# troyvvgroup/quemb

Measured on AMD Instinct MI355X. Metric: fragment CCSD iters/sec (full BE sweep over synthetic n_occ=20 n_virt=200 fragments); corr-E error vs oracle in parity_max_abs_err_Eh / parity_n220_abs_err_Eh, higher is better.
Workload: dtype f64

## Files before the change

### include/qemb_hip_ops.h

```cpp
#ifndef QEMB_HIP_OPS_H
#define QEMB_HIP_OPS_H
#include "qemb_hip.h"
#ifdef __cplusplus
extern "C" {
#endif

#define QEMB_TIMER_LADDER 0
#define QEMB_TIMER_RINGS 1
#define QEMB_TIMER_ITER 2
#define QEMB_TIMER_AO2MO 3
#define QEMB_TIMER_SCF 4
#define QEMB_TIMER_GEMM_ANY 5
#define QEMB_TIMER_SCHMIDT 6
#define QEMB_TIMER_DF 7
int qemb_timer_begin(int slot);
int qemb_timer_end(int slot);
int qemb_timer_read(int slot, double* total_ms, int64_t* count);
int qemb_timer_reset(int slot);
int qemb_alloc_stats(long long* n_driver_allocs, long long* n_driver_frees, double* ms_in_driver_calls, double* gb_allocated, int reset);
int qemb_gemm_flop_count(double* flops, int reset);
int qemb_tape_cache_counters(int64_t* reused, int64_t* recorded, int reset);
int qemb_ctx_timer_read(int ctx, int slot, double* total_ms, int64_t* count, int reset);
int qemb_timer_live_events(int slot);


int qemb_op_gemm(int64_t M, int64_t N, int64_t K, double alpha, const double* A, int64_t lda, int a_kcontig,
                 int64_t strideA, const double* B, int64_t ldb, int b_kcontig, int64_t strideB, double beta,
                 double* C, int64_t ldc, int64_t strideC, int64_t batch);
int qemb_op_gemm_slab_rows(int64_t M, int64_t N, int64_t K, const double* A, int64_t lda, int64_t a_slab, int64_t a_slab_skip, const double* B, int64_t ldb,
                           int b_kcontig, double* C, int64_t ldc, int cfg);
int qemb_set_gemm_config(int cfg);
int qemb_mfma_f64_peak(int iters, int blocks_per_cu, double* tflops);
int qemb_set_gemm_splitk(int enabled);
int qemb_op_gemm_probe(int64_t M, int64_t N, int64_t K, const double* A, int64_t lda, int a_kcontig, const double* B, int64_t ldb, int b_kcontig,
                       double* C, int64_t ldc, int cfg, int ksplit, double* ms, double* clock_ghz, int64_t* workgroups);
int qemb_op_gemm_stamps(int64_t M, int64_t N, int64_t K, const double* A, int64_t lda, const double* B, int64_t ldb, double* C, int64_t ldc, int cfg,
                        int ksplit, double* out7);
int qemb_pair_gemm_choice(int64_t rows, int64_t cols, int* cfg, int* ksplit);
int qemb_ccsd_gemm_plans(int o, int v, int64_t* out);
int qemb_set_gemm_ksplit(int ksplit);
int qemb_gemm_tile_table(int index, int* id, int* rows, int* cols, int* bk, int* mode1, int* has_classic, int* ladder_twin);
int qemb_gemm_last_launch(int* cfg, int* vec2, int* mode, int* ksplit, int* sb_m, int* sb_n, int* wide_c);
int qemb_op_copy4(const int64_t dim[4], const double* in, const int64_t si[4], double* out,
                  const int64_t so[4], double alpha, double beta);
int qemb_op_outer4(const int64_t dim[4], const double* u, int64_t su0, int64_t su2, const double* v,
                   int64_t sv1, int64_t sv3, double* out, const int64_t so[4], double alpha, double beta);
int qemb_op_div_denom(double* x, int64_t d0, int64_t d1, int64_t d2, int64_t d3, const double* ea,
                      const double* eb, const double* ec, const double* ed);
int qemb_op_ladder_pack_vvvv(int64_t n, int64_t o, const double* M, double* Vp, int64_t ldp, double* Vm, int64_t ldm);
int qemb_op_ladder_pack_tau(int64_t o, int64_t v, const double* tau, double* Tp, int64_t ldp, double* Tm, int64_t ldm);
int qemb_op_ladder_scatter_pm(int64_t o, int64_t v, const double* Rp, int64_t ldp, const double* Rm, int64_t ldm, double* t2);
int qemb_op_dot(int64_t n, const double* x, const double* y, double* out_dev);
int qemb_op_absmax(int64_t n, const double* x, double* out_dev);
int qemb_op_gemv_rows(int64_t rows, int64_t cols, const double* T, int64_t ldt, const double* x, double* y,
                      double alpha, double beta);
int qemb_op_gemv_rows_batched(int64_t rows, int64_t cols, int64_t nbatch, const double* T, int64_t ldt, int64_t strideT,
                              const double* x, int64_t stridex, double* y, double alpha, double beta);
int qemb_op_contract_mid(int64_t outer, int64_t mid, int64_t inner, const double* T, const double* x,
                         double* Y, int64_t ldy, double alpha, double beta);
int qemb_op_unpack_s4(int64_t n, const double* s4, double* s1);
int qemb_op_pack_s4(int64_t n, const double* s1, double* s4);
int qemb_op_unpack_s8_to_s4(int64_t n, const double* s8, double* s4);
int qemb_op_mirror_lower(int64_t n, double* A, int64_t lda);
int qemb_op_k_from_pairs(int64_t n, const double* H, const double* D, double* K);
int qemb_op_jk_from_packed(int64_t n, const double* S4, const double* D, const double* Dp, double* Jp, double* K);
int qemb_op_pack_pm_cols(int64_t rows, int64_t v, const double* in, double* Op, int64_t ldp, double* Om, int64_t ldm);
int qemb_op_scatter_pm_rows(int64_t o, int64_t ncols, const double* Xp, const double* Xm, double* out);
int qemb_op_pack_w_pm(int64_t o, const double* W, double* Ap, int64_t lda_p, double* Am, int64_t lda_m);
int qemb_op_ladder_scatter_pm2(int64_t o, int64_t v, const double* Rp, int64_t ldp, const double* Rm, int64_t ldm, const double* Hp, const double* Hm,
                               int assign, double* t2);
int qemb_op_lincomb2(int64_t n, double a, const double* x, double b, const double* y, double beta, double* out);
int qemb_op_small_k_update(int64_t batch, int64_t M, int64_t N, int64_t K, double alpha, const double* A, int64_t sA, const double* B, int64_t sB, double* C, int64_t sC);
int qemb_op_ccsd_ph_layouts(int64_t o, int64_t v, const double* t2, const double* t1, double* T, double* Tp, double* S, double* Ut, double* Tpt, double* Th);
int qemb_op_ccsd_y_traces(int64_t o, int64_t v, const double* ZC, const double* ZB, double* Y);
int qemb_op_copy4_two(const int64_t dim[4], const double* in, const int64_t si[4], double* out, const int64_t so[4], double alpha, double beta, const double* base,
                      double* out2, const double* in2, double c2a, double c2b);
int qemb_op_scatter_pm_rows_add(int64_t o, int64_t ncols, const double* Xp, const double* Xm, double* out, const double* add);
int qemb_op_ccsd_y_traces_add(int64_t o, int64_t v, const double* ZC, const double* ZB, double* Y, const double* add);
int qemb_op_pack_w_pm_sum(int64_t o, const double* Wt, const double* X, const double* At, double* Ap, int64_t lda_p, double* Am, int64_t lda_m);
int qemb_op_ccsd_t1_small(int64_t o, int64_t v, const double* t1, const double* Lvv, const double* Loo, const double* Fov, double* t1n);
int qemb_op_ccsd_t1_assemble(int64_t o, int64_t v, const double* t1, const double* Lvv, const double* Loo, const double* Fov, const double* S, const double* Lph1,
                             const double* PA, int SA, int64_t strideA, const double* PB, int SB, int64_t strideB, double* t1n);
int qemb_op_gemv_rows_two(int64_t rows1, int64_t cols1, const double* T1, int64_t ld1, const double* x1, double* y1, double a1, double b1,
                          int64_t rows2, int64_t cols2, const double* T2, int64_t ld2, const double* x2, double* y2, double a2, double b2);
int qemb_op_ccsd_y_traces_slabs(int64_t o, int64_t v, const double* ZC, const double* ZB, double* Y, const double* add, int S, int64_t stride, double scale);
int qemb_op_gemv_rows2(int64_t rows, int64_t cols, const double* T1, int64_t ld1, const double* x1, const double* T2, int64_t ld2, const double* x2, double* y, double alpha, double beta);
int qemb_op_ccsd_finish_t2_rings(int64_t o, int64_t v, double* t2n, const double* U, const double* OV, const double* RS, const double* M, const double* eo, const double* ev, double* t1n);
int qemb_op_diis_push(int64_t n, const double* trial, const double* prev, double* e, double* xcopy, int m, const double* const* ys, int self, double* row_dev, double* row_host);
int qemb_op_ccsd_extrapolate_energy(int64_t o, int64_t v, int nterms, const double* coef, const double* const* xs, double* amp, const double* L, double* tau, double* e_host);
int qemb_op_gather_rows(int64_t nrows, int64_t len, const int64_t* idx_dev, const double* src, int64_t ld, double* dst);
int qemb_op_scale_rows(int64_t nrows, int64_t len, double* x, const double* s);
int qemb_op_pack_pair_rows(int64_t n, int64_t ncols, const double* in, double* out);
int qemb_op_unpack_tril_pair_rows(int64_t nr, int64_t n, const double* in, double* full);
int qemb_op_extract_pf(int64_t n, const double* Mp, int64_t p0, int64_t q0, int64_t r0, int64_t s0, int64_t sp, int64_t sq,
                       int64_t sr, int64_t ss, double* out);
int qemb_op_extract_pf_t(int64_t n, const double* T, int64_t x0, int64_t r0, int64_t s0, int64_t c0, int64_t sx, int64_t sr,
                         int64_t ss, int64_t sc, double* out);
int qemb_op_ladder_pack_vvvv_pf(int64_t n, int64_t o, const double* Mp, double* Vp, int64_t ldp, double* Vm, int64_t ldm);
int qemb_op_extract_pf_t_compact(int64_t n, const double* T, int64_t x0, int64_t c0, int64_t sx, int64_t sr, int64_t ss, int64_t sc,
                                 double* out, int64_t slab);
int qemb_op_gather_pair_cols(int64_t rows, int64_t n, const double* in, int64_t r0, int64_t s0, int64_t sr, int64_t ss, double* out);
int qemb_op_extract_ps(int64_t n, const double* S, int64_t p0, int64_t q0, int64_t r0, int64_t s0, int64_t sp, int64_t sq,
                       int64_t sr, int64_t ss, double* out);
int qemb_op_extract_ps_packed(int64_t n, const double* S, int64_t p0, int64_t q0, int64_t r0, int64_t sp, int64_t sq, int64_t sr, double* out);
int qemb_op_unpack_pair_block(int64_t n, int64_t o, const double* S, double* Mv, int64_t ld);
int qemb_op_ladder_pack_vvvv_pf_ld(int64_t n, int64_t o, const double* Mp, int64_t ld, double* Vp, int64_t ldp, double* Vm, int64_t ldm);
int qemb_op_pack_pm_ovvv(int64_t o, int64_t v, const double* ovvv, double* Op, int64_t ldp, double* Om, int64_t ldm);
int qemb_op_df_pair_product(int64_t np, int64_t naux, const double* bb, double* out);
int qemb_op_unpack_tril_rows(int64_t rows, int64_t n, const double* packed, double* full);
int qemb_op_pack_tril_rows(int64_t rows, int64_t n, const double* full, double* packed);
int qemb_op_jacobi_eigh(int64_t n, double* A, double* w, double* V, int* sweeps);
int qemb_op_scf_fused_max(void);
int qemb_op_jacobi_eigh_in_basis(int64_t n, const double* F, const double* Cp, double* w, double* C_out, double* C2_out, int nocc, double* dm_out, double stop_below, int* sweeps);
int qemb_op_scf_fock_small(int64_t n, const double* h, const double* J, const double* K, const double* D, double* F, double* err, double* scal2);
int qemb_op_pack_density_sym(int64_t n, const double* D, double* Dp);
int qemb_op_jacobi_svd(int64_t m, int64_t n, double* G, double* s, double* U, double* V, int* sweeps);
int qemb_op_cholesky_lower(int64_t n, double* A);
int qemb_op_tri_inverse_lower(int64_t n, const double* L, double* Linv);


int qemb_op_mp2_amplitudes(int64_t o, int64_t v, const double* ovov, const double* eo, const double* ev, double* t2, double* G, double* e_host);

int qemb_op_rdm2_assemble(int kind, int64_t o, int64_t v, const double* t1, const double* t2, const double* dm1c, double* out);
int qemb_op_rdm2_add_nc(int64_t m, const double* g, double alpha, double* X);
int qemb_op_rdm2_symmetrize(int64_t m, const double* g, double* X);
int qemb_op_rdm2_eri_dot(int64_t m, int sym, const double* eri, const double* K, double* e_host);

int qemb_op_kdf_split(int64_t rows, int64_t nao, const double* z, double* planes);
int qemb_op_kdf_stack(int64_t nk, int64_t nao, int64_t n, const double* ta, double* Cs, double* Dk);
int qemb_op_kdf_pack(int64_t naux, int64_t n, const double* M, int paired, double w, double* F, int64_t ldf, double* out2_host);

int qemb_frag_prepare_ccsd(qemb_frag_t f, int nsocc, const double* h, const double* dm0, const qemb_solver_opts* opts);
int qemb_frag_ccsd_iterate(qemb_frag_t f, int niter, double* e_corr, double* normt);
int qemb_frag_ccsd_reset(qemb_frag_t f);
int qemb_frag_ccsd_export(qemb_frag_t f, const char* name, double* host, int64_t nelem);


int qemb_op_boys(int m_max, int64_t n, const double* x, double* out);
int qemb_op_int3c_class(int la, int lb, int lP, const void* bf_a, const void* bf_b, const void* bf_P, const double* c2s, double* out_host);
int qemb_op_int4c_class(int la, int lb, int lc, int ld, const void* bf_a, const void* bf_b, const void* bf_c, const void* bf_d, const double* c2s, double* out_host);
int qemb_op_int4c_tile(void* basis, const int32_t* pairs_r, int64_t n_r, const int32_t* pairs_s, int64_t n_s, double thresh, double* out_host);
int qemb_op_cd_panel_factor(int n, const double* A_host, double thr, double* T_host, int32_t* piv_host, int32_t* rank, int* in_lds);
int qemb_op_cd_diag_update(int64_t np, int r, const double* Lnew_host, const int32_t* pivrow_host, double* d_host, int64_t nsp, const int32_t* row0_host, const int32_t* cnt_host,
                           double* spmax_host, double* dmax_host);
int qemb_op_cd_permute(int64_t M, int64_t N, const double* L_host, const int32_t* pos_host, int full, double* out_host);
int qemb_op_df_get_ints(void* df, double* out_host, int* identity_metric);

int qemb_op_fci_sigma(int n, int nsocc, const double* h_host, const double* V_dev, const double* c_dev, double* sigma_dev);
int qemb_op_fci_rdm12(int n, int nsocc, const double* c_dev, int cumulant, double* dm1_host, double* dm2_dev);
int qemb_op_fci_sigma_timed(int n, int nsocc, const double* h_host, const double* V_dev, const double* c_dev, double* sigma_dev, double* ms3);
int qemb_op_fci_links(int n, int nsocc, int64_t* ns, int* nlink, int32_t* strings_host, int32_t* links_host);

int qemb_op_joint_diag(int64_t K, int64_t m, double* Q_dev, double* U_dev, double stop_angle, int max_sweeps, int* sweeps, double* f, int* converged);
int qemb_op_joint_diag_bytes(int64_t K, int64_t m, int64_t* bytes, int* in_lds);
int qemb_op_joint_diag_mem_limit(int64_t bytes);

#ifdef __cplusplus
}
#endif
#endif
```

### quemb_amd/_lib.py

```python

from __future__ import annotations

import ctypes as C
import os
from pathlib import Path

import numpy as np

_HERE = Path(__file__).resolve().parent
LIB_PATH = _HERE / "libqemb_hip.so"

c_dp = C.POINTER(C.c_double)
c_i64 = C.c_int64
c_vp = C.c_void_p


QEMB_ERR_ARG, QEMB_ERR_ALLOC, QEMB_ERR_DEVICE, QEMB_ERR_NOCONV, QEMB_ERR_NUMERIC, QEMB_ERR_UNSUPPORTED = -1, -2, -3, -4, -5, -6


class QembError(RuntimeError):

    def __init__(self, msg="", status=None):
        super().__init__(msg)
        self.status = status


class SolverOpts(C.Structure):
    _fields_ = [("struct_size", C.c_uint32), ("cc_conv_tol", C.c_double), ("cc_conv_tol_normt", C.c_double), ("cc_max_cycle", C.c_int),
                ("cc_diis_space", C.c_int), ("scf_conv_tol", C.c_double), ("scf_conv_tol_grad", C.c_double),
                ("scf_max_cycle", C.c_int), ("scf_diis_space", C.c_int), ("warm_start", C.c_int), ("verbose", C.c_int),
                ("relax_density", C.c_int), ("lambda_conv_tol", C.c_double), ("lambda_max_cycle", C.c_int),
                ("strict_convergence", C.c_int)]


class FciOpts(C.Structure):
    _fields_ = [("struct_size", C.c_uint32), ("conv_tol", C.c_double), ("max_cycle", C.c_int), ("max_space", C.c_int), ("lindep", C.c_double)]


_lib = None
_initialised_device = None


def _declare(lib):
    def f(name, restype, *argtypes):
        fn = getattr(lib, name)
        fn.restype = restype
        fn.argtypes = list(argtypes)

    I, D, P, V, L = C.c_int, C.c_double, c_vp, c_vp, c_i64
    f("qemb_init", I, I)
    f("qemb_last_error", C.c_char_p)
    f("qemb_backend", C.c_char_p)
    f("qemb_sync", I)
    f("qemb_device_sync", I)
    f("qemb_mem_info", I, C.POINTER(C.c_size_t), C.POINTER(C.c_size_t))
    f("qemb_malloc", I, C.POINTER(c_vp), C.c_size_t)
    f("qemb_free", I, V)
    f("qemb_trim", I)
    f("qemb_trim_all", I)
    f("qemb_h2d", I, V, V, C.c_size_t)
    f("qemb_d2h", I, V, V, C.c_size_t)
    f("qemb_h2d_async", I, V, V, C.c_size_t)
    f("qemb_d2d", I, V, V, C.c_size_t)
    f("qemb_timer_begin", I, I)
    f("qemb_timer_end", I, I)
    f("qemb_timer_read", I, I, C.POINTER(D), C.POINTER(L))
    f("qemb_timer_reset", I, I)
    f("qemb_timer_live_events", I, I)
    f("qemb_op_gemm", I, L, L, L, D, P, L, I, L, P, L, I, L, D, P, L, L, L)
    f("qemb_op_gemm_slab_rows", I, L, L, L, P, L, L, L, P, L, I, P, L, I)
    f("qemb_op_gemm_probe", I, L, L, L, P, L, I, P, L, I, P, L, I, I, C.POINTER(D), C.POINTER(D), C.POINTER(L))
    f("qemb_op_gemm_stamps", I, L, L, L, P, L, P, L, P, L, I, I, C.POINTER(D))
    f("qemb_set_gemm_config", I, I)
    f("qemb_set_gemm_splitk", I, I)
    f("qemb_set_gemm_ksplit", I, I)
    f("qemb_pair_gemm_choice", I, L, L, C.POINTER(I), C.POINTER(I))
    f("qemb_ccsd_gemm_plans", I, I, I, C.POINTER(L))
    f("qemb_gemm_tile_table", I, I, *([C.POINTER(I)] * 7))
    f("qemb_gemm_last_launch", I, *([C.POINTER(I)] * 7))
    f("qemb_op_ladder_pack_vvvv", I, L, L, P, P, L, P, L)
    f("qemb_op_ladder_pack_tau", I, L, L, P, P, L, P, L)
    f("qemb_op_ladder_scatter_pm", I, L, L, P, L, P, L, P)
    f("qemb_mfma_f64_peak", I, I, I, C.POINTER(D))
    f("qemb_op_copy4", I, C.POINTER(L), P, C.POINTER(L), P, C.POINTER(L), D, D)
    f("qemb_op_outer4", I, C.POINTER(L), P, L, L, P, L, L, P, C.POINTER(L), D, D)
    f("qemb_op_div_denom", I, P, L, L, L, L, P, P, P, P)
    f("qemb_op_dot", I, L, P, P, P)
    f("qemb_op_mp2_amplitudes", I, L, L, P, P, P, P, P, C.POINTER(D))
    f("qemb_op_rdm2_assemble", I, I, L, L, P, P, P, P)
    f("qemb_op_rdm2_add_nc", I, L, P, D, P)
    f("qemb_op_rdm2_symmetrize", I, L, P, P)
    f("qemb_op_rdm2_eri_dot", I, L, I, P, P, C.POINTER(D))
    f("qemb_op_absmax", I, L, P, P)
    f("qemb_op_gemv_rows", I, L, L, P, L, P, P, D, D)
    f("qemb_op_gemv_rows_batched", I, L, L, L, P, L, L, P, L, P, D, D)
    f("qemb_op_contract_mid", I, L, L, L, P, P, P, L, D, D)
    f("qemb_op_unpack_s4", I, L, P, P)
    f("qemb_op_pack_s4", I, L, P, P)
    f("qemb_op_unpack_s8_to_s4", I, L, P, P)
    f("qemb_op_unpack_tril_rows", I, L, L, P, P)
    f("qemb_op_pack_pair_rows", I, L, L, P, P)
    f("qemb_op_mirror_lower", I, L, P, L)
    f("qemb_op_k_from_pairs", I, L, P, P, P)
    f("qemb_op_jk_from_packed", I, L, P, P, P, P, P)
    f("qemb_op_pack_pm_cols", I, L, L, P, P, L, P, L)
    f("qemb_op_scatter_pm_rows", I, L, L, P, P, P)
    f("qemb_op_pack_w_pm", I, L, P, P, L, P, L)
    f("qemb_op_ladder_scatter_pm2", I, L, L, P, L, P, L, P, P, I, P)
    f("qemb_op_lincomb2", I, L, D, P, D, P, D, P)
    f("qemb_op_small_k_update", I, L, L, L, L, D, P, L, P, L, P, L)
    f("qemb_op_ccsd_ph_layouts", I, L, L, P, P, P, P, P, P, P, P)
    f("qemb_op_ccsd_y_traces", I, L, L, P, P, P)
    f("qemb_op_copy4_two", I, C.POINTER(L), P, C.POINTER(L), P, C.POINTER(L), D, D, P, P, P, D, D)
    f("qemb_op_scatter_pm_rows_add", I, L, L, P, P, P, P)
    f("qemb_op_ccsd_y_traces_add", I, L, L, P, P, P, P)
    f("qemb_op_pack_w_pm_sum", I, L, P, P, P, P, L, P, L)
    f("qemb_op_ccsd_t1_small", I, L, L, P, P, P, P, P)
    f("qemb_op_gemv_rows2", I, L, L, P, L, P, P, L, P, P, D, D)
    f("qemb_op_ccsd_t1_assemble", I, L, L, P, P, P, P, P, P, P, I, L, P, I, L, P)
    f("qemb_op_gemv_rows_two", I, L, L, P, L, P, P, D, D, L, L, P, L, P, P, D, D)
    f("qemb_op_ccsd_y_traces_slabs", I, L, L, P, P, P, P, I, L, D)
    f("qemb_op_ccsd_finish_t2_rings", I, L, L, P, P, P, P, P, P, P, P)
    f("qemb_op_diis_push", I, L, P, P, P, P, I, P, I, P, P)
    f("qemb_op_ccsd_extrapolate_energy", I, L, L, I, P, P, P, P, P, P)
    f("qemb_op_gather_rows", I, L, L, P, P, L, P)
    f("qemb_op_scale_rows", I, L, L, P, P)
    f("qemb_ctx_count", I, I)
    f("qemb_ctx_bind", I, I)
    f("qemb_ctx_partition", I, I)
    f("qemb_ctx_timer_read", I, I, I, C.POINTER(C.c_double), C.POINTER(c_i64), I)
    f("qemb_gemm_flop_count", I, C.POINTER(C.c_double), I)
    f("qemb_tape_cache_counters", I, C.POINTER(L), C.POINTER(L), I)
    f("qemb_alloc_stats", I, C.POINTER(C.c_longlong), C.POINTER(C.c_longlong), C.POINTER(C.c_double), C.POINTER(C.c_double), I)
    f("qemb_op_unpack_tril_pair_rows", I, L, L, P, P)
    f("qemb_op_extract_pf", I, L, P, L, L, L, L, L, L, L, L, P)
    f("qemb_op_extract_pf_t", I, L, P, L, L, L, L, L, L, L, L, P)
    f("qemb_op_ladder_pack_vvvv_pf", I, L, L, P, P, L, P, L)
    f("qemb_op_extract_pf_t_compact", I, L, P, L, L, L, L, L, L, P, L)
    f("qemb_op_gather_pair_cols", I, L, L, P, L, L, L, L, P)
    f("qemb_op_extract_ps", I, L, P, L, L, L, L, L, L, L, L, P)
    f("qemb_op_extract_ps_packed", I, L, P, L, L, L, L, L, L, P)
    f("qemb_op_unpack_pair_block", I, L, L, P, P, L)
    f("qemb_op_ladder_pack_vvvv_pf_ld", I, L, L, P, L, P, L, P, L)
    f("qemb_op_pack_pm_ovvv", I, L, L, P, P, L, P, L)
    f("qemb_op_df_pair_product", I, L, L, P, P)
    f("qemb_op_pack_tril_rows", I, L, L, P, P)
    f("qemb_op_jacobi_eigh", I, L, P, P, P, C.POINTER(I))
    f("qemb_op_scf_fused_max", I)
    f("qemb_op_jacobi_eigh_in_basis", I, L, P, P, P, P, P, I, P, D, C.POINTER(I))
    f("qemb_op_scf_fock_small", I, L, P, P, P, P, P, P, P)
    f("qemb_op_pack_density_sym", I, L, P, P)
    f("qemb_op_jacobi_svd", I, L, L, P, P, P, P, C.POINTER(I))
    f("qemb_op_cholesky_lower", I, L, P)
    f("qemb_op_joint_diag", I, L, L, P, P, D, I, C.POINTER(I), C.POINTER(D), C.POINTER(I))
    f("qemb_df_localize_er", I, V, P, I, D, I, P, C.POINTER(I), C.POINTER(D), C.POINTER(D), C.POINTER(I))
    f("qemb_op_joint_diag_bytes", I, L, L, C.POINTER(L), C.POINTER(I))
    f("qemb_op_joint_diag_mem_limit", I, L)
    f("qemb_op_tri_inverse_lower", I, L, P, P)
    f("qemb_comm_unique_id", I, P)
    f("qemb_comm_init", I, I, I, P)
    f("qemb_comm_info", I, C.POINTER(I), C.POINTER(I))
    f("qemb_comm_allreduce", I, P, L, I)
    f("qemb_comm_destroy", I)
    OP = C.POINTER(SolverOpts)
    IP = C.POINTER(I)
    DP = C.POINTER(D)
    f("qemb_default_opts", None, OP)
    f("qemb_frag_create", I, I, I, C.POINTER(c_vp))
    f("qemb_frag_free", I, V)
    f("qemb_frag_set_eri_s4", I, V, P)
    f("qemb_frag_set_eri_s4_dev", I, V, P)
    f("qemb_frag_set_df_factor", I, V, I, P)
    f("qemb_frag_set_df_factor_dev", I, V, I, P)
    f("qemb_frag_mo_route", I, V, I)
    f("qemb_frag_set_df_only", I, V, I, P)
    f("qemb_frag_set_df_only_dev", I, V, I, V)
    f("qemb_frag_resident_bytes", I, V, C.POINTER(L))
    f("qemb_frag_mo_route_used", I, V, IP, IP)
    f("qemb_frag_get_eri_s4", I, V, P)
    f("qemb_frag_set_energy_data", I, V, P, P, P, D, IP, I)
    f("qemb_frag_jk", I, V, P, P, P)
    f("qemb_frag_solve", I, V, I, P, P, OP, I, P, P, P, P, P, P, P, DP, DP, DP, IP, IP)
    f("qemb_frag_solve_mp2", I, V, I, P, P, OP, I, P, P, P, P, P, P, DP, DP, DP, IP)
    f("qemb_frag_solve_mp2_batch", I, I, P, IP, P, P, OP, I, P, P, P, P, P, P, P, P, P, IP)
    f("qemb_default_fci_opts", None, C.POINTER(FciOpts))
    f("qemb_frag_solve_fci", I, V, I, P, P, OP, C.POINTER(FciOpts), I, P, P, P, P, P, P, DP, DP, DP, IP, IP)
    f("qemb_frag_fci_bytes", I, I, I, I, C.POINTER(L))
    f("qemb_frag_fci_mem_limit", I, V, L)
    f("qemb_frag_fci_residual", I, V, DP)
    f("qemb_op_fci_sigma", I, I, I, P, P, P, P)
    f("qemb_op_fci_rdm12", I, I, I, P, I, P, P)
    f("qemb_op_fci_sigma_timed", I, I, I, P, P, P, P, P)
    f("qemb_op_fci_links", I, I, I, C.POINTER(L), IP, P, P)
    f("qemb_frag_rdm2", I, V, I, I, P)
    f("qemb_frag_rdm2_mem_limit", I, V, L)
    f("qemb_frag_rdm2_dev", I, V, I, I, P)
    f("qemb_rdm2_full_guard", I, L, L, L)
    f("qemb_frag_lambda_iters", I, P, C.POINTER(C.c_int))
    f("qemb_frag_solve_batch", I, I, P, IP, P, P, OP, I, P, P, P, P, P, P, P, P, P, P, IP, IP, C.POINTER(L))
    f("qemb_frag_scf", I, V, I, P, P, OP, P, P, P, P, DP, IP, IP)
    f("qemb_frag_cphf", I, V, I, P, P, OP, P, I, P)
    f("qemb_ccsd_solve", I, I, I, I, P, P, P, OP, P, P, D, IP, I, P, P, P, P, P, P, DP, IP)
    f("qemb_frag_prepare_ccsd", I, V, I, P, P, OP)
    f("qemb_frag_ccsd_iterate", I, V, I, DP, DP)
    f("qemb_frag_ccsd_reset", I, V)
    f("qemb_frag_ccsd_export", I, V, C.c_char_p, P, L)
    LP = C.POINTER(L)
    f("qemb_aoeri_upload", I, I, P, I, C.POINTER(c_vp))
    f("qemb_aoeri_free", I, V)
    f("qemb_ao2mo_dense", I, V, P, I, P, V)
    f("qemb_df_create", I, I, P, C.POINTER(c_vp))
    f("qemb_lpq_upload", I, P, I, C.POINTER(c_vp))
    f("qemb_df_create_pbc", I, I, P, C.POINTER(c_vp), IP)
    f("qemb_df_alloc_ints", I, V, I)
    f("qemb_df_add_pw_block", I, V, I, P, P, P, P)
    f("qemb_df_add_rs_block", I, V, I, I, P)
    f("qemb_df_pw_imag_absmax", I, V, C.POINTER(C.c_double))
    f("qemb_df_pw_select", I, V, I)
    f("qemb_df_free", I, V)
    f("qemb_df_set_ints", I, V, I, P, I)
    f("qemb_df_set_ints_semisparse", I, V, I, L, P, P, P, P)
    f("qemb_df_transform", I, V, P, I, P, V)
    f("qemb_df_transform_screened", I, V, P, I, P, D, P, V)
    f("qemb_df_transform_factor", I, V, P, I, V)
    f("qemb_df_transform_screened_factor", I, V, P, I, P, D, V)
    f("qemb_kdf_create", I, I, I, I, IP, IP, C.POINTER(c_vp))
    f("qemb_kdf_set_pair", I, V, I, I, P)
    f("qemb_kdf_transform", I, V, P, I, P, V, I)
    f("qemb_kdf_free", I, V)
    f("qemb_kdf_guard", I, I, I, I, I, I, I, L)
    f("qemb_frag_get_df_factor", I, V, P)
    f("qemb_int_basis_create", I, I, P, C.c_size_t, P, C.POINTER(c_vp))
    f("qemb_int_basis_free", I, V)
    f("qemb_int3c2e", I, V, V, P, L, I, P, I)
    f("qemb_int2c2e", I, V, P, I)
    f("qemb_df_create_empty", I, C.POINTER(c_vp))
    f("qemb_df_set_ints_from_basis", I, V, V, V)
    f("qemb_df_set_ints_semisparse_from_basis", I, V, V, V, L, P, P, P, P)
    f("qemb_int4c2e", I, V, I, D, P, I)
    f("qemb_int4c_mem_limit", I, V, L)
    f("qemb_int4c_stats", I, V, C.POINTER(L), C.POINTER(L))
    f("qemb_aoeri_from_basis", I, V, D, C.POINTER(c_vp))
    f("qemb_int_jk_direct", I, V, P, D, P, P, I)
    f("qemb_int_jk_direct_bytes", I, V, C.POINTER(L))
    f("qemb_ao2mo_direct", I, V, I, P, P, P, P, L, D)
    f("qemb_ao2mo_direct_bytes", I, V, I, P, L, C.POINTER(L))
    f("qemb_int4c_tile_stats", I, V, C.POINTER(L), C.POINTER(L))
    f("qemb_op_int4c_tile", I, V, P, L, P, L, D, P)
    f("qemb_int_cholesky", I, V, D, D, L, L, P, C.POINTER(L))
    f("qemb_int_cholesky_bytes", I, V, L, L, C.POINTER(L))
    f("qemb_int_cholesky_stats", I, V, P)
    f("qemb_df_set_ints_from_cholesky", I, V, V, D, D, L, L)
    f("qemb_op_cd_panel_factor", I, I, P, D, P, P, C.POINTER(C.c_int32), C.POINTER(I))
    f("qemb_op_cd_diag_update", I, L, I, P, P, P, L, P, P, P, P)
    f("qemb_op_cd_permute", I, L, L, P, P, I, P)
    f("qemb_op_df_get_ints", I, V, P, C.POINTER(I))
    f("qemb_int1e", I, V, I, P, P, P, P, P)
    f("qemb_int1e_dipole", I, V, P, P)
    f("qemb_df_jk", I, V, I, P, P, I, I, I, P, P)
    f("qemb_df_jk_bytes", I, V, I, I, C.POINTER(L))
    f("qemb_df_jk_mem_limit", I, V, L)
    f("qemb_op_int4c_class", I, I, I, I, I, P, P, P, P, P, P)
    f("qemb_op_boys", I, I, L, P, P)
    f("qemb_op_int3c_class", I, I, I, I, P, P, P, P, P)
    f("qemb_op_kdf_split", I, L, L, P, P)
    f("qemb_op_kdf_stack", I, L, L, L, P, P, P)
    f("qemb_op_kdf_pack", I, L, L, P, I, D, P, L, DP)
    f("qemb_schmidt", I, P, I, I, I, LP, I, D, P, I, IP, IP)
    f("qemb_schmidt_subspace", I, P, I, I, I, LP, I, D, P, I, IP, IP)
    f("qemb_schmidt_svd", I, P, I, LP, I, D, P, I, IP, IP)
    f("qemb_nsocc_guess", I, P, I, I, P, IP, P)
    f("qemb_matmul", I, L, L, L, P, I, P, I, P)
    f("qemb_abs_overlap_prim", I, I, P, P, P, P, L, I, P, P, P)
    return lib


def load(path: os.PathLike | None = None):
    global _lib
    if _lib is None:
        p = Path(path) if path else LIB_PATH
        if not p.exists():
            raise QembError(
                f"{p} not found: build it with `python -c 'import __graft_entry__ as g; g.build()'` "
                "(make -C quemb_amd/csrc). quemb_amd has no CPU fallback."
            )
        _lib = _declare(C.CDLL(str(p)))
    return _lib


def declare(cdll):
    return _declare(cdll)


class ConvergenceWarning(RuntimeWarning):
    """A fragment solve did not converge and `strict_convergence = 0` asked for PySCF's behaviour (warn, carry on)."""


def check(rc: int, what: str = "", lib=None):
    if rc > 0:
        import warnings
        msg = (lib or load()).qemb_last_error().decode(errors="replace")
        warnings.warn(ConvergenceWarning(f"{what or 'libqemb_hip call'}: {msg}"), stacklevel=3)
    elif rc != 0:
        msg = (lib or load()).qemb_last_error().decode(errors="replace")
        raise QembError(f"{what or 'libqemb_hip call'} failed (status {rc}): {msg}", status=int(rc))


def init(device: int | None = None):
    global _initialised_device
    lib = load()
    if device is None:
        if _initialised_device is not None:
            return lib
        device = int(os.environ.get("LOCAL_RANK", "0"))
    if _initialised_device != device:
        check(lib.qemb_init(int(device)), "qemb_init")
        _initialised_device = device
    return lib


class DeviceBuffer:

    def __init__(self, nelem: int, lib=None):
        self.lib = lib or init()
        self.n = int(nelem)
        p = c_vp()
        check(self.lib.qemb_malloc(C.byref(p), max(self.n, 1) * 8), "qemb_malloc")
        self.ptr = p.value

    @classmethod
    def from_numpy(cls, a: np.ndarray, lib=None):
        a = np.ascontiguousarray(a, dtype=np.float64)
        b = cls(a.size, lib=lib)
        b.upload(a)
        return b

    def upload(self, a: np.ndarray):
        a = np.ascontiguousarray(a, dtype=np.float64)
        assert a.size <= self.n
        check(self.lib.qemb_h2d(self.ptr, a.ctypes.data, a.size * 8), "qemb_h2d")

    def numpy(self, shape=None) -> np.ndarray:
        out = np.empty(self.n, dtype=np.float64)
        check(self.lib.qemb_d2h(out.ctypes.data, self.ptr, self.n * 8), "qemb_d2h")
        return out if shape is None else out[: int(np.prod(shape))].reshape(shape)

    def at(self, offset_elems: int) -> int:
        return self.ptr + 8 * int(offset_elems)

    def free(self):
        if getattr(self, "ptr", None):
            self.lib.qemb_free(self.ptr)
            self.ptr = None

    def __del__(self):
        try:
            self.free()
        except Exception:
            pass


def i64x4(v):
    return (c_i64 * 4)(*[int(x) for x in v])
```

### quemb_amd/csrc/ao2mo.cpp

```cpp
#include "ao2mo.h"
#include "int4c_core.h"
#include <algorithm>
#include <cmath>
#include <cstdlib>
#include <vector>

namespace qemb {

static inline int64_t npair(int64_t n) { return n * (n + 1) / 2; }

int AoEri::upload(int N_, const double* host, int sym) {
  N = N_;
  const int64_t np = npair(N), n2 = (int64_t)N * N;
  QTRY(s4.alloc(np * np));
  if (sym == 4) return dev_h2d(s4, host, sizeof(double) * np * np);
  if (sym == 8) {
    DBuf s8;
    const int64_t n8 = np * (np + 1) / 2;
    QTRY(s8.alloc(n8));
    QTRY(dev_h2d(s8, host, sizeof(double) * n8));
    return dev_unpack_s8_to_s4(N, s8, s4);
  }
  if (sym == 1) {
    DBuf s1;
    QTRY(s1.alloc(n2 * n2));
    QTRY(dev_h2d(s1, host, sizeof(double) * n2 * n2));
    return dev_pack_s4(N, s1, s4);
  }
  set_error("AoEri::upload: sym must be 1, 4 or 8");
  return QEMB_ERR_ARG;
}

int ao2mo_dense(const AoEri& ao, const double* TA, int n, double* out_s4) {
  const int64_t N = ao.N;
  if (N <= 0 || n <= 0 || n > N) { set_error("ao2mo_dense: need 0 < n <= N"); return QEMB_ERR_ARG; }
  const int64_t npN = npair(N), npn = npair(n);
  DBuf W1, W2;
  QTRY(W1.alloc(std::max<int64_t>(npN * N * N, (int64_t)n * n * npN)));
  QTRY(W2.alloc(std::max<int64_t>((int64_t)n * npN * N, npn * N * N)));
  TimerScope lap_AO2MO(TIMER_AO2MO);
  const int tcfg = fits_one_224_tile(n) ? GEMM_224x128 : -1;
  QTRY(dev_unpack_tril_rows(npN, N, ao.s4, W1));
  QTRY(gemm(n, npN * N, N, 1.0, TA, n, false, W1, N, true, 0.0, W2, npN * N, 1, 0, 0, 0, tcfg));
  QTRY(gemm_quarter_lower_rows(n, npN, N, TA, W2, W1));
  QTRY(dev_unpack_tril_pair_rows(n, N, W1, W2));
  QTRY(gemm(n, npn * N, N, 1.0, TA, n, false, W2, N, true, 0.0, W1, npn * N, 1, 0, 0, 0, tcfg));
  QTRY(gemm_quarter_lower_rows(n, npn, N, TA, W1, W2));
  QTRY(dev_pack_pair_rows(n, npn, W2, out_s4));
  QTRY(lap_AO2MO.close());
  return 0;
}

int ao2mo_tile_accumulate(const double* E, int64_t ld, const TileRows& R, const TileRows& S, bool diagonal, const double* TA, int n, double* PR, double* PS,
                          double* T, double* A) {
  const int64_t npq = npair(n);
  int4c::PairProdArgs g{};
  g.TA = TA; g.n = n; g.npq = npq;
  g.mu = S.mu; g.nu = S.nu; g.rows = S.rows; g.P = PS;
  QTRY(dev_int4c_pairprod(g));
  if (!diagonal) {
    g.mu = R.mu; g.nu = R.nu; g.rows = R.rows; g.P = PR;
    QTRY(dev_int4c_pairprod(g));
  }
  QTRY(gemm(R.rows, npq, S.rows, 1.0, E, ld, true, PS, npq, false, 0.0, T, npq));
  return gemm(npq, npq, R.rows, diagonal ? 0.5 : 1.0, diagonal ? PS : PR, npq, false, T, npq, false, 1.0, A, npq);
}

int DfContext::set_metric(int naux_, const double* j2c) {
  naux = naux_; identity_metric = false;
  DBuf L;
  QTRY(L.alloc((int64_t)naux * naux));
  QTRY(dev_h2d(L, j2c, sizeof(double) * naux * naux));
  QTRY(dev_cholesky_lower(naux, L));
  QTRY(Linv.alloc((int64_t)naux * naux));
  return dev_tri_inverse_lower(naux, L, Linv);
}
int DfContext::set_cholesky_factor(int naux_, const double* Lh) {
  naux = naux_; identity_metric = false;
  DBuf L;
  QTRY(L.alloc((int64_t)naux * naux));
  QTRY(dev_h2d(L, Lh, sizeof(double) * naux * naux));
  QTRY(Linv.alloc((int64_t)naux * naux));
  return dev_tri_inverse_lower(naux, L, Linv);
}
int DfContext::set_metric_pbc(int naux_, const double* j2c, int* ischol) {
  naux = naux_; identity_metric = false;
  DBuf A, w, V;
  const int64_t n2 = (int64_t)naux * naux;
  QTRY(A.alloc(n2));
  QTRY(dev_h2d(A, j2c, sizeof(double) * n2));
  QTRY(Linv.alloc(n2));
  int rc = dev_cholesky_lower(naux, A);
  if (rc == QEMB_OK) { if (ischol) *ischol = 1; return dev_tri_inverse_lower(naux, A, Linv); }
  if (rc != QEMB_ERR_NUMERIC) return rc;
  if (ischol) *ischol = 0;
  QTRY(dev_h2d(A, j2c, sizeof(double) * n2));
  QTRY(w.alloc(naux)); QTRY(V.alloc(n2));
  QTRY(dev_jacobi_eigh(naux, A, w, V, nullptr));
  {
    DBuf AV, D;
    QTRY(AV.alloc(n2)); QTRY(D.alloc(n2));
    QTRY(dev_h2d(A, j2c, sizeof(double) * n2));
    QTRY(gemm(naux, naux, naux, 1.0, A, naux, true, V, naux, false, 0.0, AV, naux));
    QTRY(gemm(naux, naux, naux, 1.0, V, naux, false, AV, naux, false, 0.0, D, naux));
    Copy4Desc c{};
    c.dim[0] = 1; c.dim[1] = 1; c.dim[2] = 1; c.dim[3] = naux;
    c.in = D; c.si[0] = 0; c.si[1] = 0; c.si[2] = 0; c.si[3] = naux + 1;
    c.out = w; c.so[0] = 0; c.so[1] = 0; c.so[2] = 0; c.so[3] = 1; c.alpha = 1.0; c.beta = 0.0;
    QTRY(dev_copy4(c));
  }
  std::vector<double> d(naux);
  QTRY(dev_d2h(d.data(), w, sizeof(double) * naux));
  for (double& x : d) x = (x > 1e-14) ? 1.0 / std::sqrt(std::sqrt(x)) : 0.0;
  QTRY(dev_h2d(w, d.data(), sizeof(double) * naux));
  QTRY(dev_mul_bcast_rows(naux, naux, V, w));
  return gemm(naux, naux, naux, 1.0, V, naux, true, V, naux, true, 0.0, Linv, naux);
}
int DfContext::alloc_ints(int N_) {
  if (naux <= 0) { set_error("DfContext: set the metric first"); return QEMB_ERR_ARG; }
  if (N_ <= 0) { set_error("DfContext::alloc_ints: N must be positive"); return QEMB_ERR_ARG; }
  N = N_;
  Usp.release(); n_unique = 0;
  const int64_t sz = (int64_t)naux * N * N;
  QTRY(Lpq.alloc(sz)); QTRY(Lpq_im.alloc(sz));
  Lpq_sum.release(); Lact = nullptr;
  QTRY(dev_fill(Lpq, sz, 0.0));
  return dev_fill(Lpq_im, sz, 0.0);
}
int DfContext::add_rs_block(int p0, int p1, const double* h) {
  if (!Lpq.p || !Lpq_im.p) { set_error("DfContext::add_rs_block: alloc_ints first"); return QEMB_ERR_ARG; }
  if (p0 < 0 || p1 > naux || p0 >= p1 || !h) { set_error("DfContext::add_rs_block: need 0 <= p0 < p1 <= naux"); return QEMB_ERR_ARG; }
  const int64_t n2 = (int64_t)N * N, sz = (int64_t)(p1 - p0) * n2;
  DBuf tmp;
  QTRY(tmp.alloc(sz));
  QTRY(dev_h2d(tmp, h, sizeof(double) * sz));
  return axpby(sz, 1.0, tmp, 1.0, Lpq.p + (int64_t)p0 * n2);
}
int DfContext::add_pw_block(int nG, const double* F_re, const double* F_im, const double* pw_re, const double* pw_im) {
  if (!Lpq.p || !Lpq_im.p) { set_error("DfContext::add_pw_block: alloc_ints first"); return QEMB_ERR_ARG; }
  if (nG <= 0 || !F_re || !F_im || !pw_re || !pw_im) { set_error("DfContext::add_pw_block: bad arguments"); return QEMB_ERR_ARG; }
  const int64_t n2 = (int64_t)N * N;
  DBuf fr, fi, pr, pi;
  QTRY(fr.alloc((int64_t)naux * nG)); QTRY(fi.alloc((int64_t)naux * nG));
  QTRY(pr.alloc((int64_t)nG * n2)); QTRY(pi.alloc((int64_t)nG * n2));
  QTRY(dev_h2d(fr, F_re, sizeof(double) * naux * nG)); QTRY(dev_h2d(fi, F_im, sizeof(double) * naux * nG));
  QTRY(dev_h2d(pr, pw_re, sizeof(double) * nG * n2)); QTRY(dev_h2d(pi, pw_im, sizeof(double) * nG * n2));
  QTRY(gemm(naux, n2, nG, 1.0, fr, nG, true, pr, n2, false, 1.0, Lpq, n2));
  QTRY(gemm(naux, n2, nG, -1.0, fi, nG, true, pi, n2, false, 1.0, Lpq, n2));
  QTRY(gemm(naux, n2, nG, 1.0, fr, nG, true, pi, n2, false, 1.0, Lpq_im, n2));
  return gemm(naux, n2, nG, 1.0, fi, nG, true, pr, n2, false, 1.0, Lpq_im, n2);
}
int DfContext::imag_absmax(double* out) const {
  if (!Lpq_im.p || !out) { set_error("DfContext::imag_absmax: no plane-wave accumulation on this context"); return QEMB_ERR_ARG; }
  DBuf r;
  QTRY(r.alloc(1));
  QTRY(dev_absmax((int64_t)naux * N * N, Lpq_im, r));
  return dev_d2h(out, r, sizeof(double));
}
int DfContext::select_part(int part) {
  if (part == 0) { Lact = nullptr; return QEMB_OK; }
  if (!Lpq.p || !Lpq_im.p) { set_error("DfContext::select_part: no plane-wave accumulation on this context"); return QEMB_ERR_ARG; }
  if (part == 1) { Lact = Lpq_im.p; return QEMB_OK; }
  if (part == 2) {
    const int64_t sz = (int64_t)naux * N * N;
    QTRY(Lpq_sum.alloc(sz));
    QTRY(dcopy(sz, Lpq, Lpq_sum));
    QTRY(axpby(sz, 1.0, Lpq_im, 1.0, Lpq_sum));
    Lact = Lpq_sum.p;
    return QEMB_OK;
  }
  set_error("DfContext::select_part: part must be 0, 1 or 2");
  return QEMB_ERR_ARG;
}
int DfContext::set_ints_Lpq(int N_, const double* h) {
  N = N_;
  Usp.release(); n_unique = 0; Lact = nullptr; Lpq_im.release(); Lpq_sum.release();
  if (naux <= 0) { set_error("DfContext: set the metric first"); return QEMB_ERR_ARG; }
  QTRY(Lpq.alloc((int64_t)naux * N * N));
  return dev_h2d(Lpq, h, sizeof(double) * naux * N * N);
}
int DfContext::set_ints_pqL(int N_, const double* h) {
  N = N_;
  Usp.release(); n_unique = 0; Lact = nullptr; Lpq_im.release(); Lpq_sum.release();
  if (naux <= 0) { set_error("DfContext: set the metric first"); return QEMB_ERR_ARG; }
  DBuf tmp;
  const int64_t n2 = (int64_t)N * N;
  QTRY(tmp.alloc(n2 * naux));
  QTRY(dev_h2d(tmp, h, sizeof(double) * n2 * naux));
  QTRY(Lpq.alloc(n2 * naux));
  return perm4(Lpq, tmp, 1, 1, n2, naux, 0, 1, 3, 2);
}
int DfContext::set_ints_packed(int N_, const double* h) {
  N = N_;
  Usp.release(); n_unique = 0; Lact = nullptr; Lpq_im.release(); Lpq_sum.release();
  if (naux <= 0) { set_error("DfContext: set the metric first"); return QEMB_ERR_ARG; }
  DBuf tmp;
  QTRY(tmp.alloc((int64_t)naux * npair(N)));
  QTRY(dev_h2d(tmp, h, sizeof(double) * naux * npair(N)));
  QTRY(Lpq.alloc((int64_t)naux * N * N));
  return dev_unpack_tril_rows(naux, N, tmp, Lpq);
}

int DfContext::set_ints_semisparse(int N_, int64_t n_unique_, const double* unique_host, const int64_t* ptr, const int32_t* nu,
                                   const int64_t* off) {
  if (n_unique_ > 0 && !unique_host) { set_error("set_ints_semisparse: bad arguments"); return QEMB_ERR_ARG; }
  QTRY(begin_ints_semisparse(N_, n_unique_, ptr, nu, off));
  return n_unique > 0 ? dev_h2d(Usp, unique_host, sizeof(double) * n_unique * naux) : QEMB_OK;
}

int DfContext::set_metric_from_device(int naux_, DBuf&& J) {
  if (naux_ <= 0 || !J.p) { set_error("DfContext::set_metric_from_device: bad arguments"); return QEMB_ERR_ARG; }
  naux = naux_; identity_metric = false;
  DBuf L = std::move(J);
  QTRY(dev_cholesky_lower(naux, L));
  QTRY(Linv.alloc((int64_t)naux * naux));
  return dev_tri_inverse_lower(naux, L, Linv);
}
int DfContext::begin_ints_Lpq(int N_) {
  if (naux <= 0) { set_error("DfContext: set the metric first"); return QEMB_ERR_ARG; }
  if (N_ <= 0) { set_error("DfContext::begin_ints_Lpq: N must be positive"); return QEMB_ERR_ARG; }
  N = N_;
  Usp.release(); n_unique = 0; Lact = nullptr; Lpq_im.release(); Lpq_sum.release();
  return Lpq.alloc((int64_t)naux * N * N);
}
int DfContext::begin_ints_identity(int N_, int naux_) {
  if (N_ <= 0 || naux_ <= 0) { set_error("DfContext::begin_ints_identity: N and the number of vectors must be positive"); return QEMB_ERR_ARG; }
  N = N_; naux = naux_;
  Linv.release(); identity_metric = true;
  Usp.release(); n_unique = 0; Lact = nullptr; Lpq_im.release(); Lpq_sum.release();
  return Lpq.alloc((int64_t)naux * N * N);
}
int DfContext::begin_ints_semisparse(int N_, int64_t n_unique_, const int64_t* ptr, const int32_t* nu, const int64_t* off) {
  if (naux <= 0) { set_error("DfContext: set the metric first"); return QEMB_ERR_ARG; }
  if (N_ <= 0 || n_unique_ < 0 || !ptr || (n_unique_ > 0 && (!nu || !off))) { set_error("set_ints_semisparse: bad arguments"); return QEMB_ERR_ARG; }
  if (ptr[0] != 0) { set_error("set_ints_semisparse: reach_ptr[0] must be 0"); return QEMB_ERR_ARG; }
  for (int mu = 0; mu < N_; ++mu) {
    if (ptr[mu + 1] < ptr[mu]) { set_error("set_ints_semisparse: reach_ptr must be non-decreasing"); return QEMB_ERR_ARG; }
    for (int64_t e = ptr[mu]; e < ptr[mu + 1]; ++e)
      if (nu[e] < 0 || nu[e] >= N_ || off[e] < 0 || off[e] >= n_unique_) { set_error("set_ints_semisparse: partner or offset out of range"); return QEMB_ERR_ARG; }
  }
  N = N_; n_unique = n_unique_;
  reach_ptr.assign(ptr, ptr + N + 1);
  reach_nu.assign(nu, nu + ptr[N]);
  reach_off.assign(off, off + ptr[N]);
  Lpq.release(); Lact = nullptr; Lpq_im.release(); Lpq_sum.release();
  return Usp.alloc(std::max<int64_t>(1, n_unique * naux));
}

int DfContext::finish_from_pair_rows(int n, const double* bpT, double* out_s4, DBuf* keep_bb) const {
  const int64_t np = npair(n);
  DBuf bbT;
  QTRY(bbT.alloc(np * naux));
  QTRY(gemm(np, naux, naux, 1.0, bpT, naux, true, Linv, naux, true, 0.0, bbT, naux));
  if (keep_bb) {
    QTRY(keep_bb->alloc(naux * np));
    QTRY(perm4(*keep_bb, bbT, 1, 1, np, naux, 0, 1, 3, 2));
  }
  if (!out_s4) return 0;
  const int64_t nblk = np >= 2048 ? 8 : 1;
  const int64_t w = ((np + nblk - 1) / nblk + 127) / 128 * 128;
  for (int64_t c0 = 0; c0 < np; c0 += w) {
    const int64_t cw = std::min(w, np - c0);
    QTRY(gemm(np - c0, cw, naux, 1.0, bbT.p + c0 * naux, naux, true, bbT.p + c0 * naux, naux, true, 0.0, out_s4 + c0 * np + c0, np));
  }
  if (nblk > 1) QTRY(dev_mirror_lower(np, out_s4, np));
  return 0;
}

int DfContext::transform_semisparse(const double* TA, int n, double* out_s4, const double* S_abs, double eps, DBuf* keep_bb) const {
  const int64_t np = npair(n);
  DBuf T1, T2, bpT, maskb, Xb, TAact, idx_dev;
  TimerScope lap_DF(TIMER_DF);
  std::vector<int64_t> act;
  if (S_abs) {
    QTRY(Xb.alloc((int64_t)N * n)); QTRY(maskb.alloc((int64_t)N * n));
    QTRY(gemm(N, n, N, 1.0, S_abs, N, true, TA, n, false, 0.0, Xb, n));
    QTRY(dev_threshold_mask((int64_t)N * n, Xb, eps, maskb));
    std::vector<double> mh((size_t)N * n);
    QTRY(dev_d2h(mh.data(), maskb, sizeof(double) * N * n));
    for (int64_t mu = 0; mu < N; ++mu) {
      bool any = false;
      for (int i = 0; i < n && !any; ++i) any = mh[(size_t)mu * n + i] != 0.0;
      if (any) act.push_back(mu);
    }
  } else {
    act.resize(N);
    for (int64_t mu = 0; mu < N; ++mu) act[mu] = mu;
  }
  const int64_t Na = (int64_t)act.size();
  if (Na == 0) {
    QTRY(dev_fill(out_s4, np * np, 0.0));
    return lap_DF.close();
  }
  QTRY(T1.alloc(Na * n * naux));
  {
    int64_t budget = (int64_t)1 << 27;
    budget = std::max<int64_t>(1, env_int("QEMB_DF_GATHER_BUDGET", budget));
    int64_t a0 = 0;
    std::vector<int64_t> idxD, idxT;
    DBuf Dg, TAg;
    while (a0 < Na) {
      int64_t Kc = 0, a1 = a0;
      while (a1 < Na) {
        const int64_t k = reach_ptr[act[a1] + 1] - reach_ptr[act[a1]];
        const int64_t Kn = std::max(Kc, std::max<int64_t>(k, 1));
        if (a1 > a0 && (a1 + 1 - a0) * Kn * (naux + n) > budget) break;
        Kc = Kn; ++a1;
      }
      const int64_t B = a1 - a0;
      idxD.assign(B * Kc, -1); idxT.assign(B * Kc, -1);
      for (int64_t b = 0; b < B; ++b) {
        const int64_t e0 = reach_ptr[act[a0 + b]], cnt = reach_ptr[act[a0 + b] + 1] - e0;
        for (int64_t k = 0; k < cnt; ++k) { idxD[b * Kc + k] = reach_off[e0 + k]; idxT[b * Kc + k] = reach_nu[e0 + k]; }
      }
      QTRY(idx_dev.alloc(2 * B * Kc));
      QTRY(dev_h2d(idx_dev, idxD.data(), sizeof(int64_t) * B * Kc));
      QTRY(dev_h2d(idx_dev.p + B * Kc, idxT.data(), sizeof(int64_t) * B * Kc));
      QTRY(Dg.alloc(B * Kc * naux)); QTRY(TAg.alloc(B * Kc * n));
      QTRY(dev_gather_rows(B * Kc, naux, reinterpret_cast<const int64_t*>(idx_dev.p), Usp, naux, Dg));
      QTRY(dev_gather_rows(B * Kc, n, reinterpret_cast<const int64_t*>(idx_dev.p + B * Kc), TA, n, TAg));
      QTRY(gemm(n, naux, Kc, 1.0, TAg, n, false, Dg, naux, false, 0.0, T1.p + a0 * n * naux, naux, B, Kc * n, Kc * naux, (int64_t)n * naux));
      QTRY(dev_sync());
      a0 = a1;
    }
  }
  QTRY(idx_dev.alloc(Na));
  QTRY(dev_h2d(idx_dev, act.data(), sizeof(int64_t) * Na));
  QTRY(TAact.alloc(Na * n));
  QTRY(dev_gather_rows(Na, n, reinterpret_cast<const int64_t*>(idx_dev.p), TA, n, TAact));
  if (S_abs) {
    QTRY(dev_gather_rows(Na, n, reinterpret_cast<const int64_t*>(idx_dev.p), maskb, n, Xb));
    QTRY(dev_scale_rows(Na * n, naux, T1, Xb));
  }
  QTRY(T2.alloc((int64_t)n * n * naux));
  QTRY(gemm(n, naux, Na, 1.0, TAact, n, false, T1, (int64_t)n * naux, false, 0.0, T2, (int64_t)n * naux, n, 0, naux, naux));
  T1.release();
  QTRY(bpT.alloc(np * naux));
  QTRY(dev_pack_pair_rows(n, naux, T2, bpT));
  T2.release();
  QTRY(finish_from_pair_rows(n, bpT, out_s4, keep_bb));
  QTRY(lap_DF.close());
  return 0;
}

int DfContext::transform(const double* TA, int n, double* out_s4, const double* S_abs, double eps, DBuf* keep_bb) const {
  if (n <= 0 || n > N) { set_error("df transform: need 0 < n <= N"); return QEMB_ERR_ARG; }
  if (Linv.p && Usp.p) return transform_semisparse(TA, n, out_s4, S_abs, eps, keep_bb);
  if ((!Linv.p && !identity_metric) || !Lpq.p) { set_error("DfContext: metric and 3-index integrals must be set"); return QEMB_ERR_ARG; }
  const int64_t np = npair(n);
  DBuf T1, T2, bp, bb;
  QTRY(T1.alloc((int64_t)naux * n * N)); QTRY(T2.alloc((int64_t)naux * n * n));
  QTRY(bp.alloc((int64_t)naux * np));
  if (!identity_metric) QTRY(bb.alloc((int64_t)naux * np));
  TimerScope lap_DF(TIMER_DF);
  QTRY(gemm(n, N, N, 1.0, TA, n, false, Lact ? Lact : Lpq.p, N, false, 0.0, T1, N, naux, 0, (int64_t)N * N, (int64_t)n * N));
  if (S_abs) {
    DBuf X, mask;
    QTRY(X.alloc((int64_t)n * N)); QTRY(mask.alloc((int64_t)n * N));
    QTRY(gemm(n, N, N, 1.0, TA, n, false, S_abs, N, false, 0.0, X, N));
    QTRY(dev_threshold_mask((int64_t)n * N, X, eps, mask));
    QTRY(dev_mul_bcast_rows(naux, (int64_t)n * N, T1, mask));
  }
  if (S_abs) {
    QTRY(gemm(n, n, N, 1.0, TA, n, false, T1, N, true, 0.0, T2, n, naux, 0, (int64_t)n * N, (int64_t)n * n));
  } else {
    QTRY(gemm((int64_t)naux * n, n, N, 1.0, T1, N, true, TA, n, false, 0.0, T2, n));
  }
  QTRY(dev_pack_tril_rows(naux, n, T2, bp));
  if (identity_metric) bb = std::move(bp);
  else QTRY(gemm(naux, np, naux, 1.0, Linv, naux, true, bp, np, false, 0.0, bb, np));
  if (out_s4) QTRY(df_pair_product(np, naux, bb, out_s4));
  if (keep_bb) *keep_bb = std::move(bb);
  QTRY(lap_DF.close());
  return 0;
}

int DfContext::jk_check(const char* who) const {
  if (Usp.p) { set_error(std::string(who) + ": a semi-sparse context holds no dense tensor; J / K from it are not supported"); return QEMB_ERR_UNSUPPORTED; }
  if (Lpq_im.p) { set_error(std::string(who) + ": a periodic context (planar re / im tensor) is not supported"); return QEMB_ERR_UNSUPPORTED; }
  if ((!Linv.p && !identity_metric) || !Lpq.p || N <= 0 || naux <= 0) { set_error(std::string(who) + ": metric and 3-index integrals must be set"); return QEMB_ERR_ARG; }
  return 0;
}
static int64_t jk_splitk_slices(int64_t N, int64_t K) {
  const int64_t t = ((N + 255) / 256) * ((N + 255) / 256);
  if (K < 1024 || t >= 256) return 0;
  const int64_t S = std::min<int64_t>((768 + t - 1) / t, K / 256);
  return S > 1 ? S : 0;
}
static int64_t jk_words(int64_t naux, int64_t N, bool identity, int64_t ncol, int64_t kb) {
  return (identity ? 1 : 2) * naux * N * kb + N * ncol + (3 + jk_splitk_slices(N, naux * kb)) * N * N + 3 * naux;
}
int DfContext::jk_bytes(int ncol, int occ_block, int64_t* bytes) const {
  QTRY(jk_check("qemb_df_jk_bytes"));
  if (ncol < 0 || occ_block < 0 || !bytes) { set_error("qemb_df_jk_bytes: bad arguments"); return QEMB_ERR_ARG; }
  const int64_t kb = occ_block > 0 ? std::min(occ_block, ncol) : ncol;
  *bytes = 8 * jk_words(naux, N, identity_metric, ncol, kb);
  return QEMB_OK;
}
int DfContext::jk(const double* dm_host, const double* Cw_host, int npos, int nneg, int occ_block, double* J_host, double* K_host) const {
  QTRY(jk_check("qemb_df_jk"));
  if (npos < 0 || nneg < 0 || occ_block < 0 || (!J_host && !K_host)) { set_error("qemb_df_jk: bad arguments"); return QEMB_ERR_ARG; }
  const int64_t ncol = (int64_t)npos + nneg, n2 = (int64_t)N * N;
  if (ncol > 0 && !Cw_host) { set_error("qemb_df_jk: the density factor is null"); return QEMB_ERR_ARG; }
  const bool need_cw = K_host || !dm_host;
  size_t free_b = 0, total_b = 0;
  QTRY(dev_mem_info(&free_b, &total_b));
  double room = (double)free_b;
  if (jk_mem_limit >= 0 && (double)jk_mem_limit < room) room = (double)jk_mem_limit;
  int64_t kb = K_host ? (occ_block > 0 ? std::min<int64_t>(occ_block, ncol) : ncol) : 0;
  if (occ_block <= 0)
    while (kb > 1 && 8.0 * (double)jk_words(naux, N, identity_metric, ncol, kb) > room) kb = (kb + 1) / 2;
  const double need = 8.0 * (double)jk_words(naux, N, identity_metric, ncol, kb);
  if (need > room) {
    auto bytes = [](double b) { const std::string t = std::to_string(b); return t.substr(0, t.find('.')) + " bytes"; };
    set_error("qemb_df_jk: with N = " + std::to_string(N) + ", naux = " + std::to_string(naux) + " and slabs of " + std::to_string(kb) + " columns the J / K work space takes " +
              bytes(need) + ", more than the " + bytes(room) + " of device memory it may take");
    return QEMB_ERR_ALLOC;
  }
  constexpr int64_t kBatchMax = 32768;
  DBuf D, Cw, J, K, vec, Y, Z;
  if (need_cw && ncol > 0) { QTRY(Cw.alloc((int64_t)N * ncol)); QTRY(dev_h2d(Cw, Cw_host, sizeof(double) * N * ncol)); }
  TimerScope lap_DF(TIMER_DF);
  if (J_host) {
    QTRY(D.alloc(n2)); QTRY(J.alloc(n2)); QTRY(vec.alloc(3 * (int64_t)naux));
    if (dm_host) QTRY(dev_h2d(D, dm_host, sizeof(double) * n2));
    else {
      QTRY(dev_fill(D, n2, 0.0));
      if (npos > 0) QTRY(gemm(N, N, npos, 1.0, Cw, ncol, true, Cw, ncol, true, 0.0, D, N, 1, 0, 0, 0, -1, -1));
      if (nneg > 0) QTRY(gemm(N, N, nneg, -1.0, Cw.p + npos, ncol, true, Cw.p + npos, ncol, true, 1.0, D, N, 1, 0, 0, 0, -1, -1));
    }
    double *rho = vec.p, *t = vec.p + naux, *c = vec.p + 2 * (int64_t)naux;
    QTRY(dev_gemv_rows(naux, n2, Lpq, n2, D, rho, 1.0, 0.0));
    if (identity_metric) c = rho;
    else {
      QTRY(dev_gemv_rows(naux, naux, Linv, naux, rho, t, 1.0, 0.0));
      QTRY(dev_contract_mid(1, naux, naux, Linv, t, c, naux, 1.0, 0.0));
    }
    QTRY(dev_contract_mid(1, naux, n2, Lpq, c, J, n2, 1.0, 0.0));
  }
  if (K_host) {
    QTRY(K.alloc(n2));
    QTRY(dev_fill(K, n2, 0.0));
    if (kb > 0) {
      QTRY(Y.alloc((int64_t)naux * N * kb));
      if (!identity_metric) QTRY(Z.alloc((int64_t)naux * N * kb));
    }
    bool first = true;
    for (int sign = 0; sign < 2; ++sign) {
      const int64_t c0 = sign ? npos : 0, c1 = sign ? ncol : npos;
      for (int64_t k0 = c0; k0 < c1; k0 += kb) {
        const int64_t w = std::min(kb, c1 - k0), ld = (int64_t)naux * w;
        for (int64_t P0 = 0; P0 < naux; P0 += kBatchMax)
          QTRY(gemm(N, w, N, 1.0, Lpq.p + P0 * n2, N, true, Cw.p + k0, ncol, false, 0.0, Y.p + P0 * w, ld, std::min<int64_t>(kBatchMax, naux - P0), n2, 0, w, -1, -1));
        const double* F = Y;
        if (!identity_metric) {
          for (int64_t m0 = 0; m0 < N; m0 += kBatchMax)
            QTRY(gemm(naux, w, naux, 1.0, Linv, naux, true, Y.p + m0 * ld, w, false, 0.0, Z.p + m0 * ld, w, std::min<int64_t>(kBatchMax, N - m0), 0, ld, ld, -1, -1));
          F = Z;
        }
        QTRY(gemm(N, N, ld, sign ? -1.0 : 1.0, F, ld, true, F, ld, true, first ? 0.0 : 1.0, K, N));
        first = false;
      }
    }
    QTRY(dev_mirror_lower(N, K, N));
  }
  QTRY(lap_DF.close());
  if (J_host) QTRY(dev_d2h(J_host, J, sizeof(double) * n2));
  if (K_host) QTRY(dev_d2h(K_host, K, sizeof(double) * n2));
  return dev_sync();
}

int df_pair_product(int64_t np, int64_t naux, const double* bb, double* out) {
  const int64_t nblk = np >= 2048 ? 8 : 1;
  const int64_t w = ((np + nblk - 1) / nblk + 127) / 128 * 128;
  for (int64_t c0 = 0; c0 < np; c0 += w) {
    const int64_t cw = std::min(w, np - c0);
    QTRY(gemm(np - c0, cw, naux, 1.0, bb + c0, np, false, bb + c0, np, false, 0.0, out + c0 * np + c0, np));
  }
  if (nblk > 1) QTRY(dev_mirror_lower(np, out, np));
  return 0;
}

}
```

### quemb_amd/csrc/ao2mo.h

```cpp
#pragma once
#include <cstdint>
#include <vector>
#include "dev_ops.h"
#include "tensor_utils.h"

namespace qemb {

class AoEri {
 public:
  int N = 0;
  DBuf s4;
  int upload(int N_, const double* eri_host, int sym);
};

int ao2mo_dense(const AoEri& ao, const double* TA_dev, int n, double* out_s4_dev);

struct TileRows { const int32_t* mu; const int32_t* nu; int64_t rows; };
int ao2mo_tile_accumulate(const double* E, int64_t ld, const TileRows& R, const TileRows& S, bool diagonal, const double* TA_dev, int n, double* PR, double* PS,
                          double* T, double* A);

class DfContext {
 public:
  int N = 0, naux = 0;
  DBuf Linv;
  DBuf Lpq;
  int set_metric(int naux_, const double* j2c_host);
  int set_cholesky_factor(int naux_, const double* L_host);
  int set_metric_pbc(int naux_, const double* j2c_host, int* ischol);
  int alloc_ints(int N_);
  int add_rs_block(int p0, int p1, const double* block_host);
  int add_pw_block(int nG, const double* F_re, const double* F_im, const double* pw_re, const double* pw_im);
  int imag_absmax(double* out_host) const;
  int select_part(int part);
  DBuf Lpq_im, Lpq_sum;
  const double* Lact = nullptr;
  int set_ints_pqL(int N_, const double* pqL_host);
  int set_ints_Lpq(int N_, const double* Lpq_host);
  int set_ints_packed(int N_, const double* P_munu_packed_host);
  int set_ints_semisparse(int N_, int64_t n_unique_, const double* unique_host, const int64_t* reach_ptr, const int32_t* reach_nu,
                          const int64_t* reach_off);
  int set_metric_from_device(int naux_, DBuf&& j2c_dev);
  int begin_ints_Lpq(int N_);
  int begin_ints_identity(int N_, int naux_);
  bool identity_metric = false;
  int begin_ints_semisparse(int N_, int64_t n_unique_, const int64_t* reach_ptr, const int32_t* reach_nu, const int64_t* reach_off);
  int transform(const double* TA_dev, int n, double* out_s4_dev, const double* S_abs_dev = nullptr, double eps = 0.0, DBuf* keep_bb = nullptr) const;

  int jk(const double* dm_host, const double* Cw_host, int npos, int nneg, int occ_block, double* J_host, double* K_host) const;
  int jk_bytes(int ncol, int occ_block, int64_t* bytes) const;
  int64_t jk_mem_limit = -1;

  DBuf Usp;
  int64_t n_unique = 0;
  std::vector<int64_t> reach_ptr, reach_off;
  std::vector<int32_t> reach_nu;
 private:
  int transform_semisparse(const double* TA_dev, int n, double* out_s4_dev, const double* S_abs_dev, double eps, DBuf* keep_bb) const;
  int finish_from_pair_rows(int n, const double* bpT, double* out_s4, DBuf* keep_bb) const;
  int jk_check(const char* who) const;
};

int df_pair_product(int64_t np, int64_t naux, const double* bb, double* out);

}
```

### quemb_amd/csrc/api.cpp

```cpp
#include <cstring>
#include <cstdlib>
#include <vector>
#include <execinfo.h>
#include <signal.h>
#include <unistd.h>
#include "../../include/qemb_hip_ops.h"
#include "dev_ops.h"
#include "ccsd.h"
#include "fragment.h"
#include "ao2mo.h"
#include "kdf.h"
#include "int3c.h"
#include "int4c.h"
#include "cd_core.h"
#include "loc_core.h"
#include <mutex>
#include <set>

using namespace qemb;
namespace qemb {
int dev_mfma_f64_peak(int iters, int blocks_per_cu, double* tflops);
int schmidt_eigh(const double* lmo, int N, int nmo, int nocc, const int64_t* frag, int n_f, double thr, double* TA_out,
                 int ld_out, int* n_b_out, int* sweeps_out);
int schmidt_subspace(const double* lmo, int N, int nmo, int nocc, const int64_t* frag, int n_f, double thr, double* TA_out,
                     int ld_out, int* n_b_out, int* sweeps_out);
int schmidt_svd(const double* rdm, int N, const int64_t* frag_in, int n_f, double thr, double* TA_out, int ld_out, int* n_b_out,
                int* sweeps_out);
int nsocc_guess(const double* Cproj, int n, int nocc, double* P_out, int* nsocc, double* mo_out);
}

static thread_local int g_test_ksplit = 0;
#ifdef QEMB_HOSTCHECK
static thread_local GemmLaunchRecord g_hostcheck_last{};
#endif

extern "C" {

static void qemb_fault_handler(int sig) {
  void* frames[64];
  const int nfr = backtrace(frames, 64);
  const char msg[] = "[qemb] fatal signal; native backtrace:\n";
  (void)!write(2, msg, sizeof(msg) - 1);
  backtrace_symbols_fd(frames, nfr, 2);
  signal(sig, SIG_DFL);
  raise(sig);
}
int qemb_init(int device) {
  static const bool bt = [] { if (env_flag("QEMB_BACKTRACE", false)) { signal(SIGSEGV, qemb_fault_handler); signal(SIGABRT, qemb_fault_handler); } return true; }();
  (void)bt;
  return dev_init(device);
}
const char* qemb_last_error(void) { return last_error(); }
const char* qemb_backend(void) { return dev_backend_name(); }
int qemb_sync(void) { return dev_sync(); }
int qemb_device_sync(void) { return dev_sync_device(); }
int qemb_mem_info(size_t* f, size_t* t) { return dev_mem_info(f, t); }
int qemb_malloc(void** p, size_t bytes) { return dev_alloc(p, bytes); }
int qemb_free(void* p) { return dev_free(p); }
int qemb_trim(void) { return dev_trim(); }
int qemb_trim_all(void) { return dev_trim_all(); }
int qemb_h2d(void* d, const void* h, size_t b) { return dev_h2d(d, h, b); }
int qemb_d2h(void* h, const void* d, size_t b) { return dev_d2h(h, d, b); }
int qemb_h2d_async(void* d, const void* h, size_t b) { return dev_h2d_async(d, h, b); }
int qemb_d2d(void* d, const void* s, size_t b) { return dev_d2d(d, s, b); }
int qemb_timer_begin(int s) { return dev_timer_begin(s); }
int qemb_timer_end(int s) { return dev_timer_end(s); }
int qemb_timer_read(int s, double* ms, int64_t* c) { return dev_timer_read(s, ms, c); }
int qemb_timer_reset(int s) { return dev_timer_reset(s); }
int qemb_timer_live_events(int s) { return dev_timer_live_events(s); }

int qemb_op_gemm(int64_t M, int64_t N, int64_t K, double alpha, const double* A, int64_t lda, int a_kcontig,
                 int64_t strideA, const double* B, int64_t ldb, int b_kcontig, int64_t strideB, double beta,
                 double* C, int64_t ldc, int64_t strideC, int64_t batch) {
  GemmDesc g{M, N, K, alpha, beta, A, lda, a_kcontig, strideA, B, ldb, b_kcontig, strideB, C, ldc, strideC, batch, -1, g_test_ksplit};
#ifdef QEMB_HOSTCHECK
  g_hostcheck_last = GemmLaunchRecord{};
  g_hostcheck_last.vec2 = gemm_desc_vec2(g) ? 1 : 0;
  g_hostcheck_last.wide_c = gemm_wide_c(C, ldc, N, strideC, batch) ? 1 : 0;
#endif
  return dev_gemm(g);
}
int qemb_op_gemm_probe(int64_t M, int64_t N, int64_t K, const double* A, int64_t lda, int a_kcontig, const double* B, int64_t ldb, int b_kcontig,
                       double* C, int64_t ldc, int cfg, int ksplit, double* ms, double* clock_ghz, int64_t* workgroups) {
  GemmDesc g{M, N, K, 1.0, 0.0, A, lda, a_kcontig, 0, B, ldb, b_kcontig, 0, C, ldc, 0, 1, cfg, ksplit};
  long long wg = 0;
  const int rc = dev_gemm_probe(g, ms, clock_ghz, &wg);
  if (workgroups) *workgroups = wg;
  return rc;
}
int qemb_op_gemm_stamps(int64_t M, int64_t N, int64_t K, const double* A, int64_t lda, const double* B, int64_t ldb, double* C, int64_t ldc, int cfg, int ksplit,
                        double* out7) {
  GemmDesc g{M, N, K, 1.0, 0.0, A, lda, 1, 0, B, ldb, 1, 0, C, ldc, 0, 1, cfg, ksplit};
  return dev_gemm_stamps(g, 8, out7);
}
int qemb_gemm_tile_table(int index, int* id, int* rows, int* cols, int* bk, int* mode1, int* has_classic, int* ladder_twin) {
  GemmTileEntry e;
  if (!gemm_tile_entry(index, &e)) { set_error("qemb_gemm_tile_table: index past the end of the table"); return QEMB_ERR_ARG; }
  if (id) *id = e.id;
  if (rows) *rows = e.rows;
  if (cols) *cols = e.cols;
  if (bk) *bk = e.bk;
  if (mode1) *mode1 = e.mode1;
  if (has_classic) *has_classic = e.has_classic;
  if (ladder_twin) *ladder_twin = e.ladder_twin;
  return QEMB_OK;
}
int qemb_gemm_last_launch(int* cfg, int* vec2, int* mode, int* ksplit, int* sb_m, int* sb_n, int* wide_c) {
#ifdef QEMB_HOSTCHECK
  const GemmLaunchRecord r = g_hostcheck_last;
#else
  GemmLaunchRecord r;
  dev_gemm_last_launch(&r);
#endif
  if (cfg) *cfg = r.cfg;
  if (vec2) *vec2 = r.vec2;
  if (mode) *mode = r.mode;
  if (ksplit) *ksplit = r.ksplit;
  if (sb_m) *sb_m = r.sb_m;
  if (sb_n) *sb_n = r.sb_n;
  if (wide_c) *wide_c = r.wide_c;
  return QEMB_OK;
}
int qemb_set_gemm_ksplit(int ks) { g_test_ksplit = ks; return QEMB_OK; }
int qemb_set_gemm_config(int cfg) { dev_gemm_set_force_cfg(cfg); return QEMB_OK; }
#ifndef QEMB_HOSTCHECK
int qemb_mfma_f64_peak(int iters, int blocks_per_cu, double* tflops) { return dev_mfma_f64_peak(iters, blocks_per_cu, tflops); }
#else
int qemb_mfma_f64_peak(int, int, double*) { set_error("not available in the hostcheck build"); return QEMB_ERR_DEVICE; }
#endif
int qemb_pair_gemm_choice(int64_t rows, int64_t cols, int* cfg, int* ksplit) {
  const GemmPlan p = pick_pair_gemm(rows, cols);
  if (cfg) *cfg = p.cfg;
  if (ksplit) *ksplit = p.ks;
  return QEMB_OK;
}
int qemb_ccsd_gemm_plans(int o, int v, int64_t* out) {
  if (o < 1 || v < 0 || !out) { set_error("qemb_ccsd_gemm_plans: bad arguments"); return QEMB_ERR_ARG; }
  const CcsdGemmPlans p = ccsd_gemm_plans(o, v);
  for (const GemmPlan* g : {&p.fvv, &p.pa, &p.pb, &p.ladder_p, &p.ladder_m, &p.xw_p, &p.xw_m, &p.x_p, &p.x_m})
    for (const int64_t x : {g->M, g->N, g->K, (int64_t)g->cfg, (int64_t)g->ks, (int64_t)g->S}) *out++ = x;
  return QEMB_OK;
}
int qemb_set_gemm_splitk(int enabled) { dev_gemm_set_auto_splitk(enabled); return QEMB_OK; }
int qemb_op_copy4(const int64_t dim[4], const double* in, const int64_t si[4], double* out, const int64_t so[4],
                  double alpha, double beta) {
  Copy4Desc c{};
  for (int k = 0; k < 4; ++k) { c.dim[k] = dim[k]; c.si[k] = si[k]; c.so[k] = so[k]; }
  c.in = in; c.out = out; c.alpha = alpha; c.beta = beta;
  return dev_copy4(c);
}
int qemb_op_outer4(const int64_t dim[4], const double* u, int64_t su0, int64_t su2, const double* v, int64_t sv1,
                   int64_t sv3, double* out, const int64_t so[4], double alpha, double beta) {
  Outer4Desc o{};
  for (int k = 0; k < 4; ++k) { o.dim[k] = dim[k]; o.so[k] = so[k]; }
  o.u = u; o.su0 = su0; o.su2 = su2; o.v = v; o.sv1 = sv1; o.sv3 = sv3; o.out = out; o.alpha = alpha; o.beta = beta;
  return dev_outer4(o);
}
int qemb_op_div_denom(double* x, int64_t d0, int64_t d1, int64_t d2, int64_t d3, const double* ea, const double* eb,
                      const double* ec, const double* ed) { return dev_div_denom(x, d0, d1, d2, d3, ea, eb, ec, ed); }
int qemb_op_ladder_pack_vvvv(int64_t n, int64_t o, const double* M, double* Vp, int64_t ldp, double* Vm, int64_t ldm) { return dev_ladder_pack_vvvv(n, o, M, Vp, ldp, Vm, ldm); }
int qemb_op_ladder_pack_tau(int64_t o, int64_t v, const double* tau, double* Tp, int64_t ldp, double* Tm, int64_t ldm) { return dev_ladder_pack_tau(o, v, tau, Tp, ldp, Tm, ldm); }
int qemb_op_ladder_scatter_pm(int64_t o, int64_t v, const double* Rp, int64_t ldp, const double* Rm, int64_t ldm, double* t2) { return dev_ladder_scatter_pm(o, v, Rp, ldp, Rm, ldm, t2); }
int qemb_op_dot(int64_t n, const double* x, const double* y, double* o) { return dev_dot(n, x, y, o); }
int qemb_op_absmax(int64_t n, const double* x, double* o) { return dev_absmax(n, x, o); }
int qemb_op_gemv_rows(int64_t rows, int64_t cols, const double* T, int64_t ldt, const double* x, double* y, double alpha,
                      double beta) { return dev_gemv_rows(rows, cols, T, ldt, x, y, alpha, beta); }
int qemb_op_gemv_rows_batched(int64_t rows, int64_t cols, int64_t nbatch, const double* T, int64_t ldt, int64_t strideT, const double* x,
                              int64_t stridex, double* y, double alpha, double beta) { return dev_gemv_rows_batched(rows, cols, nbatch, T, ldt, strideT, x, stridex, y, alpha, beta); }
int qemb_op_contract_mid(int64_t outer, int64_t mid, int64_t inner, const double* T, const double* x, double* Y,
                         int64_t ldy, double alpha, double beta) { return dev_contract_mid(outer, mid, inner, T, x, Y, ldy, alpha, beta); }
int qemb_op_unpack_s4(int64_t n, const double* s4, double* s1) { return dev_unpack_s4(n, s4, s1); }
int qemb_op_pack_s4(int64_t n, const double* s1, double* s4) { return dev_pack_s4(n, s1, s4); }
int qemb_op_unpack_s8_to_s4(int64_t n, const double* s8, double* s4) { return dev_unpack_s8_to_s4(n, s8, s4); }
int qemb_comm_unique_id(void* id) { return dev_comm_unique_id(id); }
int qemb_comm_init(int rank, int world, const void* id) { return dev_comm_init(rank, world, id); }
int qemb_comm_info(int* rank, int* world) { return dev_comm_info(rank, world); }
int qemb_comm_allreduce(double* buf, int64_t n, int op) { return dev_comm_allreduce(buf, n, op); }
int qemb_comm_destroy(void) { return dev_comm_destroy(); }
int qemb_ctx_count(int n) { return dev_ctx_count(n); }
int qemb_ctx_bind(int k) { return dev_ctx_bind(k); }
int qemb_ctx_partition(int parts) { return dev_ctx_partition(parts); }
int qemb_op_gemm_slab_rows(int64_t M, int64_t N, int64_t K, const double* A, int64_t lda, int64_t a_slab, int64_t a_slab_skip, const double* B, int64_t ldb,
                           int b_kcontig, double* C, int64_t ldc, int cfg) {
  GemmDesc g{};
  g.M = M; g.N = N; g.K = K; g.alpha = 1.0; g.beta = 0.0;
  g.A = A; g.lda = lda; g.a_kcontig = 0; g.strideA = 0; g.a_slab = a_slab; g.a_slab_skip = a_slab_skip;
  g.B = B; g.ldb = ldb; g.b_kcontig = b_kcontig; g.strideB = 0;
  g.C = C; g.ldc = ldc; g.strideC = 0; g.batch = 1; g.cfg = cfg; g.ksplit = 0;
  return dev_gemm(g);
}
int qemb_gemm_flop_count(double* flops, int reset) { return dev_gemm_flop_count(flops, reset); }
int qemb_tape_cache_counters(int64_t* reused, int64_t* recorded, int reset) {
  long long a = 0, b = 0;
  tape_cache_counters(&a, &b, reset);
  if (reused) *reused = a;
  if (recorded) *recorded = b;
  return QEMB_OK;
}
int qemb_alloc_stats(long long* n, long long* nfree, double* ms, double* gb, int reset) { return dev_alloc_stats(n, nfree, ms, gb, reset); }
int qemb_ctx_timer_read(int ctx, int slot, double* total_ms, int64_t* count, int reset) { return dev_ctx_timer_read(ctx, slot, total_ms, count, reset); }
int qemb_op_k_from_pairs(int64_t n, const double* H, const double* D, double* K) { return dev_k_from_pairs(n, H, D, K); }
int qemb_op_jk_from_packed(int64_t n, const double* S4, const double* D, const double* Dp, double* Jp, double* K) { return dev_jk_from_packed(n, S4, D, Dp, Jp, K); }
int qemb_op_pack_pm_cols(int64_t rows, int64_t v, const double* in, double* Op, int64_t ldp, double* Om, int64_t ldm) { return dev_pack_pm_cols(rows, v, in, Op, ldp, Om, ldm); }
int qemb_op_scatter_pm_rows(int64_t o, int64_t ncols, const double* Xp, const double* Xm, double* out) { return dev_scatter_pm_rows(o, ncols, Xp, Xm, out); }
int qemb_op_pack_w_pm(int64_t o, const double* W, double* Ap, int64_t lda_p, double* Am, int64_t lda_m) { return dev_pack_w_pm(o, W, Ap, lda_p, Am, lda_m); }
int qemb_op_ladder_scatter_pm2(int64_t o, int64_t v, const double* Rp, int64_t ldp, const double* Rm, int64_t ldm, const double* Hp, const double* Hm,
                               int assign, double* t2) { return dev_ladder_scatter_pm2(o, v, Rp, ldp, Rm, ldm, Hp, Hm, assign, t2); }
int qemb_op_lincomb2(int64_t n, double a, const double* x, double b, const double* y, double beta, double* out) {
  const double c[2] = {a, b};
  const double* xs[2] = {x, y};
  return dev_lincomb(n, 2, c, xs, beta, out);
}
int qemb_op_mirror_lower(int64_t n, double* A, int64_t lda) { return dev_mirror_lower(n, A, lda); }
int qemb_op_small_k_update(int64_t batch, int64_t M, int64_t N, int64_t K, double alpha, const double* A, int64_t sA, const double* B, int64_t sB, double* C, int64_t sC) {
  return dev_small_k_update(batch, M, N, K, alpha, A, sA, B, sB, C, sC);
}
int qemb_op_ccsd_ph_layouts(int64_t o, int64_t v, const double* t2, const double* t1, double* T, double* Tp, double* S, double* Ut, double* Tpt, double* Th) {
  return dev_ccsd_ph_layouts(o, v, t2, t1, T, Tp, S, Ut, Tpt, Th);
}
int qemb_op_copy4_two(const int64_t dim[4], const double* in, const int64_t si[4], double* out, const int64_t so[4], double alpha, double beta, const double* base,
                      double* out2, const double* in2, double c2a, double c2b) {
  Copy4Desc c{};
  for (int k = 0; k < 4; ++k) { c.dim[k] = dim[k]; c.si[k] = si[k]; c.so[k] = so[k]; }
  c.in = in; c.out = out; c.alpha = alpha; c.beta = beta; c.base = base;
  c.out2 = out2; c.in2 = in2; c.c2a = c2a; c.c2b = c2b;
  return dev_copy4(c);
}
int qemb_op_scatter_pm_rows_add(int64_t o, int64_t ncols, const double* Xp, const double* Xm, double* out, const double* add) { return dev_scatter_pm_rows(o, ncols, Xp, Xm, out, add); }
int qemb_op_ccsd_y_traces_add(int64_t o, int64_t v, const double* ZC, const double* ZB, double* Y, const double* add) { return dev_ccsd_y_traces(o, v, ZC, ZB, Y, add); }
int qemb_op_pack_w_pm_sum(int64_t o, const double* Wt, const double* X, const double* At, double* Ap, int64_t lda_p, double* Am, int64_t lda_m) {
  return dev_pack_w_pm_sum(o, Wt, X, At, Ap, lda_p, Am, lda_m);
}
int qemb_op_ccsd_t1_small(int64_t o, int64_t v, const double* t1, const double* Lvv, const double* Loo, const double* Fov, double* t1n) { return dev_ccsd_t1_small(o, v, t1, Lvv, Loo, Fov, t1n); }
int qemb_op_ccsd_t1_assemble(int64_t o, int64_t v, const double* t1, const double* Lvv, const double* Loo, const double* Fov, const double* S, const double* Lph1,
                             const double* PA, int SA, int64_t strideA, const double* PB, int SB, int64_t strideB, double* t1n) {
  return dev_ccsd_t1_assemble(o, v, t1, Lvv, Loo, Fov, S, Lph1, PA, SA, strideA, PB, SB, strideB, t1n);
}
int qemb_op_gemv_rows_two(int64_t rows1, int64_t cols1, const double* T1, int64_t ld1, const double* x1, double* y1, double a1, double b1,
                          int64_t rows2, int64_t cols2, const double* T2, int64_t ld2, const double* x2, double* y2, double a2, double b2) {
  return dev_gemv_rows_two(rows1, cols1, T1, ld1, x1, y1, a1, b1, rows2, cols2, T2, ld2, x2, y2, a2, b2);
}
int qemb_op_ccsd_y_traces_slabs(int64_t o, int64_t v, const double* ZC, const double* ZB, double* Y, const double* add, int S, int64_t stride, double scale) {
  return dev_ccsd_y_traces(o, v, ZC, ZB, Y, add, S, stride, scale);
}
int qemb_op_gemv_rows2(int64_t rows, int64_t cols, const double* T1, int64_t ld1, const double* x1, const double* T2, int64_t ld2, const double* x2, double* y, double alpha, double beta) {
  return dev_gemv_rows2(rows, cols, T1, ld1, x1, T2, ld2, x2, y, alpha, beta);
}
int qemb_op_ccsd_finish_t2_rings(int64_t o, int64_t v, double* t2n, const double* U, const double* OV, const double* RS, const double* M, const double* eo, const double* ev, double* t1n) {
  return dev_ccsd_finish_t2_rings(o, v, t2n, U, OV, RS, M, eo, ev, t1n);
}
int qemb_op_diis_push(int64_t n, const double* trial, const double* prev, double* e, double* xcopy, int m, const double* const* ys, int self, double* row_dev, double* row_host) {
  void* pin = nullptr;
  QTRY(dev_pinned_alloc(&pin, sizeof(double) * 8));
  int rc = dev_diis_push(n, trial, prev, e, xcopy, m, ys, self, row_dev, (double*)pin);
  if (!rc) rc = dev_sync();
  if (!rc) for (int j = 0; j < m; ++j) row_host[j] = ((double*)pin)[j];
  dev_pinned_free(pin);
  return rc;
}
int qemb_op_ccsd_extrapolate_energy(int64_t o, int64_t v, int nterms, const double* coef, const double* const* xs, double* amp, const double* L, double* tau, double* e_host) {
  void* pin = nullptr;
  DBuf e_dev;
  QTRY(e_dev.alloc(1));
  QTRY(dev_pinned_alloc(&pin, sizeof(double) * 8));
  int rc = dev_ccsd_extrapolate_energy(o, v, nterms, coef, xs, amp, L, tau, e_dev, (double*)pin);
  if (!rc) rc = dev_sync();
  if (!rc) *e_host = *(double*)pin;
  dev_pinned_free(pin);
  return rc;
}
int qemb_op_ccsd_y_traces(int64_t o, int64_t v, const double* ZC, const double* ZB, double* Y) { return dev_ccsd_y_traces(o, v, ZC, ZB, Y); }
int qemb_op_gather_rows(int64_t nrows, int64_t len, const int64_t* idx_dev, const double* src, int64_t ld, double* dst) { return dev_gather_rows(nrows, len, idx_dev, src, ld, dst); }
int qemb_op_scale_rows(int64_t nrows, int64_t len, double* x, const double* s) { return dev_scale_rows(nrows, len, x, s); }
int qemb_op_pack_pair_rows(int64_t n, int64_t ncols, const double* in, double* out) { return dev_pack_pair_rows(n, ncols, in, out); }
int qemb_op_extract_pf(int64_t n, const double* Mp, int64_t p0, int64_t q0, int64_t r0, int64_t s0, int64_t sp, int64_t sq, int64_t sr, int64_t ss, double* out) {
  return dev_extract_pf(n, Mp, p0, q0, r0, s0, sp, sq, sr, ss, out);
}
int qemb_op_extract_pf_t(int64_t n, const double* T, int64_t x0, int64_t r0, int64_t s0, int64_t c0, int64_t sx, int64_t sr, int64_t ss, int64_t sc, double* out) {
  return dev_extract_pf_t(n, T, x0, r0, s0, c0, sx, sr, ss, sc, out);
}
int qemb_op_ladder_pack_vvvv_pf(int64_t n, int64_t o, const double* Mp, double* Vp, int64_t ldp, double* Vm, int64_t ldm) { return dev_ladder_pack_vvvv_pf(n, o, Mp, Vp, ldp, Vm, ldm); }
int qemb_op_extract_pf_t_compact(int64_t n, const double* T, int64_t x0, int64_t c0, int64_t sx, int64_t sr, int64_t ss, int64_t sc, double* out, int64_t slab) {
  return dev_extract_pf_t_compact(n, T, x0, c0, sx, sr, ss, sc, out, slab);
}
int qemb_op_gather_pair_cols(int64_t rows, int64_t n, const double* in, int64_t r0, int64_t s0, int64_t sr, int64_t ss, double* out) {
  return dev_gather_pair_cols(rows, n, in, r0, s0, sr, ss, out);
}
int qemb_op_extract_ps(int64_t n, const double* S, int64_t p0, int64_t q0, int64_t r0, int64_t s0, int64_t sp, int64_t sq, int64_t sr, int64_t ss, double* out) {
  return dev_extract_ps(n, S, p0, q0, r0, s0, sp, sq, sr, ss, out);
}
int qemb_op_extract_ps_packed(int64_t n, const double* S, int64_t p0, int64_t q0, int64_t r0, int64_t sp, int64_t sq, int64_t sr, double* out) {
  return dev_extract_ps_packed(n, S, p0, q0, r0, sp, sq, sr, out);
}
int qemb_op_unpack_pair_block(int64_t n, int64_t o, const double* S, double* Mv, int64_t ld) { return dev_unpack_pair_block(n, o, S, Mv, ld); }
int qemb_op_ladder_pack_vvvv_pf_ld(int64_t n, int64_t o, const double* Mp, int64_t ld, double* Vp, int64_t ldp, double* Vm, int64_t ldm) {
  return dev_ladder_pack_vvvv_pf_ld(n, o, Mp, ld, Vp, ldp, Vm, ldm);
}
int qemb_op_pack_pm_ovvv(int64_t o, int64_t v, const double* ovvv, double* Op, int64_t ldp, double* Om, int64_t ldm) { return dev_pack_pm_ovvv(o, v, ovvv, Op, ldp, Om, ldm); }
int qemb_op_df_pair_product(int64_t np, int64_t naux, const double* bb, double* out) { return df_pair_product(np, naux, bb, out); }
int qemb_op_unpack_tril_pair_rows(int64_t nr, int64_t n, const double* in, double* full) { return dev_unpack_tril_pair_rows(nr, n, in, full); }
int qemb_op_unpack_tril_rows(int64_t rows, int64_t n, const double* p, double* f) { return dev_unpack_tril_rows(rows, n, p, f); }
int qemb_op_pack_tril_rows(int64_t rows, int64_t n, const double* f, double* p) { return dev_pack_tril_rows(rows, n, f, p); }
int qemb_op_jacobi_eigh(int64_t n, double* A, double* w, double* V, int* sweeps) { return dev_jacobi_eigh(n, A, w, V, sweeps); }
int qemb_op_scf_fused_max(void) { return dev_scf_fused_max(); }
int qemb_op_jacobi_eigh_in_basis(int64_t n, const double* F, const double* Cp, double* w, double* C_out, double* C2_out, int nocc, double* dm_out, double stop_below, int* sweeps) {
  DBuf st;
  QTRY(st.alloc(1));
  QTRY(dev_jacobi_eigh_in_basis(n, F, Cp, w, C_out, C2_out, nocc, dm_out, stop_below, reinterpret_cast<int*>(st.p)));
  double word = 0.0;
  QTRY(dev_d2h(&word, st.p, sizeof(double)));
  int sw; std::memcpy(&sw, &word, sizeof(int));
  if (sweeps) *sweeps = sw;
  return jacobi_status_code(sw, "dev_jacobi_eigh_in_basis");
}
int qemb_op_scf_fock_small(int64_t n, const double* h, const double* J, const double* K, const double* D, double* F, double* err, double* scal2) { return dev_scf_fock_small(n, h, J, K, D, F, err, scal2); }
int qemb_op_pack_density_sym(int64_t n, const double* D, double* Dp) { return dev_pack_density_sym(n, D, Dp); }
int qemb_op_jacobi_svd(int64_t m, int64_t n, double* G, double* s, double* U, double* V, int* sweeps) { return dev_jacobi_svd(m, n, G, s, U, V, sweeps); }
int qemb_op_cholesky_lower(int64_t n, double* A) { return dev_cholesky_lower(n, A); }
static thread_local int64_t g_joint_diag_limit = -1;
int qemb_op_joint_diag_mem_limit(int64_t bytes) { g_joint_diag_limit = bytes; return QEMB_OK; }
int qemb_op_joint_diag_bytes(int64_t K, int64_t m, int64_t* bytes, int* in_lds) {
  if (K < 0 || m < 0 || !bytes) { set_error("qemb_op_joint_diag_bytes: bad arguments"); return QEMB_ERR_ARG; }
  *bytes = (int64_t)loc::footprint_bytes(K, m);
  if (in_lds) *in_lds = loc::in_lds(K, m) ? 1 : 0;
  return QEMB_OK;
}
static int joint_diag_guard(const char* who, int64_t K, int64_t m, double extra_bytes, double to_allocate) {
  size_t free_b = 0, total_b = 0;
  QTRY(dev_mem_info(&free_b, &total_b));
  const double need = loc::footprint_bytes(K, m) + extra_bytes;
  if ((g_joint_diag_limit >= 0 && need > (double)g_joint_diag_limit) || to_allocate > (double)free_b) {
    set_error(std::string(who) + ": with K = " + std::to_string(K) + " and m = " + std::to_string(m) + " the stack, U and the workspace take " + std::to_string(need * 1e-9) +
              " GB (" + std::to_string(to_allocate * 1e-9) + " GB still to allocate), more than the " +
              std::to_string((g_joint_diag_limit >= 0 && (double)g_joint_diag_limit < (double)free_b ? (double)g_joint_diag_limit : (double)free_b) * 1e-9) + " GB they may take");
    return QEMB_ERR_ALLOC;
  }
  return QEMB_OK;
}
int qemb_op_joint_diag(int64_t K, int64_t m, double* Q_dev, double* U_dev, double stop_angle, int max_sweeps, int* sweeps, double* f, int* converged) {
  QTRY(loc::check_joint_diag("qemb_op_joint_diag", K, m, Q_dev != nullptr, U_dev != nullptr, stop_angle, max_sweeps));
  QTRY(joint_diag_guard("qemb_op_joint_diag", K, m, 0.0, 8.0 * (double)loc::work_doubles(K, m)));
  return dev_joint_diag(K, m, Q_dev, U_dev, stop_angle, max_sweeps, sweeps, f, converged);
}
int qemb_df_localize_er(qemb_df_t df, const double* C_host, int m, double stop_angle, int max_sweeps, double* U_host, int* sweeps, double* f_before, double* f_after, int* converged) {
  if (!df || !C_host || !U_host) { set_error("qemb_df_localize_er: null argument"); return QEMB_ERR_ARG; }
  const DfContext* d = reinterpret_cast<const DfContext*>(df);
  if (d->Usp.p || d->Lpq_im.p) { set_error("qemb_df_localize_er: a semi-sparse or periodic context holds no dense real 3-index tensor"); return QEMB_ERR_UNSUPPORTED; }
  if ((!d->Linv.p && !d->identity_metric) || !d->Lpq.p || d->N <= 0 || d->naux <= 0) { set_error("qemb_df_localize_er: metric and 3-index integrals must be set"); return QEMB_ERR_ARG; }
  if (m <= 0 || m > d->N) { set_error("qemb_df_localize_er: need 0 < m <= N"); return QEMB_ERR_ARG; }
  const int64_t K = d->naux, N = d->N, np = (int64_t)m * (m + 1) / 2;
  QTRY(loc::check_joint_diag("qemb_df_localize_er", K, m, true, true, stop_angle, max_sweeps));
  const double transform_b = 8.0 * ((double)K * m * N + (double)K * m * m + (d->identity_metric ? 1.0 : 2.0) * (double)K * np + (double)N * m);
  QTRY(joint_diag_guard("qemb_df_localize_er", K, m, transform_b, transform_b + loc::footprint_bytes(K, m)));
  DBuf dC, bb, Q, U;
  QTRY(dC.alloc(N * m));
  QTRY(dev_h2d(dC, C_host, sizeof(double) * N * m));
  QTRY(d->transform(dC, m, nullptr, nullptr, 0.0, &bb));
  QTRY(Q.alloc(K * m * m));
  QTRY(dev_unpack_tril_rows(K, m, bb, Q));
  bb.release();
  QTRY(U.alloc((int64_t)m * m));
  int cv0 = 0;
  QTRY(dev_joint_diag(K, m, Q, U, stop_angle, 0, nullptr, f_before, &cv0));
  QTRY(dev_joint_diag(K, m, Q, U, stop_angle, max_sweeps, sweeps, f_after, converged));
  return dev_d2h(U_host, U, sizeof(double) * m * m);
}

int qemb_op_tri_inverse_lower(int64_t n, const double* L, double* Linv) { return dev_tri_inverse_lower(n, L, Linv); }
int qemb_op_boys(int m_max, int64_t n, const double* x, double* out) { QTRY(dev_boys(m_max, n, x, out)); return dev_sync(); }
int qemb_op_int4c_class(int la, int lb, int lc, int ld, const void* bf_a, const void* bf_b, const void* bf_c, const void* bf_d, const double* c2s, double* out_host) {
  const int l[4] = {la, lb, lc, ld};
  const BfRecord* const rec[4] = {reinterpret_cast<const BfRecord*>(bf_a), reinterpret_cast<const BfRecord*>(bf_b), reinterpret_cast<const BfRecord*>(bf_c), reinterpret_cast<const BfRecord*>(bf_d)};
  return int4c_block(l, rec, c2s, out_host);
}
int qemb_op_int3c_class(int la, int lb, int lP, const void* bf_a, const void* bf_b, const void* bf_P, const double* c2s, double* out_host) {
  return int3c_block(la, lb, lP, reinterpret_cast<const BfRecord*>(bf_a), reinterpret_cast<const BfRecord*>(bf_b), reinterpret_cast<const BfRecord*>(bf_P), c2s, out_host);
}
int qemb_op_mp2_amplitudes(int64_t o, int64_t v, const double* ovov, const double* eo, const double* ev, double* t2, double* G, double* e_host) {
  DBuf part, e;
  QTRY(part.alloc(dev_mp2_partial_count(o, v))); QTRY(e.alloc(1));
  QTRY(dev_mp2_amplitudes(o, v, ovov, eo, ev, t2, G, part, e));
  return e_host ? dev_d2h(e_host, e, sizeof(double)) : dev_sync();
}

int qemb_op_rdm2_assemble(int kind, int64_t o, int64_t v, const double* t1, const double* t2, const double* dm1c, double* out) {
  QTRY(dev_rdm2_assemble(kind, o, v, t1, t2, dm1c, out));
  return dev_sync();
}

int qemb_op_rdm2_add_nc(int64_t m, const double* g, double alpha, double* X) { return dev_rdm2_add_nc(m, g, alpha, X); }
int qemb_op_rdm2_symmetrize(int64_t m, const double* g, double* X) { return dev_rdm2_symmetrize(m, g, X); }
int qemb_op_rdm2_eri_dot(int64_t m, int sym, const double* eri, const double* K, double* e_host) {
  if (!e_host) { set_error("qemb_op_rdm2_eri_dot: e_host is NULL"); return QEMB_ERR_ARG; }
  DBuf w;
  QTRY(w.alloc(rdm2_full_grid(m > 0 ? m : 1) + 1));
  QTRY(dev_rdm2_eri_dot(m, sym, eri, K, w.p + 1, w.p));
  return dev_d2h(e_host, w.p, sizeof(double));
}

int qemb_op_kdf_split(int64_t rows, int64_t nao, const double* z, double* planes) { QTRY(dev_kdf_split(rows, nao, z, planes)); return dev_sync(); }
int qemb_op_kdf_stack(int64_t nk, int64_t nao, int64_t n, const double* ta, double* Cs, double* Dk) { QTRY(dev_kdf_stack(nk, nao, n, ta, Cs, Dk)); return dev_sync(); }
int qemb_op_kdf_pack(int64_t naux, int64_t n, const double* M, int paired, double w, double* F, int64_t ldf, double* out2_host) {
  if (!out2_host) { set_error("qemb_op_kdf_pack: out2_host is NULL"); return QEMB_ERR_ARG; }
  DBuf wk;
  QTRY(wk.alloc(dev_kdf_partial_count(naux > 0 ? naux : 1, n > 0 ? n : 1) + 2));
  QTRY(dev_kdf_pack(naux, n, M, paired, w, F, ldf, wk.p + 2, wk.p));
  return dev_d2h(out2_host, wk.p, 2 * sizeof(double));
}

void qemb_default_opts(qemb_solver_opts* o) {
  CcsdOptions c; ScfOptions s;
  memset(o, 0, sizeof *o);
  o->struct_size = (uint32_t)sizeof(qemb_solver_opts);
  o->cc_conv_tol = c.conv_tol; o->cc_conv_tol_normt = c.conv_tol_normt; o->cc_max_cycle = c.max_cycle; o->cc_diis_space = c.diis_space;
  o->scf_conv_tol = s.conv_tol; o->scf_conv_tol_grad = s.conv_tol_grad; o->scf_max_cycle = s.max_cycle; o->scf_diis_space = s.diis_space;
  o->warm_start = 0; o->verbose = 0;
  LambdaOptions l;
  o->relax_density = 0; o->lambda_conv_tol = l.conv_tol; o->lambda_max_cycle = l.max_cycle;
  o->strict_convergence = 1;
}
static FragmentOptions to_opts(const qemb_solver_opts* o) {
  FragmentOptions f;
  if (o) {
    f.cc.conv_tol = o->cc_conv_tol; f.cc.conv_tol_normt = o->cc_conv_tol_normt; f.cc.max_cycle = o->cc_max_cycle;
    f.cc.diis_space = o->cc_diis_space; f.cc.verbose = o->verbose;
    f.scf.conv_tol = o->scf_conv_tol; f.scf.conv_tol_grad = o->scf_conv_tol_grad; f.scf.max_cycle = o->scf_max_cycle;
    f.scf.diis_space = o->scf_diis_space; f.scf.verbose = o->verbose;
    f.warm_start = o->warm_start;
    f.relax_density = o->relax_density; f.lam.conv_tol = o->lambda_conv_tol; f.lam.max_cycle = o->lambda_max_cycle;
    f.lam.diis_space = o->cc_diis_space; f.lam.verbose = o->verbose;
    f.strict = o->strict_convergence;
  }
  return f;
}
#define CHECK_OPTS(o)                                                                                                     \
  do {                                                                                                                    \
    if ((o) && (o)->struct_size != (uint32_t)sizeof(qemb_solver_opts)) {                                                  \
      set_error("qemb_solver_opts.struct_size is " + std::to_string((o)->struct_size) + ", this library expects " +       \
                std::to_string(sizeof(qemb_solver_opts)) + ": initialise the struct with qemb_default_opts() (binding built " \
                "against another qemb_hip.h?)");                                                                          \
      return QEMB_ERR_ARG;                                                                                                \
    }                                                                                                                     \
  } while (0)
#define FRAG(f) (reinterpret_cast<Fragment*>(f))
#define CHECK_FRAG(f) do { if (!(f)) { set_error("null fragment handle"); return QEMB_ERR_ARG; } } while (0)

int qemb_frag_create(int n, int n_f, qemb_frag_t* out) {
  if (n <= 0 || n_f < 0 || n_f > n || !out) { set_error("qemb_frag_create: bad arguments"); return QEMB_ERR_ARG; }
  *out = new Fragment(n, n_f);
  return QEMB_OK;
}
int qemb_frag_free(qemb_frag_t f) { delete FRAG(f); return QEMB_OK; }
int qemb_frag_set_eri_s4(qemb_frag_t f, const double* s4) { CHECK_FRAG(f); return FRAG(f)->set_eri_s4_host(s4); }
int qemb_frag_set_eri_s4_dev(qemb_frag_t f, const double* s4) { CHECK_FRAG(f); return FRAG(f)->set_eri_s4_dev(s4); }
int qemb_frag_set_df_factor(qemb_frag_t f, int naux, const double* B) { CHECK_FRAG(f); return FRAG(f)->set_df_factor_host(naux, B); }
int qemb_frag_set_df_factor_dev(qemb_frag_t f, int naux, const double* B) { CHECK_FRAG(f); return FRAG(f)->set_df_factor_dev(naux, B); }
int qemb_frag_set_df_only(qemb_frag_t f, int naux, const double* B) { CHECK_FRAG(f); return FRAG(f)->set_df_only_host(naux, B); }
int qemb_frag_set_df_only_dev(qemb_frag_t f, int naux, const double* B) { CHECK_FRAG(f); return FRAG(f)->set_df_only_dev(naux, B); }
int qemb_frag_resident_bytes(qemb_frag_t f, int64_t* bytes) { CHECK_FRAG(f); if (!bytes) { set_error("qemb_frag_resident_bytes: null argument"); return QEMB_ERR_ARG; } *bytes = FRAG(f)->resident_bytes(); return QEMB_OK; }
int qemb_frag_mo_route(qemb_frag_t f, int route) { CHECK_FRAG(f); return FRAG(f)->set_mo_route(route); }
int qemb_frag_mo_route_used(qemb_frag_t f, int* used_factor, int* naux) {
  CHECK_FRAG(f);
  if (used_factor) *used_factor = FRAG(f)->last_route_was_factor() ? 1 : 0;
  if (naux) *naux = FRAG(f)->df_naux();
  return QEMB_OK;
}
int qemb_frag_get_eri_s4(qemb_frag_t f, double* s4) {
  CHECK_FRAG(f);
  if (!s4) { set_error("qemb_frag_get_eri_s4: null buffer"); return QEMB_ERR_ARG; }
  return FRAG(f)->export_eri_s4(s4);
}
int qemb_frag_get_df_factor(qemb_frag_t f, double* B) {
  CHECK_FRAG(f);
  if (!B) { set_error("qemb_frag_get_df_factor: null buffer"); return QEMB_ERR_ARG; }
  return FRAG(f)->export_df_factor(B);
}
int qemb_frag_set_energy_data(qemb_frag_t f, const double* h1, const double* veff0, const double* veff, double weight,
                              const int* centers, int ncenter) {
  CHECK_FRAG(f);
  for (int i = 0; i < ncenter; ++i) if (centers[i] < 0 || centers[i] >= FRAG(f)->nf()) { set_error("centre index outside the fragment sites"); return QEMB_ERR_ARG; }
  FRAG(f)->set_energy_data(h1, veff0, veff, weight, centers, ncenter);
  return QEMB_OK;
}
int qemb_frag_jk(qemb_frag_t f, const double* P, double* J, double* K) { CHECK_FRAG(f); return FRAG(f)->hf_veff_from_dm(P, J, K); }
static void store_result(Fragment* fr, const FragmentResult& r, int rc, int f, bool e_total, double* e_frag, double* e, double* e_scf, double* ebe_hf, int* n_iter, int* scf_cycles) {
  if (n_iter) n_iter[f] = r.n_iter;
  if (scf_cycles) scf_cycles[f] = r.scf_cycles;
  fr->last_lambda_iters = r.lambda_iters;
  if (rc < 0) return;
  if (e_frag) for (int k = 0; k < 3; ++k) e_frag[3 * f + k] = r.e_frag[k];
  if (e) e[f] = e_total ? r.e_scf + r.e_corr_mo : r.e_corr_mo;
  if (e_scf) e_scf[f] = r.e_scf;
  if (ebe_hf) ebe_hf[f] = r.ebe_hf;
}
static int gather_batch(const char* name, int nfrag, const qemb_frag_t* frags, const int* nsocc, const double* const* h, const double* const* dm0, const qemb_solver_opts* opts,
                        double* const* mo_coeff, double* const* mo_energy, double* const* rdm1_emb, double* const* rdm1_mo, double* const* t1, double* const* t2,
                        std::vector<Fragment*>& frs, std::vector<int>& o, std::vector<const double*>& hs, std::vector<const double*>& dms, std::vector<Fragment::BatchOutputs>& outs) {
  if (nfrag < 0 || (nfrag > 0 && (!frags || !nsocc || !h))) { set_error(std::string(name) + ": bad arguments"); return QEMB_ERR_ARG; }
  CHECK_OPTS(opts);
  outs.assign(nfrag > 0 ? nfrag : 0, Fragment::BatchOutputs());
  for (int f = 0; f < nfrag; ++f) {
    if (!frags[f] || !h[f]) { set_error(std::string(name) + ": null fragment handle or h"); return QEMB_ERR_ARG; }
    for (int g = 0; g < f; ++g) if (frags[g] == frags[f]) { set_error(std::string(name) + ": the same fragment twice"); return QEMB_ERR_ARG; }
    frs.push_back(FRAG(frags[f])); o.push_back(nsocc[f]); hs.push_back(h[f]); dms.push_back(dm0 ? dm0[f] : nullptr);
    auto pick = [&](double* const* arr) { return arr ? arr[f] : nullptr; };
    outs[f].mo_coeff = pick(mo_coeff); outs[f].mo_energy = pick(mo_energy); outs[f].rdm1_emb = pick(rdm1_emb);
    outs[f].rdm1_mo = pick(rdm1_mo); outs[f].t1 = pick(t1); outs[f].t2 = pick(t2);
  }
  return QEMB_OK;
}
int qemb_frag_solve(qemb_frag_t f, int nsocc, const double* h, const double* dm0, const qemb_solver_opts* opts, int eeval,
                    double* mo_coeff, double* mo_energy, double* rdm1_emb, double* rdm1_mo, double* t1, double* t2,
                    double* e_frag, double* e_corr_mo, double* e_scf, double* ebe_hf, int* n_iter, int* scf_cycles) {
  CHECK_FRAG(f); CHECK_OPTS(opts);
  if (!h) { set_error("qemb_frag_solve: h is NULL"); return QEMB_ERR_ARG; }
  FragmentResult r;
  const int rc = FRAG(f)->solve(nsocc, h, dm0, to_opts(opts), eeval, &r, mo_coeff, mo_energy, rdm1_emb, rdm1_mo, t1, t2);
  store_result(FRAG(f), r, rc, 0, false, e_frag, e_corr_mo, e_scf, ebe_hf, n_iter, scf_cycles);
  return rc;
}
int qemb_frag_solve_batch(int nfrag, const qemb_frag_t* frags, const int* nsocc, const double* const* h, const double* const* dm0,
                          const qemb_solver_opts* opts, int eeval, double* const* mo_coeff, double* const* mo_energy,
                          double* const* rdm1_emb, double* const* rdm1_mo, double* const* t1, double* const* t2, double* e_frag,
                          double* e_corr_mo, double* e_scf, double* ebe_hf, int* n_iter, int* scf_cycles, int64_t* stats) {
  std::vector<Fragment*> frs; std::vector<int> o; std::vector<const double*> hs, dms; std::vector<Fragment::BatchOutputs> outs;
  QTRY(gather_batch("qemb_frag_solve_batch", nfrag, frags, nsocc, h, dm0, opts, mo_coeff, mo_energy, rdm1_emb, rdm1_mo, t1, t2, frs, o, hs, dms, outs));
  std::vector<FragmentResult> res;
  LockstepStats st;
  const int rc = Fragment::solve_batch(frs, o, hs, dms, to_opts(opts), eeval, res, outs, &st);
  for (int f = 0; f < (int)res.size(); ++f) store_result(frs[f], res[f], rc, f, false, e_frag, e_corr_mo, e_scf, ebe_hf, n_iter, scf_cycles);
  if (stats) { stats[0] = st.merged_runs; stats[1] = st.launches; stats[2] = st.grouped; stats[3] = st.operations; stats[4] = st.max_group; }
  return rc;
}
int qemb_frag_solve_mp2(qemb_frag_t f, int nsocc, const double* h, const double* dm0, const qemb_solver_opts* opts, int eeval,
                        double* mo_coeff, double* mo_energy, double* rdm1_emb, double* rdm1_mo, double* t2, double* e_frag,
                        double* e_corr_mo, double* e_scf, double* ebe_hf, int* scf_cycles) {
  CHECK_FRAG(f); CHECK_OPTS(opts);
  if (!h) { set_error("qemb_frag_solve_mp2: h is NULL"); return QEMB_ERR_ARG; }
  FragmentResult r;
  const int rc = FRAG(f)->solve_mp2(nsocc, h, dm0, to_opts(opts), eeval, &r, mo_coeff, mo_energy, rdm1_emb, rdm1_mo, t2);
  store_result(FRAG(f), r, rc, 0, false, e_frag, e_corr_mo, e_scf, ebe_hf, nullptr, scf_cycles);
  return rc;
}
int qemb_frag_solve_mp2_batch(int nfrag, const qemb_frag_t* frags, const int* nsocc, const double* const* h, const double* const* dm0,
                              const qemb_solver_opts* opts, int eeval, double* const* mo_coeff, double* const* mo_energy,
                              double* const* rdm1_emb, double* const* rdm1_mo, double* const* t2, double* e_frag, double* e_corr_mo,
                              double* e_scf, double* ebe_hf, int* scf_cycles) {
  std::vector<Fragment*> frs; std::vector<int> o; std::vector<const double*> hs, dms; std::vector<Fragment::BatchOutputs> outs;
  QTRY(gather_batch("qemb_frag_solve_mp2_batch", nfrag, frags, nsocc, h, dm0, opts, mo_coeff, mo_energy, rdm1_emb, rdm1_mo, nullptr, t2, frs, o, hs, dms, outs));
  std::vector<FragmentResult> res;
  const int rc = Fragment::solve_mp2_batch(frs, o, hs, dms, to_opts(opts), eeval, res, outs);
  for (int f = 0; f < (int)res.size(); ++f) store_result(frs[f], res[f], rc, f, false, e_frag, e_corr_mo, e_scf, ebe_hf, nullptr, scf_cycles);
  return rc;
}
void qemb_default_fci_opts(qemb_fci_opts* o) {
  FciOptions d;
  memset(o, 0, sizeof *o);
  o->struct_size = (uint32_t)sizeof(qemb_fci_opts);
  o->conv_tol = d.conv_tol; o->max_cycle = d.max_cycle; o->max_space = d.max_space; o->lindep = d.lindep;
}
int qemb_frag_solve_fci(qemb_frag_t f, int nsocc, const double* h, const double* dm0, const qemb_solver_opts* opts, const qemb_fci_opts* fci_opts, int eeval,
                        double* mo_coeff, double* mo_energy, double* rdm1_emb, double* rdm1_mo, double* civec, double* e_frag, double* e_fci, double* e_scf,
                        double* ebe_hf, int* n_iter, int* scf_cycles) {
  CHECK_FRAG(f); CHECK_OPTS(opts);
  if (fci_opts && fci_opts->struct_size != (uint32_t)sizeof(qemb_fci_opts)) {
    set_error("qemb_fci_opts.struct_size is " + std::to_string(fci_opts->struct_size) + ", this library expects " + std::to_string(sizeof(qemb_fci_opts)) +
              ": initialise the struct with qemb_default_fci_opts()");
    return QEMB_ERR_ARG;
  }
  if (!h) { set_error("qemb_frag_solve_fci: h is NULL"); return QEMB_ERR_ARG; }
  FciOptions fo;
  if (fci_opts) { fo.conv_tol = fci_opts->conv_tol; fo.max_cycle = fci_opts->max_cycle; fo.max_space = fci_opts->max_space; fo.lindep = fci_opts->lindep; }
  FragmentResult r;
  const int rc = FRAG(f)->solve_fci(nsocc, h, dm0, to_opts(opts), fo, eeval, &r, mo_coeff, mo_energy, rdm1_emb, rdm1_mo, civec);
  store_result(FRAG(f), r, rc, 0, true, e_frag, e_fci, e_scf, ebe_hf, n_iter, scf_cycles);
  return rc;
}
int qemb_frag_fci_bytes(int n, int nsocc, int max_space, int64_t* bytes) {
  if (n <= 0 || nsocc <= 0 || nsocc > n || max_space < 2 || !bytes) { set_error("qemb_frag_fci_bytes: bad arguments"); return QEMB_ERR_ARG; }
  if (n > kFciMaxOrb) { set_error("qemb_frag_fci_bytes: n = " + std::to_string(n) + " embedding orbitals; the determinant-space solver takes at most " + std::to_string(kFciMaxOrb)); return QEMB_ERR_UNSUPPORTED; }
  *bytes = fci_bytes(n, nsocc, max_space);
  return QEMB_OK;
}
int qemb_frag_fci_mem_limit(qemb_frag_t f, int64_t bytes) { CHECK_FRAG(f); FRAG(f)->set_fci_mem_limit(bytes); return QEMB_OK; }
int qemb_frag_fci_residual(qemb_frag_t f, double* residual) { CHECK_FRAG(f); if (residual) *residual = FRAG(f)->fci_residual(); return QEMB_OK; }
int qemb_op_fci_links(int n, int nsocc, int64_t* ns, int* nlink, int32_t* strings_host, int32_t* links_host) {
  const FciTables* T = nullptr;
  QTRY(fci_tables(n, nsocc, &T));
  if (ns) *ns = T->ns;
  if (nlink) *nlink = T->nlink;
  if (strings_host) std::memcpy(strings_host, T->strings.data(), sizeof(int32_t) * T->strings.size());
  if (links_host) std::memcpy(links_host, T->links.data(), sizeof(int32_t) * T->links.size());
  return QEMB_OK;
}
int qemb_op_fci_sigma(int n, int nsocc, const double* h_host, const double* V_dev, const double* c_dev, double* sigma_dev) {
  if (!h_host || !V_dev || !c_dev || !sigma_dev) { set_error("qemb_op_fci_sigma: null argument"); return QEMB_ERR_ARG; }
  const FciTables* T = nullptr;
  QTRY(fci_tables(n, nsocc, &T));
  const int64_t n2 = (int64_t)n * n, N = T->ndet();
  std::vector<double> Vh((size_t)(n2 * n2)), kh((size_t)n2);
  QTRY(dev_d2h(Vh.data(), V_dev, sizeof(double) * n2 * n2));
  fci_one_body(n, h_host, Vh.data(), kh.data());
// ... 557 lines not shown
```

### quemb_amd/csrc/dev_ops.h

```cpp
#pragma once
#include <cstddef>
#include <cstdint>
#include <string>
#include "../../include/qemb_hip_ops.h"
#include "gemm_tiles.h"
#include "env.h"

namespace qemb {

void set_error(const std::string& msg);
const char* last_error();

#define QTRY(expr)              \
  do {                          \
    int _rc = (expr);           \
    if (_rc != 0) return _rc;   \
  } while (0)


int dev_init(int device);
int dev_sync();
int dev_sync_device();
int dev_ctx_count(int n);
int dev_ctx_bind(int k);
int dev_ctx_partition(int parts);
int dev_alloc(void** p, size_t bytes);
int dev_free(void* p);
int dev_trim();
int dev_trim_all();
int dev_h2d(void* dst, const void* src_host, size_t bytes);
int dev_h2d_async(void* dst, const void* src, size_t bytes);
int dev_d2h(void* dst_host, const void* src, size_t bytes);
int dev_d2h_async(void* dst_pinned, const void* src, size_t bytes);
int dev_pinned_alloc(void** p, size_t bytes);
int dev_pinned_free(void* p);
int dev_d2d(void* dst, const void* src, size_t bytes);
int dev_fill(double* x, int64_t n, double value);
int dev_mem_info(size_t* free_b, size_t* total_b);
int dev_alloc_stats(long long* n_driver_allocs, long long* n_driver_frees, double* ms_in_driver_calls, double* gb_allocated, int reset);
const char* dev_backend_name();

typedef void* dev_graph_t;
int dev_graph_begin(int for_tape = 0);
int dev_region_begin();
int dev_region_chain();
int dev_region_end();
int dev_graph_end(dev_graph_t* out);
int dev_graph_launch(dev_graph_t g);
int dev_graph_destroy(dev_graph_t g);
bool dev_capturing();
typedef void* dev_tape_t;
int dev_tape_end(dev_tape_t* out);
int dev_tape_run(const dev_tape_t* tapes, int n);
int dev_tape_destroy(dev_tape_t t);
int dev_tape_equal(dev_tape_t a, dev_tape_t b);
void dev_alloc_trace_begin();
unsigned long long dev_alloc_trace_end();
int dev_tape_last_stats(long long* launches, long long* grouped, long long* operations);

int dev_timer_begin(int slot);
int dev_timer_end(int slot);
int dev_timer_read(int slot, double* total_ms, int64_t* count);
int dev_timer_reset(int slot);
int dev_ctx_timer_read(int ctx, int slot, double* total_ms, int64_t* count, int reset);
int dev_timer_live_events(int slot);
enum { TIMER_LADDER = 0, TIMER_RINGS = 1, TIMER_ITER = 2, TIMER_AO2MO = 3, TIMER_SCF = 4,
       TIMER_GEMM_ANY = 5, TIMER_SCHMIDT = 6, TIMER_DF = 7, TIMER_NSLOTS = 16 };
struct TimerScope {
  int slot; bool open;
  explicit TimerScope(int s) : slot(s), open(dev_timer_begin(s) == 0) {}
  int close() { if (!open) return 0; open = false; return dev_timer_end(slot); }
  ~TimerScope() { if (open) (void)dev_timer_end(slot); }
  TimerScope(const TimerScope&) = delete;
  TimerScope& operator=(const TimerScope&) = delete;
};

struct GemmDesc {
  int64_t M, N, K;
  double alpha, beta;
  const double* A; int64_t lda; int a_kcontig; int64_t strideA;
  const double* B; int64_t ldb; int b_kcontig; int64_t strideB;
  double* C; int64_t ldc; int64_t strideC;
  int64_t batch;
  int cfg = -1;
  int ksplit = 0;
  int keep_slabs = 0;
  int64_t a_slab = 0, a_slab_skip = 0;
};
inline int gemm_slab_count(int64_t K, int ksplit) {
  if (ksplit <= 1 || K <= 0) return 1;
  int64_t chunk = (K + ksplit - 1) / ksplit;
  chunk = (chunk + 31) / 32 * 32;
  const int64_t S = (K + chunk - 1) / chunk;
  return S > 1 ? (int)S : 1;
}
inline int gemm_auto_ksplit(int64_t tiles, int64_t K) {
  if (tiles >= 256 || K < 1024) return 0;
  int64_t S = (768 + tiles - 1) / tiles;
  if (S > K / 256) S = K / 256;
  return S > 1 ? (int)S : 0;
}
struct GemmPlan {
  int64_t M = 0, N = 0, K = 0;
  int cfg = -1, ks = 0, S = 1;
  GemmPlan() = default;
  GemmPlan(int64_t m, int64_t n, int64_t k, int cfg_, int ks_) : M(m), N(n), K(k), cfg(cfg_), ks(ks_), S(gemm_slab_count(k, ks_)) {}
  int64_t elems() const { return (int64_t)S * M * N; }
};
int dev_gemm(const GemmDesc& g);
inline const char* gemm_desc_error(const GemmDesc& d) {
  if (d.a_slab <= 0 && d.lda < (d.a_kcontig ? d.K : d.M)) return "dev_gemm: lda is smaller than the contiguous extent of A";
  if (d.ldb < (d.b_kcontig ? d.K : d.N)) return "dev_gemm: ldb is smaller than the contiguous extent of B";
  if (!d.keep_slabs && d.ldc < d.N) return "dev_gemm: ldc is smaller than N";
  if (d.strideA < 0 || d.strideB < 0 || d.strideC < 0) return "dev_gemm: negative batch stride";
  return nullptr;
}
inline bool gemm_operand_vec2_ok(const double* p, int64_t ld, int64_t stride, int64_t contig_extent, bool kcontig, bool relaxed = true) {
  if (kcontig && relaxed) return (reinterpret_cast<uintptr_t>(p) & 7) == 0;
  return ((reinterpret_cast<uintptr_t>(p) & 15) == 0) && (ld % 2 == 0) && (stride % 2 == 0) && (contig_extent % 2 == 0);
}
inline bool gemm_desc_vec2(const GemmDesc& d, bool relaxed = true) {
  return gemm_operand_vec2_ok(d.A, d.lda, d.strideA, d.a_kcontig ? d.K : d.M, d.a_kcontig != 0, relaxed) &&
         gemm_operand_vec2_ok(d.B, d.ldb, d.strideB, d.b_kcontig ? d.K : d.N, d.b_kcontig != 0, relaxed);
}
inline bool gemm_wide_c(const double* C, int64_t ldc, int64_t N, int64_t strideC, int64_t nz) {
  return (ldc % 2 == 0) && (N % 2 == 0) && ((reinterpret_cast<uintptr_t>(C) & 15) == 0) && (nz <= 1 || strideC % 2 == 0);
}
struct GemmLaunchRecord { int cfg, vec2, mode, ksplit, sb_m, sb_n, wide_c; };
void dev_gemm_last_launch(GemmLaunchRecord* out);
int dev_gemm_flop_count(double* flops, int reset);
void dev_gemm_set_force_cfg(int cfg);
void dev_gemm_set_auto_splitk(int enabled);
int dev_gemm_probe(const GemmDesc& g, double* ms, double* ghz, long long* workgroups);
int dev_gemm_stamps(const GemmDesc& g, int waves_per_wg, double* out7);

struct Copy4Desc {
  int64_t dim[4];
  const double* in; int64_t si[4];
  double* out; int64_t so[4];
  double alpha, beta;
  const double* base = nullptr;
  double* out2 = nullptr; const double* in2 = nullptr; double c2a = 0.0, c2b = 0.0;
};
int dev_copy4(const Copy4Desc& c);

struct Outer4Desc {
  int64_t dim[4];
  const double* u; int64_t su0, su2;
  const double* v; int64_t sv1, sv3;
  double* out; int64_t so[4];
  double alpha, beta;
  const double* base = nullptr;
};
int dev_outer4(const Outer4Desc& c);
int dev_lincomb(int64_t n, int nterms, const double* coef, const double* const* xs, double beta, double* out);

int dev_div_denom(double* x, int64_t d0, int64_t d1, int64_t d2, int64_t d3,
                  const double* ea, const double* eb, const double* ec, const double* ed);

int dev_mirror_lower(int64_t n, double* A, int64_t lda);

int dev_k_from_pairs(int64_t n, const double* H, const double* D, double* K);
int dev_jk_from_packed(int64_t n, const double* S4, const double* D, const double* Dp, double* Jp, double* K);

int dev_pack_pair_rows(int64_t n, int64_t ncols, const double* in, double* out);
int dev_extract_pf(int64_t n, const double* Mp, int64_t p0, int64_t q0, int64_t r0, int64_t s0, int64_t sp, int64_t sq,
                   int64_t sr, int64_t ss, double* out);
int dev_extract_pf_t(int64_t n, const double* T, int64_t x0, int64_t r0, int64_t s0, int64_t c0, int64_t sx, int64_t sr,
                     int64_t ss, int64_t sc, double* out, int64_t slab = 0);
int dev_ladder_pack_vvvv_pf(int64_t n, int64_t o, const double* Mp, double* Vp, int64_t ldp, double* Vm, int64_t ldm);
int dev_extract_pf_t_compact(int64_t n, const double* T, int64_t x0, int64_t c0, int64_t sx, int64_t sr, int64_t ss, int64_t sc, double* out, int64_t slab = 0);
int dev_gather_pair_cols(int64_t rows, int64_t n, const double* in, int64_t r0, int64_t s0, int64_t sr, int64_t ss, double* out);
int dev_extract_ps(int64_t n, const double* S, int64_t p0, int64_t q0, int64_t r0, int64_t s0, int64_t sp, int64_t sq, int64_t sr, int64_t ss, double* out);
int dev_extract_ps_packed(int64_t n, const double* S, int64_t p0, int64_t q0, int64_t r0, int64_t sp, int64_t sq, int64_t sr, double* out);
int dev_unpack_pair_block(int64_t n, int64_t o, const double* S, double* Mv, int64_t ld);
int dev_ladder_pack_vvvv_pf_ld(int64_t n, int64_t o, const double* Mp, int64_t ld, double* Vp, int64_t ldp, double* Vm, int64_t ldm);

int dev_ladder_pack_vvvv(int64_t n, int64_t o, const double* M, double* Vp, int64_t ldp, double* Vm, int64_t ldm);
int dev_ladder_pack_tau(int64_t o, int64_t v, const double* tau, double* Tp, int64_t ldp, double* Tm, int64_t ldm);
int dev_pack_pm_cols(int64_t rows, int64_t v, const double* in, double* Op, int64_t ldp, double* Om, int64_t ldm);
int dev_pack_pm_ovvv(int64_t o, int64_t v, const double* ovvv, double* Op, int64_t ldp, double* Om, int64_t ldm);
int dev_scatter_pm_rows(int64_t o, int64_t ncols, const double* Xp, const double* Xm, double* out, const double* add = nullptr, int Sp = 1, int64_t strideP = 0,
                        int Sm = 1, int64_t strideM = 0);
int dev_ccsd_finish_t2(int64_t o, int64_t v, double* t2n, const double* U, const double* OV, const double* eo, const double* ev);
int dev_ccsd_finish_t2_rings(int64_t o, int64_t v, double* t2n, const double* U, const double* OV, const double* RS, const double* M, const double* eo, const double* ev, double* t1n);
int dev_ladder_scatter_pm(int64_t o, int64_t v, const double* Rp, int64_t ldp, const double* Rm, int64_t ldm, double* t2);
int dev_ladder_scatter_pm2(int64_t o, int64_t v, const double* Rp, int64_t ldp, const double* Rm, int64_t ldm, const double* Hp, const double* Hm,
                           int assign, double* t2, int Sp = 1, int64_t strideP = 0, int Sm = 1, int64_t strideM = 0, int64_t ldhp = 0, int64_t ldhm = 0);
int dev_pack_w_pm(int64_t o, const double* W, double* Ap, int64_t lda_p, double* Am, int64_t lda_m);
int dev_pack_w_pm_sum(int64_t o, const double* Wt, const double* X, const double* At, double* Ap, int64_t lda_p, double* Am, int64_t lda_m);
int dev_ccsd_t1_small(int64_t o, int64_t v, const double* t1, const double* Lvv, const double* Loo, const double* Fov, double* t1n);
int dev_ccsd_t1_assemble(int64_t o, int64_t v, const double* t1, const double* Lvv, const double* Loo, const double* Fov, const double* S, const double* Lph1,
                         const double* PA, int SA, int64_t strideA, const double* PB, int SB, int64_t strideB, double* t1n);
int dev_gemv_rows_two(int64_t rows1, int64_t cols1, const double* T1, int64_t ld1, const double* x1, double* y1, double a1, double b1,
                      int64_t rows2, int64_t cols2, const double* T2, int64_t ld2, const double* x2, double* y2, double a2, double b2);
int dev_gemv_rows2(int64_t rows, int64_t cols, const double* T1, int64_t ld1, const double* x1, const double* T2, int64_t ld2, const double* x2, double* y, double alpha, double beta);
int dev_foo_from_x(int64_t o, const double* X, double* F);
int dev_ccsd_ph_layouts(int64_t o, int64_t v, const double* t2, const double* t1, double* T, double* Tp, double* S, double* Ut, double* Tpt, double* Th);
int dev_small_k_update(int64_t batch, int64_t M, int64_t N, int64_t K, double alpha, const double* A, int64_t sA, const double* B, int64_t sB,
                       double* C, int64_t sC);
int dev_ccsd_y_traces(int64_t o, int64_t v, const double* ZC, const double* ZB, double* Y, const double* add = nullptr, int S = 1, int64_t stride = 0, double scale = 1.0);

inline int64_t dev_mp2_partial_count(int64_t o, int64_t v) {
  const int64_t nt = (v + 31) / 32, oo = o * o;
  return nt * (nt + 1) / 2 * (oo < 4096 ? oo : 4096);
}
int dev_mp2_amplitudes(int64_t o, int64_t v, const double* ovov, const double* eo, const double* ev, double* t2, double* G, double* partials, double* e_dev);

inline int rdm2_check_args(int kind, int64_t o, int64_t v, const double* t1, const double* t2, const double* out) {
  if (kind != QEMB_RDM2_CCSD && kind != QEMB_RDM2_MP2) { set_error("dev_rdm2_assemble: kind must be QEMB_RDM2_CCSD or QEMB_RDM2_MP2"); return QEMB_ERR_ARG; }
  if (o <= 0 || v < 0 || !out || (v > 0 && (!t2 || (kind == QEMB_RDM2_CCSD && !t1)))) { set_error("dev_rdm2_assemble: bad arguments"); return QEMB_ERR_ARG; }
  if (o + v > 32767) { set_error("dev_rdm2_assemble: n = " + std::to_string(o + v) + " is beyond any n^4 tensor"); return QEMB_ERR_ARG; }
  return 0;
}
int dev_rdm2_assemble(int kind, int64_t o, int64_t v, const double* t1, const double* t2, const double* dm1c, double* out);
inline int64_t rdm2_full_grid(int64_t m) { return m * m < 4096 ? m * m : 4096; }
inline int rdm2_check_full(int64_t m, const void* a, const void* b) {
  if (m <= 0 || m > 32767 || !a || !b) { set_error("rdm2 full-basis pass: bad arguments (N = " + std::to_string(m) + ")"); return QEMB_ERR_ARG; }
  return 0;
}
int dev_rdm2_add_nc(int64_t m, const double* g, double alpha, double* X);
int dev_rdm2_symmetrize(int64_t m, const double* g, double* X);
int dev_rdm2_eri_dot(int64_t m, int sym, const double* eri, const double* K, double* partials, double* out_dev);

constexpr int kFciMaxOrb = 16;
constexpr int64_t kFciMaxDet = (int64_t)12870 * 12870;
inline int fci_check_args(const char* who, int n, int64_t ns, int nlink, const void* a, const void* b, const void* c) {
  if (n <= 0 || n > kFciMaxOrb || ns <= 0 || ns > 12870 || nlink <= 0 || nlink > kFciMaxOrb * kFciMaxOrb || !a || !b || !c) {
    set_error(std::string(who) + ": bad arguments (n = " + std::to_string(n) + ", strings = " + std::to_string(ns) + ")");
    return QEMB_ERR_ARG;
  }
  return 0;
}
int dev_fci_gather(int n, int64_t ns, int nlink, const int32_t* links, const double* c, double* D);
int dev_fci_sigma(int n, int64_t ns, int nlink, const int32_t* links, const double* k, const double* D, const double* G, double* sigma);
int dev_fci_diag(int n, int64_t ns, const int32_t* strings, const double* h, const double* V, double* hdiag);
int dev_fci_precond(int64_t N, const double* r, const double* hdiag, double theta, double* out);
int dev_fci_dm2(int n, int o_cum, const double* A, const double* dm1, double* out);

inline int64_t kdf_ld(int64_t nao) { return (nao + 15) / 16 * 16; }
int dev_kdf_split(int64_t rows, int64_t nao, const double* z, double* planes);
int dev_kdf_stack(int64_t nk, int64_t nao, int64_t n, const double* ta, double* Cs, double* Dk);
inline int64_t dev_kdf_partial_count(int64_t naux, int64_t n) {
  const int64_t nt = (n + 31) / 32;
  return 2 * (nt * (nt + 1) / 2) * (naux < 1024 ? naux : 1024);
}
inline int kdf_check_pack(int64_t naux, int64_t n, const void* M, const void* F, int64_t ldf, const void* partials, const void* out2) {
  if (naux <= 0 || n <= 0 || n > 32767 || !M || !F || !partials || !out2 || ldf < n * (n + 1) / 2) { set_error("dev_kdf_pack: bad arguments"); return QEMB_ERR_ARG; }
  return 0;
}
int dev_kdf_pack(int64_t naux, int64_t n, const double* M, int paired, double w, double* F, int64_t ldf, double* partials, double* out2_dev);

int dev_boys(int m_max, int64_t n, const double* x, double* out);
namespace int3c { struct ClassArgs; }
int dev_int3c_class(int la, int lb, int lp, const int3c::ClassArgs& args);

namespace int1e { struct Args; }
int dev_int1e_class(int la, int lb, const int1e::Args& args);

namespace int4c { struct PairArgs; struct ClassArgs; }
int dev_int4c_pairs(int la, int lb, const int4c::PairArgs& args);
int dev_int4c_class(int la, int lb, int lc, int ld, const int4c::ClassArgs& args);
namespace int4c { struct JkArgs; }
namespace int3c { struct Shell; }
int dev_int4c_jk_class(int la, int lb, int lc, int ld, const int4c::JkArgs& args);
int dev_int4c_dmax(const int3c::Shell* sh, int nshell, int64_t N, const double* dm, double* out);
namespace int4c { struct PairProdArgs; }
int dev_int4c_pairprod(const int4c::PairProdArgs& args);
int dev_int4c_add_transpose(int64_t m, double* A);

int dev_cd_gather_cols(int64_t rows, int64_t ncols, const double* in, int64_t ldi, const int32_t* idx, double* out, int64_t ldo);
int dev_joint_diag(int64_t K, int64_t m, double* Q, double* U, double stop_angle, int max_sweeps, int* sweeps, double* f, int* converged);
int dev_cd_panel_factor(const double* E, int64_t ld, const int32_t* srow, int n, double thr, const double* d, double* T, int32_t* piv, int32_t* rank, double* work);
int dev_cd_new_rows(int64_t np, int n, int r, const double* E, int64_t ld, const double* T, const int32_t* piv, double* Lnew, int64_t ldl);
int dev_cd_diag_update(int64_t np, int r, const double* Lnew, int64_t ldl, const int32_t* piv, const int32_t* srow, double* d, int64_t nsp, const int32_t* row0, const int32_t* cnt,
                       double* spmax, double* partials, double* dmax);
int dev_cd_unpack(int64_t M, int64_t N, const double* L, int64_t ld, const int32_t* pos, double* out);

int dev_threshold_mask(int64_t n, const double* x, double eps, double* out);
int dev_mul_bcast_rows(int64_t rows, int64_t cols, double* x, const double* m);

int dev_abs_overlap_prim(int nsh, const int* l, const double* ex, const double* xyz, const int64_t* cart0, int64_t ncart, int nroots,
                         const double* roots, const double* weights, double* out);

int dev_gather_rows(int64_t nrows, int64_t len, const int64_t* idx_dev, const double* src, int64_t ld, double* dst);
int dev_scale_rows(int64_t nrows, int64_t len, double* x, const double* s);

int dev_dot(int64_t n, const double* x, const double* y, double* out_dev);
int dev_absmax(int64_t n, const double* x, double* out_dev);
int dev_dot_many(int64_t n, const double* x, int m, const double* const* ys, double* out_dev);
int dev_diis_push(int64_t n, const double* trial, const double* prev, double* e, double* xcopy, int m, const double* const* ys, int self,
                  double* row_dev, double* row_host, void* flag_host = nullptr, unsigned long long seq = 0);
int dev_batch_begin();
int dev_batch_flush();
int dev_wait_flag(const void* flag_host, unsigned long long seq);
int dev_ccsd_extrapolate_energy(int64_t o, int64_t v, int nterms, const double* coef, const double* const* xs, double* amp, const double* L,
                                double* tau, double* e_dev, double* e_host, void* flag_host = nullptr, unsigned long long seq = 0);

int dev_gemv_rows(int64_t rows, int64_t cols, const double* T, int64_t ldt, const double* x,
                  double* y, double alpha, double beta);
int dev_gemv_rows_batched(int64_t rows, int64_t cols, int64_t nbatch, const double* T, int64_t ldt, int64_t strideT,
                          const double* x, int64_t stridex, double* y, double alpha, double beta);
int dev_contract_mid(int64_t outer, int64_t mid, int64_t inner, const double* T, const double* x,
                     double* Y, int64_t ldy, double alpha, double beta);

int dev_unpack_s4(int64_t n, const double* s4, double* s1);
int dev_pack_s4(int64_t n, const double* s1, double* s4);
int dev_unpack_s8_to_s4(int64_t n, const double* s8, double* s4);
int dev_unpack_tril_rows(int64_t rows, int64_t n, const double* packed, double* full);
int dev_unpack_tril_rows_ld(int64_t rows, int64_t n, int64_t ld, const double* packed, double* full);
int dev_pack_tril_rows(int64_t rows, int64_t n, const double* full, double* packed);
int dev_unpack_tril_pair_rows(int64_t nr, int64_t n, const double* in, double* full);
int dev_unpack_tril_pair_rows_ld(int64_t nr, int64_t n, int64_t ld, const double* in, double* full);

int dev_jacobi_eigh(int64_t n, double* A, double* w, double* V, int* sweeps_out);
int dev_jacobi_eigh_until(int64_t n, double* A, double* w, double* V, int* sweeps_out, double stop_below);
enum { JACOBI_STATUS_NOCONV = -1, JACOBI_STATUS_NONFINITE = -2 };
inline int jacobi_status_code(int st, const char* who) {
  if (st == JACOBI_STATUS_NONFINITE) { set_error(std::string(who) + ": the matrix holds a NaN or an infinity"); return QEMB_ERR_NUMERIC; }
  if (st < 0) { set_error(std::string(who) + ": Jacobi sweeps did not converge in 40 sweeps"); return QEMB_ERR_NOCONV; }
  return QEMB_OK;
}
int dev_scf_fused_max();
int dev_jacobi_eigh_in_basis(int64_t n, const double* F, const double* Cp, double* w, double* C_out, double* C2_out, int nocc, double* dm_out, double stop_below,
                             int* status_dev);
int dev_scf_fock_small(int64_t n, const double* h, const double* J, const double* K, const double* D, double* F, double* err, double* scal2);
int dev_pack_density_sym(int64_t n, const double* D, double* Dp);
int dev_jacobi_svd(int64_t m, int64_t n, double* G, double* s, double* U, double* V, int* sweeps_out);

enum { COMM_ID_BYTES = 128, COMM_SUM = 0, COMM_MAX = 1 };
int dev_comm_unique_id(void* id128);
int dev_comm_init(int rank, int world, const void* id128);
int dev_comm_info(int* rank, int* world);
int dev_comm_allreduce(double* host_buf, int64_t n, int op);
int dev_comm_destroy();

int dev_cholesky_lower(int64_t n, double* A);
int dev_tri_inverse_lower(int64_t n, const double* L, double* Linv);

}
```

### quemb_amd/csrc/gemm_f64.hip

```cpp
#include <hip/hip_runtime.h>
#include <algorithm>
#include <atomic>
#include <mutex>
#include <cstdint>
#include <cstdio>
#include <cstdlib>
#include <type_traits>
#include <vector>
#include "dev_ops.h"
#include "hip_common.h"
#include "grouped_launch.h"

namespace qemb {

typedef double d4 __attribute__((ext_vector_type(4)));
typedef double d2 __attribute__((ext_vector_type(2)));
typedef double d2u __attribute__((ext_vector_type(2), aligned(8)));

static thread_local int t_gemm_force_cfg = -1;
static thread_local int t_gemm_splitk_enabled = 1;
static std::atomic<long long> g_gemm_flops{0};
static thread_local GemmLaunchRecord t_gemm_last{};
void dev_gemm_last_launch(GemmLaunchRecord* out) { *out = t_gemm_last; }
int dev_gemm_flop_count(double* flops, int reset) { if (flops) *flops = (double)g_gemm_flops.load(); if (reset) g_gemm_flops = 0; return QEMB_OK; }
void dev_gemm_set_force_cfg(int cfg) { t_gemm_force_cfg = cfg; }
void dev_gemm_set_auto_splitk(int enabled) { t_gemm_splitk_enabled = enabled; }

struct GemmKArgs {
  const double* A; const double* B; double* C;
  long long lda, ldb, ldc, strideA, strideB, strideC;
  int M, N, K;
  int tiles_m, tiles_n;
  int ksplit, kchunk;
  double alpha, beta;
  long long* cyc2;
  long long* cyc;
  int sb_m, sb_n;
  int a_slab; long long a_slab_skip;
};

__device__ __forceinline__ int xcd_remap(int bid, int nwg) {
  const int q = nwg >> 3, r = nwg & 7;
  const int xcd = bid & 7, k = bid >> 3;
  const int base = (xcd < r) ? xcd * (q + 1) : r * (q + 1) + (xcd - r) * q;
  return base + k;
}

template <int BMN, int BK, bool KCONTIG>
struct LdsImage {
  static constexpr int PADK = 2;
  static constexpr int PADMN = (16 - (BMN % 32) + 32) % 32;
  static constexpr int LDK = BK + PADK;
  static constexpr int LDMN = BMN + PADMN;
  static constexpr int SIZE = KCONTIG ? BMN * LDK : BK * LDMN;
  __host__ __device__ static constexpr int off(int mn, int k) {
    return KCONTIG ? mn * LDK + k : k * LDMN + mn;
  }
};

template <int BMN, int BK, bool KCONTIG, int VEC, int T, int NCH>
__device__ __forceinline__ void stage_load(double (&reg)[NCH][VEC], const double* __restrict__ P,
                                           long long ld, int mn0, int k0, int MN, int K, int tid, int slab = 0, long long slab_skip = 0) {
  constexpr int CPR = (KCONTIG ? BK : BMN) / VEC;
  constexpr int TOTAL = BMN * BK / VEC;
#pragma unroll
  for (int c = 0; c < NCH; ++c) {
    const int chunk = tid + c * T;
    if ((TOTAL % T != 0) && chunk >= TOTAL) { reg[c][0] = 0.0; reg[c][VEC - 1] = 0.0; continue; }
    const int r = chunk / CPR;
    const int cc = (chunk % CPR) * VEC;
    const int mn = KCONTIG ? r : cc;
    const int k = KCONTIG ? cc : r;
    const int gmn = mn0 + mn, gk = k0 + k;
    long long g = KCONTIG ? (long long)gmn * ld + gk : (long long)gk * ld + gmn;
    if (!KCONTIG && slab > 0) g += (long long)(gmn / slab) * slab_skip;
    if constexpr (VEC == 2) {
      const bool ok = (gmn < MN) && (gk < K);
      d2 v = {0.0, 0.0};
      if (KCONTIG) {
        if (ok && gk + 1 < K) { const d2u u = *reinterpret_cast<const d2u*>(P + g); v[0] = u[0]; v[1] = u[1]; }
        else if (ok) v[0] = P[g];
      } else if (ok) v = *reinterpret_cast<const d2*>(P + g);
      reg[c][0] = v[0];
      reg[c][VEC - 1] = v[1];
    } else {
      const bool ok = (gmn < MN) && (gk < K);
      reg[c][0] = ok ? P[g] : 0.0;
    }
  }
}

template <int BMN, int BK, bool KCONTIG, int VEC, int T, int NCH>
__device__ __forceinline__ void stage_ptrs(const double* (&ptr)[NCH], const double* __restrict__ P, long long ld, int mn0, int k0, int MN, int tid, int slab = 0,
                                           long long slab_skip = 0) {
  constexpr int CPR = (KCONTIG ? BK : BMN) / VEC;
  constexpr int TOTAL = BMN * BK / VEC;
#pragma unroll
  for (int c = 0; c < NCH; ++c) {
    const int chunk = tid + c * T;
    if ((TOTAL % T != 0) && chunk >= TOTAL) { ptr[c] = P; continue; }
    const int r = chunk / CPR, cc = (chunk % CPR) * VEC;
    const int mn = KCONTIG ? r : cc, k = KCONTIG ? cc : r;
    int gmn = mn0 + mn;
    const int last = KCONTIG ? MN - 1 : MN - VEC;
    gmn = gmn < last ? gmn : (last > 0 ? last : 0);
    ptr[c] = KCONTIG ? P + (long long)gmn * ld + (k0 + k) : P + (long long)(k0 + k) * ld + gmn;
    if (!KCONTIG && slab > 0) ptr[c] += (long long)(gmn / slab) * slab_skip;
  }
}
template <int BMN, int BK, bool KCONTIG, int VEC, int T, int NCH>
__device__ __forceinline__ void stage_load_fast(double (&reg)[NCH][VEC], const double* (&ptr)[NCH], long long step, int tid) {
#pragma unroll
  for (int c = 0; c < NCH; ++c) {
    if constexpr (VEC == 2) {
      if constexpr (KCONTIG) { const d2u v = *reinterpret_cast<const d2u*>(ptr[c]); reg[c][0] = v[0]; reg[c][VEC - 1] = v[1]; }
      else { const d2 v = *reinterpret_cast<const d2*>(ptr[c]); reg[c][0] = v[0]; reg[c][VEC - 1] = v[1]; }
    } else {
      reg[c][0] = *ptr[c];
    }
    ptr[c] += ((BMN * BK / VEC) % T != 0 && (tid + c * T) >= BMN * BK / VEC) ? 0 : step;
  }
}

template <int BMN, int BK, bool KCONTIG, int VEC, int T, int NCH>
__device__ __forceinline__ void stage_store(const double (&reg)[NCH][VEC], double* __restrict__ S,
                                            int tid) {
  using Img = LdsImage<BMN, BK, KCONTIG>;
  constexpr int CPR = (KCONTIG ? BK : BMN) / VEC;
  constexpr int TOTAL = BMN * BK / VEC;
#pragma unroll
  for (int c = 0; c < NCH; ++c) {
    const int chunk = tid + c * T;
    if ((TOTAL % T != 0) && chunk >= TOTAL) continue;
    const int r = chunk / CPR;
    const int cc = (chunk % CPR) * VEC;
    const int mn = KCONTIG ? r : cc;
    const int k = KCONTIG ? cc : r;
    double* dst = S + Img::off(mn, k);
    if constexpr (VEC == 2) {
      d2 v = {reg[c][0], reg[c][VEC - 1]};
      *reinterpret_cast<d2*>(dst) = v;
    } else {
      dst[0] = reg[c][0];
    }
  }
}


template <int I, int N, class F>
__device__ __forceinline__ void static_for(F&& f) {
  if constexpr (I < N) { f(std::integral_constant<int, I>{}); static_for<I + 1, N>(f); }
}
__device__ __forceinline__ unsigned lds_byte_address(const double* p) {
  return (unsigned)(size_t)(__attribute__((address_space(3))) const double*)p;
}
template <int OFF>
__device__ __forceinline__ void lds_read_f64(double& dst, unsigned base) {
  static_assert(OFF >= 0 && OFF < 65536, "ds_read_b64 immediate offset");
  asm volatile("ds_read_b64 %0, %1 offset:%2" : "=v"(dst) : "v"(base), "n"(OFF));
}
template <int N>
__device__ __forceinline__ void lds_wait(double& x) {
  asm volatile("s_waitcnt lgkmcnt(%1)" : "+v"(x) : "n"(N));
}

template <int BMN, int BK, bool KCONTIG, int VEC, int T, int NCH, int C>
__device__ __forceinline__ void stage_store_chunk(const double (&reg)[NCH][VEC], double* __restrict__ S, int tid) {
  using Img = LdsImage<BMN, BK, KCONTIG>;
  constexpr int CPR = (KCONTIG ? BK : BMN) / VEC;
  constexpr int TOTAL = BMN * BK / VEC;
  const int chunk = tid + C * T;
  if ((TOTAL % T != 0) && chunk >= TOTAL) return;
  const int r = chunk / CPR;
  const int cc = (chunk % CPR) * VEC;
  const int mn = KCONTIG ? r : cc;
  const int k = KCONTIG ? cc : r;
  double* dst = S + Img::off(mn, k);
  if constexpr (VEC == 2) {
    d2 v = {reg[C][0], reg[C][VEC - 1]};
    *reinterpret_cast<d2*>(dst) = v;
  } else {
    dst[0] = reg[C][0];
  }
}

__device__ __forceinline__ double lane_swap_neighbour(double x) {
  const unsigned long long u = __double_as_longlong(x);
  const int lo = __builtin_amdgcn_update_dpp(0, (int)(u & 0xffffffffu), 0xB1, 0xF, 0xF, false);
  const int hi = __builtin_amdgcn_update_dpp(0, (int)(u >> 32), 0xB1, 0xF, 0xF, false);
  return __longlong_as_double((long long)(((unsigned long long)(unsigned)hi << 32) | (unsigned)lo));
}

template <int WM, int WN, int WAVES_M, int WAVES_N, int BK, bool A_KC, bool B_KC, int VEC, int TAG = 0, int MODE = 0>
__device__ __forceinline__ void dgemm_mfma_body(const uint3 BID, const uint3 GDIM, GemmKArgs g) {
  const long long t_start = g.cyc ? (long long)__builtin_amdgcn_s_memtime() : 0;
  constexpr int BM = WM * 16 * WAVES_M;
  constexpr int BN = WN * 16 * WAVES_N;
  constexpr int T = WAVES_M * WAVES_N * 64;
  using ImgA = LdsImage<BM, BK, A_KC>;
  using ImgB = LdsImage<BN, BK, B_KC>;
  constexpr int NCH_A = (BM * BK / VEC + T - 1) / T;
  constexpr int NCH_B = (BN * BK / VEC + T - 1) / T;
  static_assert(BK % 4 == 0, "BK must be a multiple of the MFMA K (4)");

  extern __shared__ __attribute__((aligned(16))) double smem[];
  double* sA0 = smem;
  double* sB0 = sA0 + ImgA::SIZE;
  double* sA1 = sB0 + ImgB::SIZE;
  double* sB1 = sA1 + ImgA::SIZE;

  const int tid = threadIdx.x;
  const int lane = tid & 63;
  const int wave = tid >> 6;
  const int wm = wave / WAVES_N, wn = wave % WAVES_N;

  const int ntiles = g.tiles_m * g.tiles_n;
  const int L = xcd_remap(BID.x, ntiles);
  int tm = L % g.tiles_m, tn = L / g.tiles_m;
  if (g.sb_m > 0) {
    const int per = g.sb_m * g.sb_n, sb = L / per, w = L - sb * per, nsbm = g.tiles_m / g.sb_m;
    tm = (sb % nsbm) * g.sb_m + w % g.sb_m;
    tn = (sb / nsbm) * g.sb_n + w / g.sb_m;
  }
  const int m0 = tm * BM, n0 = tn * BN;

  const long long bz = BID.y / g.ksplit;
  const int kslice = BID.y % g.ksplit;
  const int kbeg = kslice * g.kchunk;
  const int kend = (kbeg + g.kchunk < g.K) ? kbeg + g.kchunk : g.K;
  const double* __restrict__ A = g.A + bz * g.strideA;
  const double* __restrict__ B = g.B + bz * g.strideB;
  double* __restrict__ C = g.C + (long long)BID.y * g.strideC;

  d4 acc[WM][WN];
#pragma unroll
  for (int i = 0; i < WM; ++i)
#pragma unroll
    for (int j = 0; j < WN; ++j) acc[i][j] = d4{0.0, 0.0, 0.0, 0.0};

  constexpr int DA = (MODE == 0 && VEC == 2 && (WM * WN <= 8 || (WM == 6 && WN == 2))) ? 2 : 1;
  constexpr int DB = (MODE == 0 && VEC == 2 && WM < 14) ? 2 : 1;
  double ra[DA][NCH_A][VEC], rb[DB][NCH_B][VEC];
  const int nk = (kend - kbeg + BK - 1) / BK;

  const double* pa[NCH_A];
  const double* pb[NCH_B];
  stage_ptrs<BM, BK, A_KC, VEC, T, NCH_A>(pa, A, g.lda, m0, kbeg + BK, g.M, tid, g.a_slab, g.a_slab_skip);
  stage_ptrs<BN, BK, B_KC, VEC, T, NCH_B>(pb, B, g.ldb, n0, kbeg + BK, g.N, tid);
  const long long step_a = A_KC ? (long long)BK : (long long)BK * g.lda;
  const long long step_b = B_KC ? (long long)BK : (long long)BK * g.ldb;
  constexpr bool FAST = (VEC == 2);
  auto fetch_a = [&](double (&r)[NCH_A][VEC], int tt) {
    if (FAST && tt + 1 < nk) stage_load_fast<BM, BK, A_KC, VEC, T, NCH_A>(r, pa, step_a, tid);
    else if (tt < nk) stage_load<BM, BK, A_KC, VEC, T, NCH_A>(r, A, g.lda, m0, kbeg + tt * BK, g.M, kend, tid, g.a_slab, g.a_slab_skip);
  };
  auto fetch_b = [&](double (&r)[NCH_B][VEC], int tt) {
    if (FAST && tt + 1 < nk) stage_load_fast<BN, BK, B_KC, VEC, T, NCH_B>(r, pb, step_b, tid);
    else if (tt < nk) stage_load<BN, BK, B_KC, VEC, T, NCH_B>(r, B, g.ldb, n0, kbeg + tt * BK, g.N, kend, tid);
  };

  long long pst[4] = {0, 0, 0, 0};
  if constexpr (TAG == 2) pst[0] = __builtin_amdgcn_s_memtime();
  stage_load<BM, BK, A_KC, VEC, T, NCH_A>(ra[0], A, g.lda, m0, kbeg, g.M, kend, tid, g.a_slab, g.a_slab_skip);
  stage_load<BN, BK, B_KC, VEC, T, NCH_B>(rb[0], B, g.ldb, n0, kbeg, g.N, kend, tid);
  stage_store<BM, BK, A_KC, VEC, T, NCH_A>(ra[0], sA0, tid);
  stage_store<BN, BK, B_KC, VEC, T, NCH_B>(rb[0], sB0, tid);
  if constexpr (TAG == 2) pst[1] = __builtin_amdgcn_s_memtime();
  if (DA == 2 || MODE == 1) fetch_a(ra[DA - 1], 1);
  if (DB == 2 || MODE == 1) fetch_b(rb[DB - 1], 1);
  if constexpr (TAG == 2) pst[2] = __builtin_amdgcn_s_memtime();
  __syncthreads();
  if constexpr (TAG == 2) pst[3] = __builtin_amdgcn_s_memtime();

  const int fr = lane & 15, fk = lane >> 4;
  if constexpr (MODE == 1) {
    static_assert(VEC == 2, "MODE 1 uses the vector staging path");
    constexpr int NKS = BK / 4;
    static_assert(NKS >= 2 && NKS % 2 == 0, "the B fragment sets alternate per k-step");
    const unsigned ldsA[2] = {lds_byte_address(sA0 + ImgA::off(wm * WM * 16 + fr, fk)), lds_byte_address(sA1 + ImgA::off(wm * WM * 16 + fr, fk))};
    const unsigned ldsB[2] = {lds_byte_address(sB0 + ImgB::off(wn * WN * 16 + fr, fk)), lds_byte_address(sB1 + ImgB::off(wn * WN * 16 + fr, fk))};
    double a[WM], b[2][WN];
    static_for<0, WN>([&](auto j) { lds_read_f64<ImgB::off(decltype(j)::value * 16, 0) * 8>(b[0][decltype(j)::value], ldsB[0]); });
    static_for<0, WM>([&](auto i) { lds_read_f64<ImgA::off(decltype(i)::value * 16, 0) * 8>(a[decltype(i)::value], ldsA[0]); });
    long long st_work = 0, st_bar = 0, st_last = 0, st_t0 = 0;
    auto kstep = [&](auto ks_c, auto p_c, auto&& after_row) {
      constexpr int KS = decltype(ks_c)::value, P = decltype(p_c)::value;
      constexpr int S = KS & 1;
      constexpr int KSn = (KS + 1) % NKS, Pn = (KS + 1 < NKS) ? P : 1 - P;
      static_for<0, WN>([&](auto j) { lds_read_f64<ImgB::off(decltype(j)::value * 16, KSn * 4) * 8>(b[S ^ 1][decltype(j)::value], ldsB[Pn]); });
      static_for<0, WM>([&](auto i) {
        constexpr int I = decltype(i)::value;
        constexpr int NW = WM + WN - 1;
        if constexpr (I == 0) static_for<0, WN>([&](auto j) { lds_wait<NW>(b[S][decltype(j)::value]); });
        lds_wait<NW>(a[I]);
#pragma unroll
        for (int j = 0; j < WN; ++j) acc[I][j] = __builtin_amdgcn_mfma_f64_16x16x4f64(a[I], b[S][j], acc[I][j], 0, 0, 0);
        if constexpr (!((TAG == 4 || TAG == 5) && (I & 1)))
          lds_read_f64<ImgA::off(I * 16, KSn * 4) * 8>(a[I], ldsA[Pn]);
        after_row(ks_c, i);
      });
    };
    constexpr int NCH = NCH_A + NCH_B, NSLOT = WM;
    auto tile = [&](auto parity, int kt) {
      constexpr int P = decltype(parity)::value;
      double* nA = P ? sA0 : sA1;
      double* nB = P ? sB0 : sB1;
      auto stores = [&](auto ks_c, auto i_c) {
        constexpr int KS = decltype(ks_c)::value, I = decltype(i_c)::value;
        if constexpr (KS == NKS - 2) {
          constexpr int slot = I;
          static_for<0, NCH>([&](auto c_c) {
            constexpr int C = decltype(c_c)::value;
            if constexpr ((C * NSLOT) / NCH == slot) {
              if constexpr (C < NCH_A) stage_store_chunk<BM, BK, A_KC, VEC, T, NCH_A, C>(ra[0], nA, tid);
              else stage_store_chunk<BN, BK, B_KC, VEC, T, NCH_B, C - NCH_A>(rb[0], nB, tid);
            }
          });
        }
      };
      long long ts0 = 0;
      if constexpr (TAG == 2) ts0 = __builtin_amdgcn_s_memtime();
      static_for<0, NKS - 1>([&](auto ks) { kstep(ks, parity, stores); });
      if constexpr (TAG != 3 && TAG != 5) {
        fetch_a(ra[0], kt + 2);
        fetch_b(rb[0], kt + 2);
      }
      long long ts1 = 0;
      if constexpr (TAG == 2) ts1 = __builtin_amdgcn_s_memtime();
      __syncthreads();
      if constexpr (TAG == 2) { const long long ts2 = __builtin_amdgcn_s_memtime(); st_work += ts1 - ts0; st_bar += ts2 - ts1; st_t0 = ts2; }
      kstep(std::integral_constant<int, NKS - 1>{}, parity, stores);
      if constexpr (TAG == 2) st_last += __builtin_amdgcn_s_memtime() - st_t0;
    };
    for (int kt = 0; kt < nk; kt += 2) {
      tile(std::integral_constant<int, 0>{}, kt);
      if (kt + 1 < nk) tile(std::integral_constant<int, 1>{}, kt + 1);
    }
    if constexpr (TAG == 2) {
      if (g.cyc && lane == 0) {
        long long* o = g.cyc + (((long long)BID.y * GDIM.x + BID.x) * (WAVES_M * WAVES_N) + wave) * 4;
        o[0] = st_work; o[1] = st_bar; o[2] = st_last; o[3] = (long long)__builtin_amdgcn_s_memtime() - t_start;
        if (g.cyc2) { long long* q = g.cyc2 + (((long long)BID.y * GDIM.x + BID.x) * (WAVES_M * WAVES_N) + wave) * 4; q[0] = pst[0] - t_start; q[1] = pst[1] - pst[0]; q[2] = pst[2] - pst[1]; q[3] = pst[3] - pst[2]; }
      }
    }
    static_for<0, WN>([&](auto j) { lds_wait<0>(b[0][decltype(j)::value]); lds_wait<0>(b[1][decltype(j)::value]); });
    static_for<0, WM>([&](auto i) { lds_wait<0>(a[decltype(i)::value]); });
  } else {
    auto step = [&](auto parity, int kt) {
      constexpr int P = decltype(parity)::value;
      const double* sA = P ? sA1 : sA0;
      const double* sB = P ? sB1 : sB0;
      double* nA = P ? sA0 : sA1;
      double* nB = P ? sB0 : sB1;
      fetch_a(ra[DA == 2 ? P : 0], kt + DA);
      fetch_b(rb[DB == 2 ? P : 0], kt + DB);
#pragma unroll
      for (int ks = 0; ks < BK / 4; ++ks) {
        const int kk = ks * 4 + fk;
        double a[WM], b[WN];
#pragma unroll
        for (int j = 0; j < WN; ++j) b[j] = sB[ImgB::off((wn * WN + j) * 16 + fr, kk)];
#pragma unroll
        for (int i = 0; i < WM; ++i) a[i] = sA[ImgA::off((wm * WM + i) * 16 + fr, kk)];
#pragma unroll
        for (int i = 0; i < WM; ++i)
#pragma unroll
          for (int j = 0; j < WN; ++j)
            acc[i][j] = __builtin_amdgcn_mfma_f64_16x16x4f64(a[i], b[j], acc[i][j], 0, 0, 0);
      }
      if (kt + 1 < nk) {
        stage_store<BM, BK, A_KC, VEC, T, NCH_A>(ra[DA == 2 ? 1 - P : 0], nA, tid);
        stage_store<BN, BK, B_KC, VEC, T, NCH_B>(rb[DB == 2 ? 1 - P : 0], nB, tid);
      }
      __syncthreads();
    };
    for (int kt = 0; kt < nk; kt += 2) {
      step(std::integral_constant<int, 0>{}, kt);
      if (kt + 1 < nk) step(std::integral_constant<int, 1>{}, kt + 1);
    }

  }

  const double alpha = g.alpha, beta = g.beta;
  const bool wide = ((g.ldc & 1) == 0) && ((g.N & 1) == 0) && ((reinterpret_cast<uintptr_t>(C) & 15) == 0);
  if (wide) {
    const bool odd = (fr & 1) != 0;
#pragma unroll
    for (int i = 0; i < WM; ++i) {
#pragma unroll
      for (int j = 0; j < WN; ++j) {
        const d4 v = acc[i][j];
        const double r0 = lane_swap_neighbour(odd ? v[0] : v[2]), r1 = lane_swap_neighbour(odd ? v[1] : v[3]);
        const d2 pa = odd ? d2{r0, v[2]} : d2{v[0], r0};
        const d2 pb = odd ? d2{r1, v[3]} : d2{v[1], r1};
        const int col = n0 + (wn * WN + j) * 16 + (fr & ~1);
        const int row = m0 + (wm * WM + i) * 16 + fk + (odd ? 8 : 0);
        if (col < g.N) {
          if (row < g.M) {
            d2* p = reinterpret_cast<d2*>(C + (long long)row * g.ldc + col);
            d2 o = {alpha * pa[0], alpha * pa[1]};
            if (beta != 0.0) { const d2 c = *p; o[0] += beta * c[0]; o[1] += beta * c[1]; }
            *p = o;
          }
          if (row + 4 < g.M) {
            d2* p = reinterpret_cast<d2*>(C + (long long)(row + 4) * g.ldc + col);
            d2 o = {alpha * pb[0], alpha * pb[1]};
            if (beta != 0.0) { const d2 c = *p; o[0] += beta * c[0]; o[1] += beta * c[1]; }
            *p = o;
          }
        }
      }
    }
  } else {
#pragma unroll
    for (int i = 0; i < WM; ++i) {
#pragma unroll
      for (int j = 0; j < WN; ++j) {
        const int col = n0 + (wn * WN + j) * 16 + fr;
#pragma unroll
        for (int r = 0; r < 4; ++r) {
          const int row = m0 + (wm * WM + i) * 16 + fk + 4 * r;
          if (row < g.M && col < g.N) {
            double* p = C + (long long)row * g.ldc + col;
            double v = alpha * acc[i][j][r];
            if (beta != 0.0) v += beta * (*p);
            *p = v;
          }
        }
      }
    }
  }
  if (TAG != 2 && g.cyc && threadIdx.x == 0) g.cyc[(long long)BID.y * GDIM.x + BID.x] = (long long)__builtin_amdgcn_s_memtime() - t_start;
  if (TAG == 2 && g.cyc && lane == 0) g.cyc[(long long)GDIM.x * GDIM.y * (WAVES_M * WAVES_N) * 4 + ((long long)BID.y * GDIM.x + BID.x) * (WAVES_M * WAVES_N) + wave] = (long long)__builtin_amdgcn_s_memtime() - t_start;
}

template <int WM, int WN, int WAVES_M, int WAVES_N, int BK, bool A_KC, bool B_KC, int VEC, int TAG = 0, int MODE = 0>
__global__ void __launch_bounds__(WAVES_M* WAVES_N * 64, (WM * WN <= 16) ? 2 : 1)
    dgemm_mfma_kernel(GemmKArgs g) {
  dgemm_mfma_body<WM, WN, WAVES_M, WAVES_N, BK, A_KC, B_KC, VEC, TAG, MODE>(block_id(), grid_dim(), g);
}
template <int WM, int WN, int WAVES_M, int WAVES_N, int BK, int MODE>
struct GroupableGemmTile {
  GroupableGemmTile() {
#define QEMB_REG(AK, BKC)                                                                                                                                                                      \
  register_groupable<dgemm_mfma_body<WM, WN, WAVES_M, WAVES_N, BK, AK, BKC, 2, 0, MODE>, WAVES_M * WAVES_N * 64>(dgemm_mfma_kernel<WM, WN, WAVES_M, WAVES_N, BK, AK, BKC, 2, 0, MODE>);       \
  register_groupable<dgemm_mfma_body<WM, WN, WAVES_M, WAVES_N, BK, AK, BKC, 1, 0, 0>, WAVES_M * WAVES_N * 64>(dgemm_mfma_kernel<WM, WN, WAVES_M, WAVES_N, BK, AK, BKC, 1, 0, 0>);
    QEMB_REG(true, true) QEMB_REG(true, false) QEMB_REG(false, true) QEMB_REG(false, false)
#undef QEMB_REG
  }
};
static const GroupableGemmTile<1, 1, 2, 2, 32, 0> reg_gemm_cfg2;
static const GroupableGemmTile<2, 2, 2, 2, 16, 1> reg_gemm_cfg1;
static const GroupableGemmTile<4, 1, 2, 2, 16, 0> reg_gemm_cfg20;
static const GroupableGemmTile<1, 4, 2, 2, 16, 0> reg_gemm_cfg21;

__device__ __forceinline__ void splitk_reduce_kernel_body(const uint3 BID, const uint3 GDIM, const double* __restrict__ ws, int S, long long M, long long N,
                                                            double* __restrict__ C, long long ldc, long long strideC,
                                                            double alpha, double beta) {
  const long long mn = M * N;
  const long long b = BID.y;
  for (long long t = (long long)BID.x * blockDim.x + threadIdx.x; t < mn; t += (long long)GDIM.x * blockDim.x) {
    double acc = 0.0;
    const double* p = ws + b * S * mn + t;
    int s = 0;
    for (; s + 8 <= S; s += 8) {
      double x[8];
#pragma unroll
      for (int q = 0; q < 8; ++q) x[q] = p[(long long)(s + q) * mn];
#pragma unroll
      for (int q = 0; q < 8; ++q) acc += x[q];
    }
    for (; s < S; ++s) acc += p[(long long)s * mn];
    const long long m = t / N, n = t - m * N;
    double* c = C + b * strideC + m * ldc + n;
    *c = (beta != 0.0) ? alpha * acc + beta * (*c) : alpha * acc;
  }
}
__global__ void __launch_bounds__(256) splitk_reduce_kernel(const double* __restrict__ ws, int S, long long M, long long N,
                                                            double* __restrict__ C, long long ldc, long long strideC,
                                                            double alpha, double beta) { splitk_reduce_kernel_body(block_id(), grid_dim(), ws, S, M, N, C, ldc, strideC, alpha, beta); }
static const Groupable<splitk_reduce_kernel_body, 256> reg_splitk_reduce(splitk_reduce_kernel);
__device__ __forceinline__ void splitk_reduce_wave_kernel_body(const uint3 BID, const uint3 GDIM, const double* __restrict__ ws, int S, long long M, long long N,
                                                                 double* __restrict__ C, long long ldc, long long strideC,
                                                                 double alpha, double beta) {
  const long long mn = M * N;
  const long long b = BID.y;
  const int lane = threadIdx.x & 63;
  const long long wave = ((long long)BID.x * blockDim.x + threadIdx.x) >> 6, nwaves = ((long long)GDIM.x * blockDim.x) >> 6;
  for (long long t = wave; t < mn; t += nwaves) {
    double acc = 0.0;
    const double* p = ws + b * S * mn + t;
    for (int s = lane; s < S; s += 64) acc += p[(long long)s * mn];
#pragma unroll
    for (int off = 32; off > 0; off >>= 1) acc += __shfl_down(acc, off, 64);
    if (lane == 0) {
      const long long m = t / N, n = t - m * N;
      double* c = C + b * strideC + m * ldc + n;
      *c = (beta != 0.0) ? alpha * acc + beta * (*c) : alpha * acc;
    }
  }
}
__global__ void __launch_bounds__(256) splitk_reduce_wave_kernel(const double* __restrict__ ws, int S, long long M, long long N,
                                                                 double* __restrict__ C, long long ldc, long long strideC,
                                                                 double alpha, double beta) { splitk_reduce_wave_kernel_body(block_id(), grid_dim(), ws, S, M, N, C, ldc, strideC, alpha, beta); }
static const Groupable<splitk_reduce_wave_kernel_body, 256> reg_splitk_reduce_wave(splitk_reduce_wave_kernel);

double* gemm_workspace(size_t bytes);
static long long* g_gemm_cyc = nullptr;
static long long g_gemm_cyc_cap = 0, g_gemm_cyc_blocks = 0;
static bool g_gemm_cyc_on = false;

template <int WM, int WN, int WAVES_M, int WAVES_N, int BK, bool A_KC, bool B_KC, int VEC, int TAG = 0, int MODE = 0>
static int launch_cfg(const GemmDesc& d, hipStream_t s) {
  constexpr int BM = WM * 16 * WAVES_M, BN = WN * 16 * WAVES_N;
  using ImgA = LdsImage<BM, BK, A_KC>;
  using ImgB = LdsImage<BN, BK, B_KC>;
  GemmKArgs g{};
  g.A = d.A; g.B = d.B; g.C = d.C;
  g.lda = d.lda; g.ldb = d.ldb; g.ldc = d.ldc;
  g.strideA = d.strideA; g.strideB = d.strideB; g.strideC = d.strideC;
  g.M = (int)d.M; g.N = (int)d.N; g.K = (int)d.K;
  g.tiles_m = (int)((d.M + BM - 1) / BM);
  g.tiles_n = (int)((d.N + BN - 1) / BN);
  g.alpha = d.alpha; g.beta = d.beta;
  g.cyc = nullptr; g.cyc2 = nullptr;
  g.sb_m = g.sb_n = 0;
  g.a_slab = 0; g.a_slab_skip = 0;
  if (d.a_slab > 0) {
    if (A_KC || d.batch != 1 || d.a_slab > 0x3fffffff || (VEC == 2 && (d.a_slab % 2 || d.a_slab_skip % 2))) { set_error("dev_gemm: a_slab needs a !a_kcontig A operand, batch = 1 and (16-byte loads) an even slab"); return QEMB_ERR_ARG; }
    g.a_slab = (int)d.a_slab; g.a_slab_skip = d.a_slab_skip;
  }
  {
    static const bool sb_on = env_flag("QEMB_GEMM_SB", true);
    if (sb_on && d.batch == 1 && d.ksplit <= 1 && g.tiles_m >= 8 && g.tiles_n >= 4 && ((long long)g.tiles_m * g.tiles_n) % 256 == 0) {
      long long best = -1;
      for (int sm = 1; sm <= 32; sm *= 2) {
        const int sn = 32 / sm;
        if (g.tiles_m % sm || g.tiles_n % sn) continue;
        const long long cost = (long long)sm * BM + (long long)sn * BN;
        if (best < 0 || cost < best) { best = cost; g.sb_m = sm; g.sb_n = sn; }
      }
      if (g.sb_m == 32) g.sb_m = g.sb_n = 0;
    }
  }
  g.ksplit = 1; g.kchunk = g.K > 0 ? g.K : 1;
  const long long tiles = (long long)g.tiles_m * g.tiles_n * d.batch;
  if (d.keep_slabs && (d.ksplit <= 1 || d.alpha != 1.0 || d.beta != 0.0 || d.batch != 1)) { set_error("dev_gemm: keep_slabs needs ksplit > 1, alpha = 1, beta = 0, batch = 1"); return QEMB_ERR_ARG; }
  const int want = d.ksplit > 1 ? d.ksplit : (d.ksplit == 0 && t_gemm_splitk_enabled) ? gemm_auto_ksplit(tiles, d.K) : 0;
  if (want > 1) {
    long long chunk = (d.K + want - 1) / want;
    chunk = (chunk + 31) / 32 * 32;
    const long long S = (d.K + chunk - 1) / chunk;
    if (S > 1 && S * d.batch <= 65535) { g.ksplit = (int)S; g.kchunk = (int)chunk; }
  }
  if (d.keep_slabs) {
    if (g.ksplit != gemm_slab_count(d.K, d.ksplit)) { set_error("dev_gemm: slab count mismatch"); return QEMB_ERR_ARG; }
    g.ldc = d.N; g.strideC = d.M * d.N;
  } else if (g.ksplit > 1) {
    double* ws = gemm_workspace(sizeof(double) * (size_t)d.batch * g.ksplit * d.M * d.N);
    if (!ws) return QEMB_ERR_ALLOC;
    g.C = ws; g.ldc = d.N; g.strideC = d.M * d.N; g.alpha = 1.0; g.beta = 0.0;
  }
  const size_t lds = 2 * (size_t)(ImgA::SIZE + ImgB::SIZE) * sizeof(double);
  auto kern = dgemm_mfma_kernel<WM, WN, WAVES_M, WAVES_N, BK, A_KC, B_KC, VEC, TAG, MODE>;
  static std::atomic<bool> attr_set{false};
  if (!attr_set) {
    HIP_TRY(hipFuncSetAttribute((const void*)kern, hipFuncAttributeMaxDynamicSharedMemorySize, (int)lds));
    attr_set = true;
  }
  dim3 grid((unsigned)(g.tiles_m * g.tiles_n), (unsigned)(d.batch * g.ksplit), 1);
  dim3 block(WAVES_M * WAVES_N * 64, 1, 1);
  t_gemm_last.mode = MODE; t_gemm_last.ksplit = g.ksplit; t_gemm_last.sb_m = g.sb_m; t_gemm_last.sb_n = g.sb_n;
  t_gemm_last.wide_c = gemm_wide_c(g.C, g.ldc, g.N, g.strideC, grid.y) ? 1 : 0;
  if (g_gemm_cyc_on && g_gemm_cyc && (long long)grid.x * grid.y * (TAG == 2 ? 72 : 1) <= g_gemm_cyc_cap) { g.cyc = g_gemm_cyc; g_gemm_cyc_blocks = (long long)grid.x * grid.y; if (TAG == 2) g.cyc2 = g_gemm_cyc + (long long)grid.x * grid.y * (WAVES_M * WAVES_N) * 5; }
  QTRY(launch("dev_gemm", kern, grid, block, lds, s, g));
  if (g.ksplit > 1 && !d.keep_slabs) {
    const long long mn = d.M * d.N;
    if (g.ksplit >= 128 && mn <= 65536) {
      const unsigned gx = (unsigned)((mn + 3) / 4 < 4096 ? (mn + 3) / 4 : 4096);
      return launch("dev_gemm", splitk_reduce_wave_kernel, dim3(gx, (unsigned)d.batch), dim3(256), 0, s, g.C, g.ksplit, d.M, d.N, d.C, d.ldc, d.strideC, d.alpha, d.beta);
    }
    const unsigned gx = (unsigned)((mn + 255) / 256 < 2048 ? (mn + 255) / 256 : 2048);
    return launch("dev_gemm", splitk_reduce_kernel, dim3(gx, (unsigned)d.batch), dim3(256), 0, s, g.C, g.ksplit, d.M, d.N, d.C, d.ldc, d.strideC, d.alpha, d.beta);
  }
  return QEMB_OK;
}

template <int WM, int WN, int WAVES_M, int WAVES_N, int BK, int TAG = 0, int MODE = 0>
static int launch_layout(const GemmDesc& d, hipStream_t s, bool vec2) {
  const bool a = d.a_kcontig != 0, b = d.b_kcontig != 0;
#define QEMB_GEMM_CASE(AK, BKC)                                                                \
  if (a == AK && b == BKC)                                                                      \
    return vec2 ? launch_cfg<WM, WN, WAVES_M, WAVES_N, BK, AK, BKC, 2, TAG, MODE>(d, s)          \
                : launch_cfg<WM, WN, WAVES_M, WAVES_N, BK, AK, BKC, 1, TAG, 0>(d, s);
  QEMB_GEMM_CASE(true, true)
  QEMB_GEMM_CASE(true, false)
  QEMB_GEMM_CASE(false, true)
  QEMB_GEMM_CASE(false, false)
#undef QEMB_GEMM_CASE
  return QEMB_ERR_ARG;
}

template <int ID, int TAG, int MODE>
static int launch_tile(const GemmDesc& d, hipStream_t s, bool vec2) {
  constexpr GemmTile t = gemm_tile(ID);
  static_assert(t.wm > 0, "not a tile of gemm_tiles.h");
  return launch_layout<t.wm, t.wn, t.waves_m, t.waves_n, t.bk, TAG, MODE>(d, s, vec2);
}

static bool gemm_vec2_relaxed() {
  static const bool relaxed = env_flag("QEMB_GEMM_VEC2_ODD", true);
  return relaxed;
}

template <int NACC>
__global__ void __launch_bounds__(256) mfma_f64_peak_kernel(double* out, int iters, double seed) {
  d4 acc[NACC];
  double a[NACC], b[4];
#pragma unroll
  for (int i = 0; i < NACC; ++i) {
    acc[i] = d4{0.0, 0.0, 0.0, 0.0};
    a[i] = seed * (1.0 + 0.37 * i) + 1e-3 * (double)((threadIdx.x * 2654435761u + i * 40503u) & 1023u) - 0.5;
  }
#pragma unroll
  for (int j = 0; j < 4; ++j) b[j] = seed * (0.5 - 0.21 * j) + 1e-3 * (double)((threadIdx.x * 40503u + j * 2654435761u) & 1023u) - 0.5;
  for (int it = 0; it < iters; ++it) {
#pragma unroll
    for (int i = 0; i < NACC; ++i) asm volatile("v_mfma_f64_16x16x4_f64 %0, %1, %2, %0" : "+v"(acc[i]) : "v"(a[i]), "v"(b[i & 3]));
  }
  double s = 0.0;
#pragma unroll
  for (int i = 0; i < NACC; ++i) s += acc[i][0] + acc[i][1] + acc[i][2] + acc[i][3];
  if (s == 12345.678) out[0] = s;
}
int dev_mfma_f64_peak(int iters, int blocks_per_cu, double* tflops) {
  hipStream_t s = hip_stream();
  if (!s) { set_error("libqemb_hip: call qemb_init(device) first"); return QEMB_ERR_DEVICE; }
  constexpr int NACC = 16;
  double* out = nullptr;
  HIP_TRY(hipMalloc((void**)&out, 64));
  hipEvent_t e0, e1;
  HIP_TRY(hipEventCreate(&e0)); HIP_TRY(hipEventCreate(&e1));
  const int grid = 256 * blocks_per_cu;
  QTRY(launch("dev_mfma_f64_peak", mfma_f64_peak_kernel<NACC>, dim3(grid), dim3(256), 0, s, out, 64, 0.731));
  HIP_TRY(hipEventRecord(e0, s));
  QTRY(launch("dev_mfma_f64_peak", mfma_f64_peak_kernel<NACC>, dim3(grid), dim3(256), 0, s, out, iters, 0.731));
  HIP_TRY(hipEventRecord(e1, s));
  HIP_TRY(hipEventSynchronize(e1));
  float ms = 0.f;
  HIP_TRY(hipEventElapsedTime(&ms, e0, e1));
  const double flop = 2.0 * 16 * 16 * 4 * (double)NACC * iters * 4.0 * grid;
  *tflops = flop / (ms * 1e-3) / 1e12;
  (void)hipEventDestroy(e0); (void)hipEventDestroy(e1); (void)hipFree(out);
  return QEMB_OK;
}

static int dev_gemm_dispatch(const GemmDesc& d);

int dev_gemm_probe(const GemmDesc& d, double* ms_out, double* ghz_out, long long* workgroups) {
  hipEvent_t t0, t1;
  if (dev_capturing() || hipEventCreate(&t0) != hipSuccess || hipEventCreate(&t1) != hipSuccess) { set_error("dev_gemm_probe: cannot time this launch"); return QEMB_ERR_DEVICE; }
  hipStream_t s = hip_stream();
  float ms = 0.f;
  if (!g_gemm_cyc) { g_gemm_cyc_cap = 1 << 20; if (hipMalloc((void**)&g_gemm_cyc, sizeof(long long) * g_gemm_cyc_cap) != hipSuccess) g_gemm_cyc = nullptr; }
  g_gemm_cyc_blocks = 0;
  g_gemm_cyc_on = true;
  (void)hipEventRecord(t0, s);
  const int rc = dev_gemm_dispatch(d);
  (void)hipEventRecord(t1, s);
  (void)hipEventSynchronize(t1);
  g_gemm_cyc_on = false;
  (void)hipEventElapsedTime(&ms, t0, t1);
  (void)hipEventDestroy(t0); (void)hipEventDestroy(t1);
  double ghz = 0.0;
  if (g_gemm_cyc && g_gemm_cyc_blocks > 0 && ms > 0) {
    std::vector<long long> h((size_t)g_gemm_cyc_blocks);
    if (hipMemcpy(h.data(), g_gemm_cyc, sizeof(long long) * h.size(), hipMemcpyDeviceToHost) == hipSuccess) {
      double sum = 0; for (long long c : h) sum += (double)c;
      ghz = sum / 256.0 / (ms * 1e6);
    }
  }
  if (ms_out) *ms_out = ms;
  if (ghz_out) *ghz_out = ghz;
  if (workgroups) *workgroups = g_gemm_cyc_blocks;
  return rc;
}

int dev_gemm_stamps(const GemmDesc& d, int waves_per_wg, double* out) {
  hipStream_t s = hip_stream();
  if (!g_gemm_cyc) { g_gemm_cyc_cap = 1 << 20; if (hipMalloc((void**)&g_gemm_cyc, sizeof(long long) * g_gemm_cyc_cap) != hipSuccess) { g_gemm_cyc = nullptr; set_error("dev_gemm_stamps: no buffer"); return QEMB_ERR_ALLOC; } }
  HIP_TRY(hipMemsetAsync(g_gemm_cyc, 0, sizeof(long long) * g_gemm_cyc_cap, s));
  hipEvent_t t0, t1;
  HIP_TRY(hipEventCreate(&t0)); HIP_TRY(hipEventCreate(&t1));
  g_gemm_cyc_blocks = 0; g_gemm_cyc_on = true;
  (void)hipEventRecord(t0, s);
  const int rc = dev_gemm_dispatch(d);
  (void)hipEventRecord(t1, s);
  (void)hipEventSynchronize(t1);
  g_gemm_cyc_on = false;
  float ms = 0.f; (void)hipEventElapsedTime(&ms, t0, t1);
  (void)hipEventDestroy(t0); (void)hipEventDestroy(t1);
  if (rc) return rc;
  const size_t nw_ = (size_t)g_gemm_cyc_blocks * waves_per_wg;
  std::vector<long long> h(nw_ * 9);
  HIP_TRY(hipMemcpy(h.data(), g_gemm_cyc, sizeof(long long) * h.size(), hipMemcpyDeviceToHost));
  double sum[5] = {0, 0, 0, 0, 0};
  for (size_t w = 0; w < nw_; ++w) { for (int k = 0; k < 4; ++k) sum[k] += (double)h[w * 4 + k]; sum[4] += (double)h[nw_ * 4 + w]; }
  const double nw = (double)nw_;
  for (int k = 0; k < 3; ++k) out[k] = nw > 0 ? sum[k] / nw : 0.0;
  out[4] = nw > 0 ? sum[3] / nw : 0.0;
  out[5] = nw > 0 ? sum[4] / nw : 0.0;
  out[6] = (double)g_gemm_cyc_blocks;
  for (int k = 0; k < 4; ++k) { double t = 0; for (size_t w = 0; w < nw_; ++w) t += (double)h[nw_ * 5 + w * 4 + k]; out[7 + k] = nw > 0 ? t / nw : 0.0; }
  out[3] = ms;
  return QEMB_OK;
}

int dev_gemm(const GemmDesc& d) {
  static const bool trace = env_flag("QEMB_GEMM_TRACE", false);
  if (!trace || dev_capturing()) return dev_gemm_dispatch(d);
  double ms = 0.0, ghz = 0.0; long long wg = 0;
  const int rc = dev_gemm_probe(d, &ms, &ghz, &wg);
  std::fprintf(stderr, "[qemb gemm] M=%lld N=%lld K=%lld batch=%lld a_kc=%d b_kc=%d cfg=%d beta=%g  %.4f ms  %.1f TF  wg-ticks/(256 CU x t) = %.2f GHz (%lld workgroups)\n",
               (long long)d.M, (long long)d.N, (long long)d.K, (long long)d.batch, (int)d.a_kcontig, (int)d.b_kcontig, d.cfg, d.beta, ms,
               ms > 0 ? 2.0 * d.M * d.N * d.K * d.batch / (ms * 1e9) : 0.0, ghz, wg);
  return rc;
}

static int dev_gemm_dispatch(const GemmDesc& d) {
  if (d.M <= 0 || d.N <= 0 || d.batch <= 0) return QEMB_OK;
  if (d.K < 0 || !d.A || !d.B || !d.C) { set_error("dev_gemm: bad arguments"); return QEMB_ERR_ARG; }
  if (d.M > 0x3fffffff || d.N > 0x3fffffff || d.K > 0x3fffffff) {
    set_error("dev_gemm: dimension too large"); return QEMB_ERR_ARG;
  }
  if (const char* bad = gemm_desc_error(d)) { set_error(bad); return QEMB_ERR_ARG; }
  hipStream_t s = hip_stream();
  g_gemm_flops += 2ll * d.M * d.N * d.K * d.batch;
  {
    static FILE* shapelog = [] { const char* e = env_str("QEMB_GEMM_SHAPELOG"); return e ? std::fopen(e, "w") : (FILE*)nullptr; }();
    if (shapelog) {
      static std::mutex mu;
      std::lock_guard<std::mutex> lock(mu);
      std::fprintf(shapelog, "%lld %lld %lld %lld %d %d %d %d\n", (long long)d.M, (long long)d.N, (long long)d.K, (long long)d.batch, (int)d.a_kcontig, (int)d.b_kcontig, d.cfg, d.ksplit);
      std::fflush(shapelog);
    }
  }
  const bool vec2 = gemm_desc_vec2(d, gemm_vec2_relaxed());
  const int64_t t128 = ((d.M + 127) / 128) * ((d.N + 127) / 128) * d.batch;
  const int64_t t64 = ((d.M + 63) / 64) * ((d.N + 63) / 64) * d.batch;
  const double w128 = (double)(((d.M + 127) / 128) * 128) * (double)(((d.N + 127) / 128) * 128);
  const double w64 = (double)(((d.M + 63) / 64) * 64) * (double)(((d.N + 63) / 64) * 64);
  int cfg;
  if (t128 >= 384) cfg = (w128 > 1.08 * w64) ? 1 : 0;
  else if (t64 >= 256) cfg = 1;
  else if (d.M >= 128 && d.N >= 128 && d.K >= 4096) cfg = 1;
  else cfg = 2;
  if (vec2 && fits_one_224_tile(d.N) && d.M >= 128 * 1024) cfg = GEMM_128x224;
  if (d.cfg >= 0) cfg = d.cfg;
  if (t_gemm_force_cfg >= 0) cfg = t_gemm_force_cfg;
  if (cfg >= 300) {
    static const bool diag = env_flag("QEMB_GEMM_DIAGNOSTICS", false);
    if (!diag) { set_error("dev_gemm: tile configs >= 300 are diagnostic instantiations (set QEMB_GEMM_DIAGNOSTICS=1 in a measurement run)"); return QEMB_ERR_ARG; }
  }
  t_gemm_last = GemmLaunchRecord{};
  t_gemm_last.cfg = cfg; t_gemm_last.vec2 = vec2 ? 1 : 0;
  switch (cfg) {
#define QEMB_IF_0(...)
#define QEMB_IF_1(...) __VA_ARGS__
#define QEMB_X(id, name, wm, wn, waves_m, waves_n, bk, mode1, classic) \
    case id: return launch_tile<id, 0, mode1>(d, s, vec2);             \
    QEMB_IF_##classic(case GEMM_CLASSIC + id: return launch_tile<id, 0, 0>(d, s, vec2);)
    QEMB_GEMM_TILES(QEMB_X)
#undef QEMB_X
#define QEMB_X(id, name) case id: return launch_tile<GEMM_##name, 1, 1>(d, s, vec2);
    QEMB_GEMM_LADDER_TWINS(QEMB_X)
#undef QEMB_X
#undef QEMB_IF_0
#undef QEMB_IF_1
    case 313: return launch_tile<GEMM_224x128, 2, 1>(d, s, vec2);
    case 315: return launch_tile<GEMM_192x128, 2, 1>(d, s, vec2);
    case 304: return launch_tile<GEMM_128x256, 2, 1>(d, s, vec2);
    case 413: return launch_tile<GEMM_224x128, 3, 1>(d, s, vec2);
    case 513: return launch_tile<GEMM_224x128, 4, 1>(d, s, vec2);
    case 613: return launch_tile<GEMM_224x128, 5, 1>(d, s, vec2);
    case 404: return launch_tile<GEMM_128x256, 3, 1>(d, s, vec2);
    case 504: return launch_tile<GEMM_128x256, 4, 1>(d, s, vec2);
    case 604: return launch_tile<GEMM_128x256, 5, 1>(d, s, vec2);
    default: set_error("dev_gemm: unknown tile config"); return QEMB_ERR_ARG;
  }
}

}
```

### quemb_amd/csrc/gemm_tiles.h

```cpp
#pragma once
#include <cstdint>

namespace qemb {

#define QEMB_GEMM_TILES(X)                                                                                                                                  \
  X(0, 128x128, 4, 4, 2, 2, 16, 1, 1)                                                                                                          \
  X(1, 64x64, 2, 2, 2, 2, 16, 1, 1)                                                                                                            \
  X(2, 32x32, 1, 1, 2, 2, 32, 0, 0)                                                                                                            \
  X(4, 128x256, 4, 4, 2, 4, 16, 1, 1)                                                             \
  X(10, 224x128_COL, 14, 1, 1, 8, 16, 0, 0)         \
  X(11, 112x128_COL, 7, 1, 1, 8, 16, 0, 0)                                                                                             \
  X(12, 64x128_COL, 4, 1, 1, 8, 16, 0, 0)                                                                                              \
  X(13, 224x128, 7, 2, 2, 4, 16, 1, 1)                                             \
  X(15, 192x128, 6, 2, 2, 4, 16, 1, 1)                                                    \
  X(20, 128x32, 4, 1, 2, 2, 16, 0, 0)                                              \
  X(21, 32x128, 1, 4, 2, 2, 16, 0, 0)                                                                                 \
  X(33, 112x128, 7, 2, 1, 4, 16, 1, 1)                                            \
  X(34, 128x224, 2, 7, 4, 2, 16, 1, 1)                                 \
  X(35, 160x128, 5, 2, 2, 4, 16, 1, 1)                                       \
  X(36, 80x128, 5, 2, 1, 4, 16, 1, 1)           \
  X(37, 96x96, 3, 3, 2, 2, 16, 1, 1)                 \
  X(38, 48x128, 3, 2, 1, 4, 16, 1, 0)
#define QEMB_GEMM_LADDER_TWINS(X) X(23, 224x128) X(25, 192x128)

enum : int {
#define QEMB_X(id, name, wm, wn, waves_m, waves_n, bk, mode1, classic) GEMM_##name = id,
  QEMB_GEMM_TILES(QEMB_X)
#undef QEMB_X
  GEMM_CLASSIC = 200
};

struct GemmTile { int wm, wn, waves_m, waves_n, bk, mode1; };
constexpr GemmTile gemm_tile(int cfg) {
  switch (cfg) {
#define QEMB_X(id, name, wm, wn, waves_m, waves_n, bk, mode1, classic) case id: return GemmTile{wm, wn, waves_m, waves_n, bk, mode1};
    QEMB_GEMM_TILES(QEMB_X)
#undef QEMB_X
    default: return GemmTile{0, 0, 0, 0, 0, 0};
  }
}
constexpr int gemm_tile_rows(int cfg) { return gemm_tile(cfg).wm * 16 * gemm_tile(cfg).waves_m; }
constexpr int gemm_tile_cols(int cfg) { return gemm_tile(cfg).wn * 16 * gemm_tile(cfg).waves_n; }
constexpr int64_t gemm_tile_count(int cfg, int64_t M, int64_t N) {
  return ((M + gemm_tile_rows(cfg) - 1) / gemm_tile_rows(cfg)) * ((N + gemm_tile_cols(cfg) - 1) / gemm_tile_cols(cfg));
}
constexpr int gemm_tile_ladder_symbol(int cfg) {
  switch (cfg) {
#define QEMB_X(id, name) case GEMM_##name: return id;
    QEMB_GEMM_LADDER_TWINS(QEMB_X)
#undef QEMB_X
    default: return cfg;
  }
}
struct GemmTileEntry { int id, rows, cols, bk, mode1, has_classic, ladder_twin; };
constexpr int gemm_tile_entries() {
#define QEMB_X(id, name, wm, wn, waves_m, waves_n, bk, mode1, classic) +1
  return 0 QEMB_GEMM_TILES(QEMB_X);
#undef QEMB_X
}
inline bool gemm_tile_entry(int index, GemmTileEntry* e) {
  static const GemmTileEntry table[] = {
#define QEMB_X(id, name, wm, wn, waves_m, waves_n, bk, mode1, classic) \
    {id, gemm_tile_rows(id), gemm_tile_cols(id), bk, mode1, classic, gemm_tile_ladder_symbol(id) != id ? gemm_tile_ladder_symbol(id) : -1},
    QEMB_GEMM_TILES(QEMB_X)
#undef QEMB_X
  };
  if (index < 0 || index >= gemm_tile_entries()) return false;
  *e = table[index];
  return true;
}
constexpr bool fits_one_224_tile(int64_t n) { return n > gemm_tile_rows(GEMM_192x128) && n <= gemm_tile_rows(GEMM_224x128); }

}
```

Measured before the change: 57.55.

## Compute DF pair product with lower-triangle-only symmetric GEMM tiles

```diff
diff --git a/include/qemb_hip_ops.h b/include/qemb_hip_ops.h
--- a/include/qemb_hip_ops.h
+++ b/include/qemb_hip_ops.h
@@ -37,6 +37,8 @@
 int qemb_op_gemm_stamps(int64_t M, int64_t N, int64_t K, const double* A, int64_t lda, const double* B, int64_t ldb, double* C, int64_t ldc, int cfg,
                         int ksplit, double* out7);
 int qemb_pair_gemm_choice(int64_t rows, int64_t cols, int* cfg, int* ksplit);
+int qemb_gemm_sym_tile_choice(int64_t M);
+int qemb_gemm_sym_tile_walk(int64_t M, int tile_rows, int tile_cols, int64_t workgroup, int64_t* count, int* tile_row, int* tile_col);
 int qemb_ccsd_gemm_plans(int o, int v, int64_t* out);
 int qemb_set_gemm_ksplit(int ksplit);
 int qemb_gemm_tile_table(int index, int* id, int* rows, int* cols, int* bk, int* mode1, int* has_classic, int* ladder_twin);
@@ -107,6 +109,7 @@
 int qemb_op_ladder_pack_vvvv_pf_ld(int64_t n, int64_t o, const double* Mp, int64_t ld, double* Vp, int64_t ldp, double* Vm, int64_t ldm);
 int qemb_op_pack_pm_ovvv(int64_t o, int64_t v, const double* ovvv, double* Op, int64_t ldp, double* Om, int64_t ldm);
 int qemb_op_df_pair_product(int64_t np, int64_t naux, const double* bb, double* out);
+int qemb_op_df_pair_product_rows(int64_t np, int64_t naux, const double* bbT, double* out);
 int qemb_op_unpack_tril_rows(int64_t rows, int64_t n, const double* packed, double* full);
 int qemb_op_pack_tril_rows(int64_t rows, int64_t n, const double* full, double* packed);
 int qemb_op_jacobi_eigh(int64_t n, double* A, double* w, double* V, int* sweeps);
diff --git a/quemb_amd/_lib.py b/quemb_amd/_lib.py
--- a/quemb_amd/_lib.py
+++ b/quemb_amd/_lib.py
@@ -75,6 +75,8 @@
     f("qemb_set_gemm_splitk", I, I)
     f("qemb_set_gemm_ksplit", I, I)
     f("qemb_pair_gemm_choice", I, L, L, C.POINTER(I), C.POINTER(I))
+    f("qemb_gemm_sym_tile_choice", I, L)
+    f("qemb_gemm_sym_tile_walk", I, L, I, I, L, C.POINTER(L), C.POINTER(I), C.POINTER(I))
     f("qemb_ccsd_gemm_plans", I, I, I, C.POINTER(L))
     f("qemb_gemm_tile_table", I, I, *([C.POINTER(I)] * 7))
     f("qemb_gemm_last_launch", I, *([C.POINTER(I)] * 7))
@@ -144,6 +146,7 @@
     f("qemb_op_ladder_pack_vvvv_pf_ld", I, L, L, P, L, P, L, P, L)
     f("qemb_op_pack_pm_ovvv", I, L, L, P, P, L, P, L)
     f("qemb_op_df_pair_product", I, L, L, P, P)
+    f("qemb_op_df_pair_product_rows", I, L, L, P, P)
     f("qemb_op_pack_tril_rows", I, L, L, P, P)
     f("qemb_op_jacobi_eigh", I, L, P, P, P, C.POINTER(I))
     f("qemb_op_scf_fused_max", I)
diff --git a/quemb_amd/csrc/ao2mo.cpp b/quemb_amd/csrc/ao2mo.cpp
--- a/quemb_amd/csrc/ao2mo.cpp
+++ b/quemb_amd/csrc/ao2mo.cpp
@@ -257,14 +257,7 @@
     QTRY(perm4(*keep_bb, bbT, 1, 1, np, naux, 0, 1, 3, 2));
   }
   if (!out_s4) return 0;
-  const int64_t nblk = np >= 2048 ? 8 : 1;
-  const int64_t w = ((np + nblk - 1) / nblk + 127) / 128 * 128;
-  for (int64_t c0 = 0; c0 < np; c0 += w) {
-    const int64_t cw = std::min(w, np - c0);
-    QTRY(gemm(np - c0, cw, naux, 1.0, bbT.p + c0 * naux, naux, true, bbT.p + c0 * naux, naux, true, 0.0, out_s4 + c0 * np + c0, np));
-  }
-  if (nblk > 1) QTRY(dev_mirror_lower(np, out_s4, np));
-  return 0;
+  return df_pair_product_rows(np, naux, bbT, out_s4);
 }
 
 int DfContext::transform_semisparse(const double* TA, int n, double* out_s4, const double* S_abs, double eps, DBuf* keep_bb) const {
@@ -470,15 +463,26 @@
   return dev_sync();
 }
 
-int df_pair_product(int64_t np, int64_t naux, const double* bb, double* out) {
+static int pair_product(int64_t np, int64_t naux, const double* f, int64_t ld, bool pair_rows, double* out) {
+  static const bool lower_tiles = env_flag("QEMB_PAIR_PRODUCT_TILES", true);
+  if (lower_tiles) {
+    GemmDesc g{};
+    g.M = g.N = np; g.K = naux; g.alpha = 1.0; g.beta = 0.0;
+    g.A = g.B = f; g.lda = g.ldb = ld; g.a_kcontig = g.b_kcontig = pair_rows ? 1 : 0;
+    g.C = out; g.ldc = np; g.batch = 1; g.sym_lower = 1;
+    return dev_gemm(g);
+  }
   const int64_t nblk = np >= 2048 ? 8 : 1;
   const int64_t w = ((np + nblk - 1) / nblk + 127) / 128 * 128;
   for (int64_t c0 = 0; c0 < np; c0 += w) {
     const int64_t cw = std::min(w, np - c0);
-    QTRY(gemm(np - c0, cw, naux, 1.0, bb + c0, np, false, bb + c0, np, false, 0.0, out + c0 * np + c0, np));
+    const double* fc = f + (pair_rows ? c0 * ld : c0);
+    QTRY(gemm(np - c0, cw, naux, 1.0, fc, ld, pair_rows, fc, ld, pair_rows, 0.0, out + c0 * np + c0, np));
   }
   if (nblk > 1) QTRY(dev_mirror_lower(np, out, np));
   return 0;
 }
-
-}
+int df_pair_product(int64_t np, int64_t naux, const double* bb, double* out) { return pair_product(np, naux, bb, np, false, out); }
+int df_pair_product_rows(int64_t np, int64_t naux, const double* bbT, double* out) { return pair_product(np, naux, bbT, naux, true, out); }
+
+}
diff --git a/quemb_amd/csrc/ao2mo.h b/quemb_amd/csrc/ao2mo.h
--- a/quemb_amd/csrc/ao2mo.h
+++ b/quemb_amd/csrc/ao2mo.h
@@ -61,5 +61,6 @@
 };
 
 int df_pair_product(int64_t np, int64_t naux, const double* bb, double* out);
+int df_pair_product_rows(int64_t np, int64_t naux, const double* bbT, double* out);
 
 }
diff --git a/quemb_amd/csrc/api.cpp b/quemb_amd/csrc/api.cpp
--- a/quemb_amd/csrc/api.cpp
+++ b/quemb_amd/csrc/api.cpp
@@ -132,6 +132,16 @@
   const GemmPlan p = pick_pair_gemm(rows, cols);
   if (cfg) *cfg = p.cfg;
   if (ksplit) *ksplit = p.ks;
+  return QEMB_OK;
+}
+int qemb_gemm_sym_tile_choice(int64_t M) { return gemm_sym_tile_choice(M); }
+int qemb_gemm_sym_tile_walk(int64_t M, int tile_rows, int tile_cols, int64_t workgroup, int64_t* count, int* tile_row, int* tile_col) {
+  if (M < 1 || tile_rows < 1 || tile_cols < 1) { set_error("qemb_gemm_sym_tile_walk: bad arguments"); return QEMB_ERR_ARG; }
+  const int64_t n = gemm_sym_tile_count(M, tile_rows, tile_cols);
+  if (count) *count = n;
+  if (workgroup < 0) return QEMB_OK;
+  if (workgroup >= n || n > 0x7fffffff || !tile_row || !tile_col) { set_error("qemb_gemm_sym_tile_walk: no such workgroup"); return QEMB_ERR_ARG; }
+  gemm_sym_tile(xcd_contiguous_index<int>((int)workgroup, (int)n), (int)((M + tile_rows - 1) / tile_rows), tile_rows, tile_cols, tile_row, tile_col);
   return QEMB_OK;
 }
 int qemb_ccsd_gemm_plans(int o, int v, int64_t* out) {
@@ -298,6 +308,7 @@
 }
 int qemb_op_pack_pm_ovvv(int64_t o, int64_t v, const double* ovvv, double* Op, int64_t ldp, double* Om, int64_t ldm) { return dev_pack_pm_ovvv(o, v, ovvv, Op, ldp, Om, ldm); }
 int qemb_op_df_pair_product(int64_t np, int64_t naux, const double* bb, double* out) { return df_pair_product(np, naux, bb, out); }
+int qemb_op_df_pair_product_rows(int64_t np, int64_t naux, const double* bbT, double* out) { return df_pair_product_rows(np, naux, bbT, out); }
 int qemb_op_unpack_tril_pair_rows(int64_t nr, int64_t n, const double* in, double* full) { return dev_unpack_tril_pair_rows(nr, n, in, full); }
 int qemb_op_unpack_tril_rows(int64_t rows, int64_t n, const double* p, double* f) { return dev_unpack_tril_rows(rows, n, p, f); }
 int qemb_op_pack_tril_rows(int64_t rows, int64_t n, const double* f, double* p) { return dev_pack_tril_rows(rows, n, f, p); }
diff --git a/quemb_amd/csrc/dev_ops.h b/quemb_amd/csrc/dev_ops.h
--- a/quemb_amd/csrc/dev_ops.h
+++ b/quemb_amd/csrc/dev_ops.h
@@ -86,6 +86,7 @@
   int ksplit = 0;
   int keep_slabs = 0;
   int64_t a_slab = 0, a_slab_skip = 0;
+  int sym_lower = 0;
 };
 inline int gemm_slab_count(int64_t K, int ksplit) {
   if (ksplit <= 1 || K <= 0) return 1;
diff --git a/quemb_amd/csrc/gemm_f64.hip b/quemb_amd/csrc/gemm_f64.hip
--- a/quemb_amd/csrc/gemm_f64.hip
+++ b/quemb_amd/csrc/gemm_f64.hip
@@ -37,13 +37,11 @@
   long long* cyc;
   int sb_m, sb_n;
   int a_slab; long long a_slab_skip;
+  int sym_tiles;
 };
 
 __device__ __forceinline__ int xcd_remap(int bid, int nwg) {
-  const int q = nwg >> 3, r = nwg & 7;
-  const int xcd = bid & 7, k = bid >> 3;
-  const int base = (xcd < r) ? xcd * (q + 1) : r * (q + 1) + (xcd - r) * q;
-  return base + k;
+  return xcd_contiguous_index<int>(bid, nwg);
 }
 
 template <int BMN, int BK, bool KCONTIG>
@@ -191,6 +189,28 @@
   return __longlong_as_double((long long)(((unsigned long long)(unsigned)hi << 32) | (unsigned)lo));
 }
 
+typedef unsigned uint2v __attribute__((ext_vector_type(2)));
+template <int SPAN>
+__device__ __forceinline__ void permlane_swap_f64(double& a, double& b) {
+  const unsigned long long ua = __double_as_longlong(a), ub = __double_as_longlong(b);
+  uint2v lo, hi;
+  if constexpr (SPAN == 32) {
+    lo = __builtin_amdgcn_permlane32_swap((unsigned)(ua & 0xffffffffu), (unsigned)(ub & 0xffffffffu), false, false);
+    hi = __builtin_amdgcn_permlane32_swap((unsigned)(ua >> 32), (unsigned)(ub >> 32), false, false);
+  } else {
+    lo = __builtin_amdgcn_permlane16_swap((unsigned)(ua & 0xffffffffu), (unsigned)(ub & 0xffffffffu), false, false);
+    hi = __builtin_amdgcn_permlane16_swap((unsigned)(ua >> 32), (unsigned)(ub >> 32), false, false);
+  }
+  a = __longlong_as_double((long long)(((unsigned long long)hi[0] << 32) | lo[0]));
+  b = __longlong_as_double((long long)(((unsigned long long)hi[1] << 32) | lo[1]));
+}
+__device__ __forceinline__ void rows_to_lanes(d4& t) {
+  double t0 = t[0], t1 = t[1], t2 = t[2], t3 = t[3];
+  permlane_swap_f64<32>(t0, t2); permlane_swap_f64<32>(t1, t3);
+  permlane_swap_f64<16>(t0, t1); permlane_swap_f64<16>(t2, t3);
+  t = d4{t0, t1, t2, t3};
+}
+
 template <int WM, int WN, int WAVES_M, int WAVES_N, int BK, bool A_KC, bool B_KC, int VEC, int TAG = 0, int MODE = 0>
 __device__ __forceinline__ void dgemm_mfma_body(const uint3 BID, const uint3 GDIM, GemmKArgs g) {
   const long long t_start = g.cyc ? (long long)__builtin_amdgcn_s_memtime() : 0;
@@ -214,10 +234,12 @@
   const int wave = tid >> 6;
   const int wm = wave / WAVES_N, wn = wave % WAVES_N;
 
-  const int ntiles = g.tiles_m * g.tiles_n;
+  constexpr bool SYM = (TAG == 6);
+  const int ntiles = SYM ? g.sym_tiles : g.tiles_m * g.tiles_n;
   const int L = xcd_remap(BID.x, ntiles);
   int tm = L % g.tiles_m, tn = L / g.tiles_m;
-  if (g.sb_m > 0) {
+  if constexpr (SYM) gemm_sym_tile(L, g.tiles_m, BM, BN, &tm, &tn);
+  else if (g.sb_m > 0) {
     const int per = g.sb_m * g.sb_n, sb = L / per, w = L - sb * per, nsbm = g.tiles_m / g.sb_m;
     tm = (sb % nsbm) * g.sb_m + w % g.sb_m;
     tn = (sb / nsbm) * g.sb_n + w / g.sb_m;
@@ -395,6 +417,25 @@
         const d2 pb = odd ? d2{r1, v[3]} : d2{v[1], r1};
         const int col = n0 + (wn * WN + j) * 16 + (fr & ~1);
         const int row = m0 + (wm * WM + i) * 16 + fk + (odd ? 8 : 0);
+        if constexpr (SYM) {
+          if (col < g.N) {
+            if (row < g.M && row > col) *reinterpret_cast<d2*>(C + (long long)row * g.ldc + col) = d2{alpha * pa[0], alpha * pa[1]};
+            else if (row == col) C[(long long)row * g.ldc + col] = alpha * pa[0];
+            if (row + 4 < g.M && row + 4 > col) *reinterpret_cast<d2*>(C + (long long)(row + 4) * g.ldc + col) = d2{alpha * pb[0], alpha * pb[1]};
+            else if (row + 4 == col) C[(long long)(row + 4) * g.ldc + col] = alpha * pb[0];
+          }
+          d4 t = v;
+          rows_to_lanes(t);
+          const int tcol = n0 + (wn * WN + j) * 16 + fr, trow = m0 + (wm * WM + i) * 16 + 4 * fk;
+          if (tcol < g.N) {
+            double* p = C + (long long)tcol * g.ldc + trow;
+#pragma unroll
+            for (int h = 0; h < 4; h += 2) {
+              if (trow + h < g.M && trow + h > tcol) *reinterpret_cast<d2*>(p + h) = d2{alpha * t[h], alpha * t[h + 1]};
+              else if (trow + h == tcol && trow + h + 1 < g.M) p[h + 1] = alpha * t[h + 1];
+            }
+          }
+        } else
         if (col < g.N) {
           if (row < g.M) {
             d2* p = reinterpret_cast<d2*>(C + (long long)row * g.ldc + col);
@@ -420,6 +461,13 @@
 #pragma unroll
         for (int r = 0; r < 4; ++r) {
           const int row = m0 + (wm * WM + i) * 16 + fk + 4 * r;
+          if constexpr (SYM) {
+            if (row < g.M && col < g.N && row >= col) {
+              const double v = alpha * acc[i][j][r];
+              C[(long long)row * g.ldc + col] = v;
+              if (row > col) C[(long long)col * g.ldc + row] = v;
+            }
+          } else
           if (row < g.M && col < g.N) {
             double* p = C + (long long)row * g.ldc + col;
             double v = alpha * acc[i][j][r];
@@ -532,7 +580,7 @@
   }
   {
     static const bool sb_on = env_flag("QEMB_GEMM_SB", true);
-    if (sb_on && d.batch == 1 && d.ksplit <= 1 && g.tiles_m >= 8 && g.tiles_n >= 4 && ((long long)g.tiles_m * g.tiles_n) % 256 == 0) {
+    if (TAG != 6 && sb_on && d.batch == 1 && d.ksplit <= 1 && g.tiles_m >= 8 && g.tiles_n >= 4 && ((long long)g.tiles_m * g.tiles_n) % 256 == 0) {
       long long best = -1;
       for (int sm = 1; sm <= 32; sm *= 2) {
         const int sn = 32 / sm;
@@ -546,7 +594,7 @@
   g.ksplit = 1; g.kchunk = g.K > 0 ? g.K : 1;
   const long long tiles = (long long)g.tiles_m * g.tiles_n * d.batch;
   if (d.keep_slabs && (d.ksplit <= 1 || d.alpha != 1.0 || d.beta != 0.0 || d.batch != 1)) { set_error("dev_gemm: keep_slabs needs ksplit > 1, alpha = 1, beta = 0, batch = 1"); return QEMB_ERR_ARG; }
-  const int want = d.ksplit > 1 ? d.ksplit : (d.ksplit == 0 && t_gemm_splitk_enabled) ? gemm_auto_ksplit(tiles, d.K) : 0;
+  const int want = TAG == 6 ? 0 : d.ksplit > 1 ? d.ksplit : (d.ksplit == 0 && t_gemm_splitk_enabled) ? gemm_auto_ksplit(tiles, d.K) : 0;
   if (want > 1) {
     long long chunk = (d.K + want - 1) / want;
     chunk = (chunk + 31) / 32 * 32;
@@ -568,7 +616,8 @@
     HIP_TRY(hipFuncSetAttribute((const void*)kern, hipFuncAttributeMaxDynamicSharedMemorySize, (int)lds));
     attr_set = true;
   }
-  dim3 grid((unsigned)(g.tiles_m * g.tiles_n), (unsigned)(d.batch * g.ksplit), 1);
+  if constexpr (TAG == 6) g.sym_tiles = (int)gemm_sym_tile_count(d.M, BM, BN);
+  dim3 grid((unsigned)(TAG == 6 ? g.sym_tiles : g.tiles_m * g.tiles_n), (unsigned)(d.batch * g.ksplit), 1);
   dim3 block(WAVES_M * WAVES_N * 64, 1, 1);
   t_gemm_last.mode = MODE; t_gemm_last.ksplit = g.ksplit; t_gemm_last.sb_m = g.sb_m; t_gemm_last.sb_n = g.sb_n;
   t_gemm_last.wide_c = gemm_wide_c(g.C, g.ldc, g.N, g.strideC, grid.y) ? 1 : 0;
@@ -606,6 +655,14 @@
   constexpr GemmTile t = gemm_tile(ID);
   static_assert(t.wm > 0, "not a tile of gemm_tiles.h");
   return launch_layout<t.wm, t.wn, t.waves_m, t.waves_n, t.bk, TAG, MODE>(d, s, vec2);
+}
+
+template <int ID>
+static int launch_sym_tile(const GemmDesc& d, hipStream_t s, bool vec2) {
+  constexpr GemmTile t = gemm_tile(ID);
+  static_assert(t.wm > 0 && t.mode1, "a MODE 1 tile of gemm_tiles.h");
+  if (d.a_kcontig) return vec2 ? launch_cfg<t.wm, t.wn, t.waves_m, t.waves_n, t.bk, true, true, 2, 6, 1>(d, s) : launch_cfg<t.wm, t.wn, t.waves_m, t.waves_n, t.bk, true, true, 1, 6, 0>(d, s);
+  return vec2 ? launch_cfg<t.wm, t.wn, t.waves_m, t.waves_n, t.bk, false, false, 2, 6, 1>(d, s) : launch_cfg<t.wm, t.wn, t.waves_m, t.waves_n, t.bk, false, false, 1, 6, 0>(d, s);
 }
 
 static bool gemm_vec2_relaxed() {
@@ -735,7 +792,15 @@
   }
   if (const char* bad = gemm_desc_error(d)) { set_error(bad); return QEMB_ERR_ARG; }
   hipStream_t s = hip_stream();
-  g_gemm_flops += 2ll * d.M * d.N * d.K * d.batch;
+  int sym_cfg = -1;
+  if (d.sym_lower) {
+    if (d.A != d.B || d.lda != d.ldb || (d.a_kcontig != 0) != (d.b_kcontig != 0) || d.M != d.N || d.batch != 1 || d.beta != 0.0 || d.a_slab > 0 || d.keep_slabs) {
+      set_error("dev_gemm: sym_lower needs the same operand on both sides (A == B, lda == ldb, a_kcontig == b_kcontig, M == N), batch = 1, beta = 0 and plain rows"); return QEMB_ERR_ARG;
+    }
+    sym_cfg = t_gemm_force_cfg >= 0 ? t_gemm_force_cfg : d.cfg >= 0 ? d.cfg : gemm_sym_tile_choice(d.M);
+    if (!gemm_sym_has_kernel(sym_cfg) || gemm_sym_tile_count(d.M, gemm_tile_rows(sym_cfg), gemm_tile_cols(sym_cfg)) > 0x7fffffff) sym_cfg = -1;
+  }
+  g_gemm_flops += sym_cfg >= 0 ? 2ll * d.K * gemm_sym_elements(d.M, gemm_tile_rows(sym_cfg), gemm_tile_cols(sym_cfg)) : 2ll * d.M * d.N * d.K * d.batch;
   {
     static FILE* shapelog = [] { const char* e = env_str("QEMB_GEMM_SHAPELOG"); return e ? std::fopen(e, "w") : (FILE*)nullptr; }();
     if (shapelog) {
@@ -764,6 +829,10 @@
   }
   t_gemm_last = GemmLaunchRecord{};
   t_gemm_last.cfg = cfg; t_gemm_last.vec2 = vec2 ? 1 : 0;
+  if (sym_cfg >= 0) {
+    t_gemm_last.cfg = sym_cfg;
+    return sym_cfg == GEMM_128x256 ? launch_sym_tile<GEMM_128x256>(d, s, vec2) : launch_sym_tile<GEMM_64x64>(d, s, vec2);
+  }
   switch (cfg) {
 #define QEMB_IF_0(...)
 #define QEMB_IF_1(...) __VA_ARGS__
diff --git a/quemb_amd/csrc/gemm_tiles.h b/quemb_amd/csrc/gemm_tiles.h
--- a/quemb_amd/csrc/gemm_tiles.h
+++ b/quemb_amd/csrc/gemm_tiles.h
@@ -69,6 +69,33 @@
   *e = table[index];
   return true;
 }
+constexpr int64_t gemm_sym_first_row_tile(int64_t J, int bm, int bn) { return J * bn / bm; }
+constexpr int64_t gemm_sym_tile_count(int64_t M, int bm, int bn) {
+  const int64_t tiles_m = (M + bm - 1) / bm, tiles_n = (M + bn - 1) / bn;
+  int64_t count = 0;
+  for (int64_t J = 0; J < tiles_n; ++J) count += tiles_m - gemm_sym_first_row_tile(J, bm, bn);
+  return count;
+}
+constexpr void gemm_sym_tile(int L, int tiles_m, int bm, int bn, int* I, int* J) {
+  int j = 0, first = 0;
+  for (int kept = tiles_m; L >= kept; kept = tiles_m - first) { L -= kept; ++j; first = (int)gemm_sym_first_row_tile(j, bm, bn); }
+  *I = first + L; *J = j;
+}
+constexpr int64_t gemm_sym_elements(int64_t M, int bm, int bn) {
+  int64_t e = 0;
+  for (int64_t J = 0; J * bn < M; ++J) e += (M - gemm_sym_first_row_tile(J, bm, bn) * bm) * ((J + 1) * bn <= M ? bn : M - J * bn);
+  return e;
+}
+constexpr bool gemm_sym_has_kernel(int cfg) { return cfg == GEMM_128x256 || cfg == GEMM_64x64; }
+constexpr int gemm_sym_tile_choice(int64_t M) { return M >= 2048 ? (int)GEMM_128x256 : (int)GEMM_64x64; }
+template <class Int>
+constexpr Int xcd_contiguous_index(Int b, Int n) {
+  const Int q = n >> 3, r = n & 7;
+  const Int xcd = b & 7, k = b >> 3;
+  const Int base = (xcd < r) ? xcd * (q + 1) : r * (q + 1) + (xcd - r) * q;
+  return base + k;
+}
+
 constexpr bool fits_one_224_tile(int64_t n) { return n > gemm_tile_rows(GEMM_192x128) && n <= gemm_tile_rows(GEMM_224x128); }
 
 }
```

Result: no change. 57.85, median of 6 (+0.5%).
